# ZhangT-tech/MoCA-Video

Hardware: AMD Instinct MI355X
Metric: denoising UNet-steps/sec @16x320x512 fp16 (higher is better)
Workload: dtype f16

## Files before the change

include/moca_hip.h:

```cpp
#ifndef MOCA_HIP_H
#define MOCA_HIP_H

#include <stdint.h>

#ifdef __cplusplus
extern "C" {
#endif

#define MOCA_OK            0
#define MOCA_E_BADARG     -1
#define MOCA_E_LAUNCH     -2
#define MOCA_E_NODEVICE   -3
#define MOCA_E_GRAPH      -4

#define MOCA_A_LINEAR   0
#define MOCA_A_CONV3X3  1
#define MOCA_A_TCONV3   2

#define MOCA_EP_GEGLU   1
#define MOCA_EP_OUT_F32 2
#define MOCA_FORCE_SMALL_TILE 4
#define MOCA_EP_COLSUM 16
#define MOCA_EP_LN     32
#define MOCA_EP_GELU    8
#define MOCA_EP_ROWSUM 64
#define MOCA_EP_GSTAT  256
#define MOCA_EP_TATTN  512
#define MOCA_EP_LNFOLD 128

#define MOCA_EP_SLABS 1024

typedef struct moca_gemm_params {
    const void* a;
    const void* w;
    void*       out;
    const float* bias;
    const void* rowadd;
    const void* residual;
    float*      splitk_ws;
    int32_t M, N, K;
    int32_t lda, ldw, ldo, ldr, ld_rowadd;
    int32_t rowadd_div;
    int32_t a_mode;
    int32_t C;
    int32_t inH, inW;
    int32_t outH, outW;
    int32_t stride;
    int32_t up;
    int32_t T;
    int32_t HW;
    int32_t flags;
    int32_t splits;
    int32_t nopad_lo;
    int32_t prefetch_kib;
    int32_t tattn_causal;
    float*      colsum;
    const float* ln_gamma;
    const float* ln_beta;
    void*       ln_out;
    int32_t     ld_ln;
    float       ln_eps;
    float*      rowsum;
    const float* lnf_part;
    const float* lnf_wsum;
    int32_t     lnf_nparts;
    int32_t     reserved2_;
    int64_t*    gstat;
    int32_t     gstat_rows;
    float       tattn_scale;
    const void* prefetch;
    int32_t     up_phase;
    int32_t     reserved4_;
    const void* a2;
    int32_t     lda2;
    int32_t     k1;
    int32_t     gstat_cpg;
    int32_t     gstat_coff;
    int32_t     wgroup_rows;
    int32_t     wgroup_stride;
} moca_gemm_params;

int moca_gemm_f16(const moca_gemm_params* p, void* stream);
int moca_gemm_colsum_rows(const moca_gemm_params* p);
int moca_gemm_ln_ok(const moca_gemm_params* p);
int moca_gemm_rowsum_cols(const moca_gemm_params* p);
int moca_gemm_lnfold_ok(const moca_gemm_params* p);
int moca_gemm_tattn_ok(const moca_gemm_params* p);
int moca_gemm_wgroup_ok(const moca_gemm_params* p);
int moca_gemm_cat_ok(const moca_gemm_params* p);
#define MOCA_ROUTE_SMALL64   1
#define MOCA_ROUTE_SMALL128  2
#define MOCA_ROUTE_GLDS128   3
#define MOCA_ROUTE_GLDS160   4
#define MOCA_ROUTE_G4        5
#define MOCA_ROUTE_W80       6
#define MOCA_ROUTE_W80W      7
#define MOCA_ROUTE_SQ256     8
#define MOCA_ROUTE_G4P       9
#define MOCA_ROUTE_SQP       10
#define MOCA_ROUTE_TATTN     11
#define MOCA_ROUTE_WS        12
int moca_gemm_route(const moca_gemm_params* p);
int moca_gemm_splitk_groupnorm_ok(const moca_gemm_params* p, int32_t HW, int32_t frames_per_stat);
int moca_gemm_splitk_groupnorm_f16(const moca_gemm_params* p, void* y, const float* gamma, const float* beta, int32_t HW,
                                   int32_t frames_per_stat, float eps, int32_t silu, int32_t write_x, void* stream);
int64_t moca_gemm_splitk_ws_bytes(int32_t M, int32_t N, int32_t splits);

int moca_groupnorm_nhwc_f16(const void* x, void* y, const float* gamma, const float* beta,
                            int32_t F, int32_t HW, int32_t C, int32_t frames_per_stat,
                            float eps, int32_t silu, float* ws, void* stream);
int64_t moca_groupnorm_ws_bytes(int32_t F, int32_t HW, int32_t C);
int moca_groupnorm_colsum_f16(const void* x, void* y, const float* gamma, const float* beta, const float* colsum,
                              int32_t tile_rows, int32_t F, int32_t HW, int32_t C, int32_t frames_per_stat,
                              float eps, int32_t silu, float* ws, void* stream);

int moca_groupnorm_fold_weights_f16(const void* w, const float* bias, const float* gamma, const float* beta, const int64_t* gstat,
                                    void* wg, float* bg, int32_t n_sg, int32_t N, int32_t K, int32_t ldw, int64_t count, float eps,
                                    void* stream);

int moca_groupnorm_gstat_f16(const void* x, void* y, const float* gamma, const float* beta, const int64_t* gstat,
                             int32_t F, int32_t HW, int32_t C, int32_t frames_per_stat,
                             float eps, int32_t silu, void* stream);
int moca_concat_channels_gstat_f16(const void* a, const void* b, void* out, int32_t F, int32_t HW, int32_t C1, int32_t C2,
                                   int32_t frames_per_stat, int64_t* gstat, void* stream);
int moca_groupnorm_gstat_cat_f16(const void* a, const void* b, void* y, const float* gamma, const float* beta,
                                 const int64_t* gstat_cat, const int64_t* gstat_b, int32_t Fb, int32_t F, int32_t HW, int32_t C1,
                                 int32_t C2, int32_t frames_per_stat, float eps, int32_t silu, void* stream);
int moca_gstat_accum_f16(const void* x, int32_t F, int32_t HW, int32_t C, int32_t frames_per_stat, int32_t cpg, int32_t coff,
                         int64_t* gstat, void* stream);
int moca_memset_zero(void* ptr, int64_t bytes, void* stream);

int moca_layernorm_f16(const void* x, void* y, const float* gamma, const float* beta,
                       int32_t M, int32_t C, float eps, void* stream);

int moca_attention_f16(const void* q, const void* k, const void* v, void* out,
                       int32_t Bq, int32_t heads, int32_t Nq, int32_t Nk,
                       int32_t ldq, int32_t ldk, int32_t ldv, int32_t ldo,
                       int32_t kv_div, float scale, void* stream);

int moca_attention_ip_f16(const void* q, const void* k, const void* v, const void* k_ip, const void* v_ip, void* out,
                          int32_t Bq, int32_t heads, int32_t Nq, int32_t Nt, int32_t Ni,
                          int32_t ldq, int32_t ldk, int32_t ldv, int32_t ldk_ip, int32_t ldv_ip, int32_t ldo,
                          int32_t kv_div, float scale, float ip_scale, void* stream);

int moca_attention_causal_f16(const void* q, const void* k, const void* v, void* out,
                              int32_t B, int32_t heads, int32_t N, int32_t ldq, int32_t ldk, int32_t ldv, int32_t ldo,
                              float scale, void* stream);

int moca_temporal_attention_f16(const void* q, const void* k, const void* v, void* out,
                                int32_t B, int32_t T, int32_t HW, int32_t heads,
                                int32_t ld_qkv, int32_t ldo, float scale, void* stream);
int moca_temporal_attention_causal_f16(const void* q, const void* k, const void* v, void* out,
                                       int32_t B, int32_t T, int32_t HW, int32_t heads,
                                       int32_t ld_qkv, int32_t ldo, float scale, void* stream);
int moca_temporal_attention_long_f16(const void* q, const void* k, const void* v, void* out,
                                     int32_t B, int32_t T, int32_t HW, int32_t heads,
                                     int32_t ld_qkv, int32_t ldo, float scale, int32_t causal, void* stream);

int moca_ncthw_to_nhwc_f16(const void* x, int32_t x_is_f32, void* y, int32_t B, int32_t Cin,
                           int32_t T, int32_t HW, int32_t Cpad, void* stream);
int moca_ncthw_scatter_f16(const void* x, int32_t x_is_f32, void* y, int32_t B, int32_t k, int32_t T,
                           int32_t HW, int32_t Cpad, int32_t c0, void* stream);
int moca_nchw_add_rows_f16(void* rows, const void* src, int32_t src_is_f32, int32_t F, int32_t Fsrc, int32_t C,
                           int32_t HW, int32_t ld, void* stream);
int moca_nhwc_to_ncthw(const void* y, int32_t ld, void* x, int32_t x_is_f32, int32_t B,
                       int32_t Cout, int32_t T, int32_t HW, void* stream);
int moca_concat_channels_f16(const void* a, const void* b, void* out, int64_t rows,
                             int32_t C1, int32_t C2, void* stream);
int moca_repeat_f16(const void* src, void* dst, int64_t bytes, int32_t reps, void* stream);
int moca_timestep_embedding_f16(const int64_t* t, void* out, int32_t n, int32_t dim,
                                float max_period, void* stream);
int moca_silu_add_rows_f16(const void* a, int32_t div_a, const void* b, int32_t div_b, void* out,
                           int32_t rows, int32_t C, int32_t apply_silu, void* stream);

int moca_embed_tokens_f16(const int64_t* tokens, const float* table, const float* pos, void* out,
                          int32_t n_tokens, int32_t L, int32_t C, int32_t vocab, void* stream);

int moca_attention_d80_f16(const void* q, const void* k, const void* v, void* out,
                           int32_t B, int32_t heads, int32_t N, int32_t ldq, int32_t ldk, int32_t ldv, int32_t ldo,
                           float scale, void* stream);
int moca_clip_preprocess_patches_f16(const void* img, int32_t img_is_f32, void* out, int32_t B, int32_t H, int32_t W,
                                     int32_t size, int32_t patch, int32_t ldo, int32_t antialias, void* stream);
int moca_clip_assemble_tokens_f16(const float* patch, int32_t ldp, const float* cls, const float* pos, void* out, int32_t B, int32_t P,
                                  int32_t C, void* stream);

int moca_channel_mix_f16(const void* z, int32_t z_is_f32, const float* w, const float* bias, void* out,
                         int32_t B, int32_t Cin, int32_t T, int32_t HW, int32_t Cout, int32_t Cpad,
                         float inv_scale, void* stream);
int moca_gaussian_sample_f32(const float* moments, const float* noise, float* out, int32_t n, int32_t z, int32_t hw,
                             float scale, void* stream);
int moca_softmax_rows_f16(const float* s, void* p, int64_t R, int32_t N, int64_t lds, int64_t ldp, float scale,
                          void* stream);

int moca_cfg_combine_f32(const float* e_c, const float* e_u, float* out, float scale,
                         int64_t n, void* stream);
int moca_ddim_update_f32(const float* x, const float* e, const float* noise, float* x_prev,
                         float* pred_x0, float a_t, float a_prev, float sigma_t,
                         float sqrt_one_minus_at, int32_t use_scale, float scale_t,
                         float scale_prev, int64_t n, void* stream);
int moca_q_sample_f32(const float* x0, const float* noise, float* out, const float* coef_x, const float* coef_n,
                      const int64_t* t, int32_t B, int32_t n_tab, int64_t per, void* stream);
int moca_fifo_ddim_step_f32(const float* sample, const float* eps, const float* noise,
                            float* momentum, float* x_prev, float* pred_x0,
                            const float* coef, const float* mask, const float* cond,
                            const int32_t* mask_index, const float* enh, float* ws,
                            int32_t B, int32_t C, int32_t F, int32_t Fm, int32_t HW,
                            float beta, float one_minus_beta, float gamma, float one_minus_gamma,
                            void* stream);

typedef struct moca_fifo_state {
    int32_t head;
    int32_t iter;
    uint32_t seed_lo, seed_hi;
    int32_t ext_noise;
    int32_t reserved_[3];
} moca_fifo_state;

int moca_fifo_randn_f32(const moca_fifo_state* state, float* out, int64_t n, void* stream);
int moca_fifo_gather_windows_f32(const moca_fifo_state* state, const float* queue, float* x, float* anchor,
                                 const int32_t* win_start, int32_t nW, int32_t reps, int32_t C, int32_t Q, int32_t f,
                                 int32_t HW, void* stream);
typedef struct moca_fifo_step_params {
    const moca_fifo_state* state;
    const float* x;
    const float* eps_c;
    const float* eps_u;
    const float* noise;
    float* momentum;
    float* queue;
    float* x_prev;
    float* pred_x0;
    const float* coef;
    const int32_t* win_start;
    const float* mask;
    const float* mask_sums;
    const int32_t* mask_frame;
    const float* enh;
    const float* cond;
    const float* sam_eff;
    const int32_t* sam_idx;
    float cfg_scale, beta, one_minus_beta, gamma, one_minus_gamma;
    int32_t nW, C, Q, f, HW, wb_from;
} moca_fifo_step_params;
int moca_fifo_step_windows_f32(const moca_fifo_step_params* p, void* stream);
int moca_sam_select_masks_f32(const float* cand, const int32_t* cand_off, const int32_t* ncand, const int64_t* t_rows, float* eff,
                              int32_t* eff_idx, int32_t nW, int32_t f, int32_t HW, void* stream);
int moca_fifo_advance_f32(moca_fifo_state* state, float* queue, const float* newframe, float* emitted, int32_t n_slots,
                          int32_t emit_frame, float* mask, float* mask_sums, int32_t C, int32_t Q, int32_t HW, void* stream);
int moca_fifo_prepare_queue_f32(const float* z, const float* noise, float* queue, const float* coef_z, const float* coef_noise,
                                const int32_t* frame_idx, int32_t BC, int32_t Tz, int32_t Q, int32_t HW, void* stream);
int moca_base_set_timestep(const moca_fifo_state* state, const int64_t* table, int32_t S, int64_t* rows, int32_t n, void* stream);
int moca_base_ddim_step_f32(moca_fifo_state* state, float* x, const float* eps_c, const float* eps_u, const float* noise,
                            float* pred_x0, const float* coef, int32_t S, float cfg_scale, int32_t use_scale, int64_t n, void* stream);
int moca_mask_frame_sums_f32(const float* mask, float* sums, int32_t frames, int32_t HW, void* stream);

int moca_freq_mix_3d_f32(const float* x, const float* noise, const float* lpf, float* out,
                         int32_t C, int32_t T, int32_t H, int32_t W, float* ws, void* stream);
int64_t moca_freq_mix_ws_bytes(int32_t C, int32_t T, int32_t H, int32_t W);
int moca_freq_filter_f32(float* lpf, int32_t T, int32_t H, int32_t W, int32_t type, int32_t n,
                         double d_s, double d_t, void* stream);

int moca_graph_begin(void* stream);
int moca_graph_end(void* stream, void** graph_exec_out);
int moca_graph_launch(void* graph_exec, void* stream);
int moca_graph_destroy(void* graph_exec);
int moca_stream_create(void** stream_out);
int moca_stream_destroy(void* stream);
int moca_stream_sync(void* stream);
int moca_event_create(void** ev_out);
int moca_event_record(void* ev, void* stream);
int moca_event_elapsed_ms(void* ev_start, void* ev_stop, float* ms_out);
int moca_event_destroy(void* ev);

#define MOCA_TUNE_GEMM_W80   0
#define MOCA_TUNE_GEMM_G4    1
#define MOCA_TUNE_GEMM_SQ256 2
#define MOCA_TUNE_GEMM_WIDE  3
#define MOCA_TUNE_GN_SLAB    4
#define MOCA_TUNE_GEMM_G4P   5
#define MOCA_TUNE_GEMM_MF32  6
#define MOCA_TUNE_GEMM_SQP   7
#define MOCA_TUNE_SQP_WALK   8
#define MOCA_TUNE_SLAB_F16   9
#define MOCA_TUNE_GEMM_WS    10
#define MOCA_TUNE_COUNT      11
int moca_set_tuning(int32_t knob, int32_t value);
int moca_debug_clock_sampler(void* buf, int32_t blocks, int32_t nsamples, const int32_t* stop, void* stream);

int moca_device_info(char* name, int32_t len, int32_t* cu_count);
const char* moca_version(void);

#ifdef __cplusplus
}
#endif
#endif
```

moca_video_amd/csrc/gemm.hip:

```cpp
#include "gemm_launch.h"

namespace {

template <int BN, int AMODE>
__global__ __launch_bounds__(256, 2) void gemm_f16_kernel(const moca_gemm_params p) {
    constexpr int NT = BN / 64;
    constexpr int B_SLOTS = BN / 32;
    constexpr int A_BYTES = BM * ROW_BYTES;
    constexpr int B_BYTES = BN * ROW_BYTES;

    extern __shared__ __attribute__((aligned(16))) char smem[];
    char* sA = smem;
    char* sB = smem + 2 * A_BYTES;

    const int tid = threadIdx.x, lane = tid & 63, wave = tid >> 6;
    const int wave_m = wave >> 1, wave_n = wave & 1;

    const int tiles_m = (p.M + BM - 1) / BM;
    const int tiles_n = p.N / BN;
    const int nblk = tiles_m * tiles_n * p.splits;
    int logical;
    remap_block<BN>(nblk, logical);
    const int split = logical % p.splits;
    const int tile = logical / p.splits;
// ... 148 lines not shown
                    acc[mt][nt] = __builtin_amdgcn_mfma_f32_32x32x16_f16(af[mt], bf[nt], acc[mt][nt], 0, 0, 0);
        }
        if (has_next) store_tile(cur ^ 1);
        __syncthreads();
        cur ^= 1;
    }

    if (p.splits > 1) {
        float* ws = p.splitk_ws + (int64_t)split * p.M * p.N;
#pragma unroll
        for (int mt = 0; mt < 2; ++mt)
#pragma unroll
            for (int nt = 0; nt < NT; ++nt)
#pragma unroll
                for (int r = 0; r < 16; ++r) {
                    const int row = m0 + wave_m * 64 + mt * 32 + (r & 3) + 8 * (r >> 2) + 4 * fh;
                    const int col = n0 + wave_n * (BN / 2) + nt * 32 + frow;
                    if (row < p.M) ws[(int64_t)row * p.N + col] = acc[mt][nt][r];
                }
        return;
    }

    float* sC = reinterpret_cast<float*>(smem);
    const bool geglu = (p.flags & MOCA_EP_GEGLU) != 0;
    const int out_bn = geglu ? BN / 2 : BN;
    if (geglu) {
        if constexpr (NT == 2) {
            const int ncol = n0 + wave_n * 64 + frow;
            const float bv = p.bias ? p.bias[ncol] : 0.f;
            const float bg = p.bias ? p.bias[ncol + 32] : 0.f;
#pragma unroll
            for (int mt = 0; mt < 2; ++mt)
#pragma unroll
                for (int r = 0; r < 16; ++r) {
                    const int row = wave_m * 64 + mt * 32 + (r & 3) + 8 * (r >> 2) + 4 * fh;
                    const float v = acc[mt][0][r] + bv;
                    const float g = acc[mt][1][r] + bg;
                    sC[row * out_bn + wave_n * 32 + frow] = v * moca_gelu(g);
                }
        }
    } else {
#pragma unroll
        for (int nt = 0; nt < NT; ++nt) {
            const int col = wave_n * (BN / 2) + nt * 32 + frow;
            const float bv = p.bias ? p.bias[n0 + col] : 0.f;
#pragma unroll
            for (int mt = 0; mt < 2; ++mt)
#pragma unroll
                for (int r = 0; r < 16; ++r) {
                    const int row = wave_m * 64 + mt * 32 + (r & 3) + 8 * (r >> 2) + 4 * fh;
                    const float v = acc[mt][nt][r] + bv;
                    sC[row * out_bn + col] = (p.flags & MOCA_EP_GELU) ? moca_gelu(v) : v;
                }
        }
    }
    __syncthreads();

    const int chunks_per_row = out_bn / 8;
    const int total_chunks = BM * chunks_per_row;
    const int on0 = geglu ? n0 / 2 : n0;
    const half_t* __restrict__ rowadd = reinterpret_cast<const half_t*>(p.rowadd);
    const half_t* __restrict__ resid = reinterpret_cast<const half_t*>(p.residual);
    for (int idx = tid; idx < total_chunks; idx += 256) {
        const int row = idx / chunks_per_row, ch = idx - row * chunks_per_row;
        const int m = m0 + row;
        if (m >= p.M) continue;
        const int col = on0 + ch * 8;
        float v[8];
        const f32x4 c0 = *reinterpret_cast<const f32x4*>(sC + row * out_bn + ch * 8);
        const f32x4 c1 = *reinterpret_cast<const f32x4*>(sC + row * out_bn + ch * 8 + 4);
        v[0] = c0[0]; v[1] = c0[1]; v[2] = c0[2]; v[3] = c0[3];
        v[4] = c1[0]; v[5] = c1[1]; v[6] = c1[2]; v[7] = c1[3];
        if (rowadd) {
            const half8v e = *reinterpret_cast<const half8v*>(rowadd + (int64_t)(m / p.rowadd_div) * p.ld_rowadd + col);
#pragma unroll
            for (int j = 0; j < 8; ++j) v[j] += (float)e[j];
        }
        if (resid) {
            const half8v e = *reinterpret_cast<const half8v*>(resid + (int64_t)m * p.ldr + col);
#pragma unroll
            for (int j = 0; j < 8; ++j) v[j] += (float)e[j];
        }
        if (p.flags & MOCA_EP_OUT_F32) {
            float* o = reinterpret_cast<float*>(p.out) + (int64_t)m * p.ldo + col;
            *reinterpret_cast<f32x4*>(o) = f32x4{v[0], v[1], v[2], v[3]};
            *reinterpret_cast<f32x4*>(o + 4) = f32x4{v[4], v[5], v[6], v[7]};
        } else {
            half8v h;
#pragma unroll
            for (int j = 0; j < 8; ++j) h[j] = (half_t)v[j];
            *reinterpret_cast<half8v*>(reinterpret_cast<half_t*>(p.out) + (int64_t)m * p.ldo + col) = h;
        }
    }
}

__global__ __launch_bounds__(256) void splitk_reduce_kernel(const moca_gemm_params p) {
    const bool geglu = (p.flags & MOCA_EP_GEGLU) != 0;
    const int out_n = geglu ? p.N / 2 : p.N;
    const int cpr = out_n / 8;
    const int64_t total = (int64_t)p.M * cpr;
    const half_t* __restrict__ rowadd = reinterpret_cast<const half_t*>(p.rowadd);
    const half_t* __restrict__ resid = reinterpret_cast<const half_t*>(p.residual);
    for (int64_t idx = (int64_t)blockIdx.x * 256 + threadIdx.x; idx < total; idx += (int64_t)gridDim.x * 256) {
        const int m = (int)(idx / cpr), ch = (int)(idx - (int64_t)m * cpr);
        const int col = ch * 8;
        float v[8];
        if (geglu) {
            const int vc = (col / 32) * 64 + (col % 32);
            float a[8], g[8];
#pragma unroll
            for (int j = 0; j < 8; ++j) { a[j] = p.bias ? p.bias[vc + j] : 0.f; g[j] = p.bias ? p.bias[vc + 32 + j] : 0.f; }
            for (int s = 0; s < p.splits; ++s) {
                const float* w = p.splitk_ws + ((int64_t)s * p.M + m) * p.N + vc;
                const f32x4 a0 = *reinterpret_cast<const f32x4*>(w), a1 = *reinterpret_cast<const f32x4*>(w + 4);
                const f32x4 g0 = *reinterpret_cast<const f32x4*>(w + 32), g1 = *reinterpret_cast<const f32x4*>(w + 36);
#pragma unroll
                for (int j = 0; j < 4; ++j) { a[j] += a0[j]; a[4 + j] += a1[j]; g[j] += g0[j]; g[4 + j] += g1[j]; }
            }
#pragma unroll
            for (int j = 0; j < 8; ++j) v[j] = a[j] * moca_gelu(g[j]);
        } else {
#pragma unroll
            for (int j = 0; j < 8; ++j) v[j] = p.bias ? p.bias[col + j] : 0.f;
            if (p.reserved4_ & 4) {
                for (int s = 0; s < p.splits; ++s) {
                    const half8v a = *reinterpret_cast<const half8v*>(reinterpret_cast<const half_t*>(p.splitk_ws) + ((int64_t)s * p.M + m) * p.N + col);
#pragma unroll
                    for (int j = 0; j < 8; ++j) v[j] += (float)a[j];
                }
            } else {
                for (int s = 0; s < p.splits; ++s) {
                    const float* w = p.splitk_ws + ((int64_t)s * p.M + m) * p.N + col;
                    const f32x4 a0 = *reinterpret_cast<const f32x4*>(w), a1 = *reinterpret_cast<const f32x4*>(w + 4);
#pragma unroll
                    for (int j = 0; j < 4; ++j) { v[j] += a0[j]; v[4 + j] += a1[j]; }
                }
            }
        }
        if (rowadd) {
            const half8v e = *reinterpret_cast<const half8v*>(rowadd + (int64_t)(m / p.rowadd_div) * p.ld_rowadd + col);
#pragma unroll
            for (int j = 0; j < 8; ++j) v[j] += (float)e[j];
        }
        if (resid) {
            const half8v e = *reinterpret_cast<const half8v*>(resid + (int64_t)m * p.ldr + col);
#pragma unroll
            for (int j = 0; j < 8; ++j) v[j] += (float)e[j];
        }
        if (p.flags & MOCA_EP_OUT_F32) {
            float* o = reinterpret_cast<float*>(p.out) + (int64_t)m * p.ldo + col;
            *reinterpret_cast<f32x4*>(o) = f32x4{v[0], v[1], v[2], v[3]};
            *reinterpret_cast<f32x4*>(o + 4) = f32x4{v[4], v[5], v[6], v[7]};
        } else {
            half8v h;
#pragma unroll
            for (int j = 0; j < 8; ++j) h[j] = (half_t)v[j];
            *reinterpret_cast<half8v*>(reinterpret_cast<half_t*>(p.out) + (int64_t)m * p.ldo + col) = h;
        }
    }
}

template <int CPT>
__global__ __launch_bounds__(1024) void splitk_gn_kernel(const moca_gemm_params p, half_t* __restrict__ y, const float* __restrict__ gamma,
                                                         const float* __restrict__ beta, int R, int cpg, double inv_count, float eps,
                                                         int silu, int write_x) {
    __shared__ float s_red[2][16];
    __shared__ float s_sc[128], s_sh[128];
    const int tid = threadIdx.x, nthr = blockDim.x;
    const int slab = blockIdx.x, sg = slab / 32, g = slab % 32;
    const int vpr = cpg / 8, nchunks = R * vpr;
    const int N = p.N;
    const half_t* __restrict__ rowadd = reinterpret_cast<const half_t*>(p.rowadd);
    const half_t* __restrict__ resid = reinterpret_cast<const half_t*>(p.residual);
    const float gm_t = tid < cpg ? gamma[g * cpg + tid] : 0.f, bt_t = tid < cpg ? beta[g * cpg + tid] : 0.f;
    half8v v[CPT];
    int mrow[CPT], ccol[CPT];
    float s = 0.f, q = 0.f;
#pragma unroll
    for (int i = 0; i < CPT; ++i) {
        const int idx = tid + i * nthr;
        mrow[i] = -1;
        if (idx < nchunks) {
            const int row = idx / vpr, c = idx - row * vpr;
            const int m = sg * R + row, col = g * cpg + c * 8;
            mrow[i] = m; ccol[i] = col;
            float a[8];
#pragma unroll
            for (int j = 0; j < 8; ++j) a[j] = p.bias ? p.bias[col + j] : 0.f;
            if (p.reserved4_ & 4) {
                for (int sp = 0; sp < p.splits; ++sp) {
                    const half8v h = *reinterpret_cast<const half8v*>(reinterpret_cast<const half_t*>(p.splitk_ws) + ((int64_t)sp * p.M + m) * N + col);
#pragma unroll
                    for (int j = 0; j < 8; ++j) a[j] += (float)h[j];
                }
            } else {
                for (int sp = 0; sp < p.splits; ++sp) {
                    const float* w = p.splitk_ws + ((int64_t)sp * p.M + m) * N + col;
                    const f32x4 a0 = *reinterpret_cast<const f32x4*>(w), a1 = *reinterpret_cast<const f32x4*>(w + 4);
#pragma unroll
                    for (int j = 0; j < 4; ++j) { a[j] += a0[j]; a[4 + j] += a1[j]; }
                }
            }
            if (rowadd) {
                const half8v e = *reinterpret_cast<const half8v*>(rowadd + (int64_t)(m / p.rowadd_div) * p.ld_rowadd + col);
#pragma unroll
                for (int j = 0; j < 8; ++j) a[j] += (float)e[j];
            }
            if (resid) {
                const half8v e = *reinterpret_cast<const half8v*>(resid + (int64_t)m * p.ldr + col);
#pragma unroll
                for (int j = 0; j < 8; ++j) a[j] += (float)e[j];
            }
#pragma unroll
            for (int j = 0; j < 8; ++j) v[i][j] = (half_t)a[j];
            if (write_x) *reinterpret_cast<half8v*>(reinterpret_cast<half_t*>(p.out) + (int64_t)m * p.ldo + col) = v[i];
        }
    }
#pragma unroll
    for (int i = 0; i < CPT; ++i)
        if (mrow[i] >= 0) {
#pragma unroll
            for (int j = 0; j < 8; ++j) { const float a = (float)v[i][j]; s += a; q += a * a; }
        }
    s = wave_sum(s); q = wave_sum(q);
    if ((tid & 63) == 0) { s_red[0][tid >> 6] = s; s_red[1][tid >> 6] = q; }
    __syncthreads();
    if (tid < cpg) {
        double a = 0.0, b = 0.0;
        for (int w = 0; w < (nthr >> 6); ++w) { a += (double)s_red[0][w]; b += (double)s_red[1][w]; }
        const double mean = a * inv_count;
        double var = b * inv_count - mean * mean;
        if (var < 0.0) var = 0.0;
        const float rstd = (float)(1.0 / sqrt(var + (double)eps));
        const float sc = rstd * gm_t;
        s_sc[tid] = sc;
        s_sh[tid] = bt_t - (float)mean * sc;
    }
    __syncthreads();
#pragma unroll
    for (int i = 0; i < CPT; ++i)
        if (mrow[i] >= 0) {
            const int c0 = ccol[i] - g * cpg;
            half8v r;
#pragma unroll
            for (int j = 0; j < 8; ++j) {
                float a = (float)v[i][j] * s_sc[c0 + j] + s_sh[c0 + j];
                if (silu) a = moca_silu(a);
                r[j] = (half_t)a;
            }
            *reinterpret_cast<half8v*>(y + (int64_t)mrow[i] * N + ccol[i]) = r;
        }
}

template <int BN, int AMODE>
int launch_gemm(const moca_gemm_params& p, hipStream_t st) {
    const int tiles_m = (p.M + BM - 1) / BM, tiles_n = p.N / BN;
    const int nblk = tiles_m * tiles_n * p.splits;
    constexpr int lds_pipe = 2 * (BM + BN) * ROW_BYTES;
    constexpr int lds_epi = BM * BN * 4;
    constexpr int lds = lds_pipe > lds_epi ? lds_pipe : lds_epi;
    if (!dyn_lds_once<&gemm_f16_kernel<BN, AMODE>>(lds)) return MOCA_E_LAUNCH;
    hipLaunchKernelGGL((gemm_f16_kernel<BN, AMODE>), dim3(nblk), dim3(256), lds, st, p);
    MOCA_CHECK_LAUNCH();
    return MOCA_OK;
}
int launch_gemm_small(int bn, const moca_gemm_params& p, hipStream_t st) {
    if (bn == 128) return with_gather(p, [&](auto am, auto) { return launch_gemm<128, decltype(am)::value>(p, st); });
    return with_gather(p, [&](auto am, auto) { return launch_gemm<64, decltype(am)::value>(p, st); });
}

enum Route : int {
    R_NONE = 0,
    R_SMALL64 = MOCA_ROUTE_SMALL64, R_SMALL128 = MOCA_ROUTE_SMALL128, R_GLDS128 = MOCA_ROUTE_GLDS128, R_GLDS160 = MOCA_ROUTE_GLDS160,
    R_G4 = MOCA_ROUTE_G4, R_W80 = MOCA_ROUTE_W80, R_W80W = MOCA_ROUTE_W80W, R_SQ256 = MOCA_ROUTE_SQ256, R_G4P = MOCA_ROUTE_G4P,
    R_SQP = MOCA_ROUTE_SQP, R_TATTN = MOCA_ROUTE_TATTN, R_WS = MOCA_ROUTE_WS,
};

void normalise_splits(moca_gemm_params& p) {
    if (p.splits < 1) p.splits = 1;
    if (p.splits > (p.K + BK - 1) / BK) p.splits = (p.K + BK - 1) / BK;
    if (p.splits > 1) {
        const int nkt = (p.K + BK - 1) / BK, kts = (nkt + p.splits - 1) / p.splits;
        p.splits = (nkt + kts - 1) / kts;
    }
}

inline int64_t a_span_bytes(const moca_gemm_params& p) {
    if (p.a_mode == MOCA_A_LINEAR) return ((int64_t)p.M * p.lda + 64) * 2;
    if (p.a_mode == MOCA_A_CONV3X3) return ((int64_t)(p.M / (p.outH * p.outW)) * p.inH * p.inW * p.C + 64) * 2;
    return ((int64_t)p.M * p.C + 64) * 2;
}
inline bool buffer_addressable(const moca_gemm_params& p) {
    if (p.a2 && ((int64_t)p.M * p.lda2 + 64) * 2 >= (1ll << 31)) return false;
    return a_span_bytes(p) < (1ll << 31) && (int64_t)p.N * p.ldw * 2 < (1ll << 31);
}

bool persistent_ok(const moca_gemm_params& p, int BN, int blocks) {
    if (p.a_mode != MOCA_A_LINEAR || p.splits != 1 || p.N % BN || p.K % 64 || !buffer_addressable(p)) return false;
    if (p.flags & ~(MOCA_EP_GEGLU | MOCA_EP_LNFOLD)) return false;
    if ((p.flags & MOCA_EP_GEGLU) && (p.residual || p.rowadd)) return false;
    return ((p.M + 255) / 256) * (p.N / BN) >= blocks;
}

Route route_of(const moca_gemm_params& p) {
    if (p.flags & MOCA_EP_TATTN) return R_TATTN;
    const int ws_mode = moca_tuning_get(MOCA_TUNE_GEMM_WS);
    if (ws_mode && moca_gemm_ws_ok(p) && (ws_mode == 2 || p.residual || p.M >= (1 << 17))) return R_WS;
    if (!p.a2 && p.wgroup_rows <= 0) {
        const int sqp_mode = moca_tuning_get(MOCA_TUNE_GEMM_SQP), g4p_mode = moca_tuning_get(MOCA_TUNE_GEMM_G4P);
        if (sqp_mode && persistent_ok(p, 256, SQP_BLOCKS) && (sqp_mode == 2 || (p.flags & MOCA_EP_GEGLU))) return R_SQP;
        if (g4p_mode && persistent_ok(p, 128, G4P_BLOCKS) && (g4p_mode == 2 || (p.flags & MOCA_EP_GEGLU))) return R_G4P;
    }
    const int w80_mode = moca_tuning_get(MOCA_TUNE_GEMM_W80);
    const int tiles320 = ((p.M + 319) / 320) * (p.N / 160);
    if (w80_mode && p.N % 160 == 0 && !(p.flags & (MOCA_EP_GEGLU | MOCA_EP_OUT_F32 | MOCA_FORCE_SMALL_TILE)) && p.M > 160 &&
        (tiles320 * p.splits >= 200 || w80_mode == 2) && fast_gather(p) && buffer_addressable(p)) {
        if (p.flags & MOCA_EP_LN) return R_W80W;
        const int wide_mode = moca_tuning_get(MOCA_TUNE_GEMM_WIDE);
        if (wide_mode == 0 || p.N % 320) return R_W80;
        return (p.a_mode == MOCA_A_LINEAR || wide_mode == 2) ? R_W80W : R_W80;
    }
    const int g4_mode = moca_tuning_get(MOCA_TUNE_GEMM_G4);
    const bool use_g4 = !(p.flags & MOCA_EP_OUT_F32) &&
                        (g4_mode == 2 || (g4_mode == 1 && (p.flags & MOCA_EP_GEGLU) && p.K <= 640 && p.M < (1 << 17)));
    const int sq256_mode = moca_tuning_get(MOCA_TUNE_GEMM_SQ256);
    if (sq256_mode && p.a_mode == MOCA_A_LINEAR && p.N % 256 == 0 && p.N >= 2560 && p.M >= 512 && fast_gather(p) && buffer_addressable(p) &&
        !(p.flags & (MOCA_EP_OUT_F32 | MOCA_FORCE_SMALL_TILE)) && ((p.M + 255) / 256) * (p.N / 256) * p.splits >= 200 &&
        (sq256_mode == 2 || !use_g4)) return R_SQ256;
    const int big_bn = (p.N % 128 == 0) ? 128 : (p.N % 160 == 0 ? 160 : 0);
    if (big_bn != 0 && p.M > 128 && !(p.flags & MOCA_FORCE_SMALL_TILE)) {
        if (big_bn == 128) return use_g4 ? R_G4 : R_GLDS128;
        return R_GLDS160;
    }
    return p.N % 128 == 0 ? R_SMALL128 : R_SMALL64;
}

constexpr int CAN_SPLITK = 1 << 16, CAN_A2 = 1 << 17, CAN_WGROUP = 1 << 18, CAN_UP_PHASE = 1 << 19;
constexpr int EP_STATS = MOCA_EP_COLSUM | MOCA_EP_GSTAT;
struct RouteInfo { int tm, tn, can; };
RouteInfo route_info(Route r) {
    constexpr int GLDS = MOCA_EP_GEGLU | MOCA_EP_OUT_F32 | EP_STATS | MOCA_EP_ROWSUM | MOCA_EP_LNFOLD | CAN_SPLITK | CAN_UP_PHASE;
    constexpr int W80 = EP_STATS | MOCA_EP_ROWSUM | MOCA_EP_LNFOLD | CAN_SPLITK | CAN_UP_PHASE | CAN_A2 | CAN_WGROUP;
    switch (r) {
        case R_SMALL64: return {BM, 64, MOCA_EP_OUT_F32 | MOCA_EP_GELU | CAN_SPLITK};
        case R_SMALL128: return {BM, 128, MOCA_EP_GEGLU | MOCA_EP_OUT_F32 | MOCA_EP_GELU | CAN_SPLITK};
        case R_GLDS128: return {256, 128, GLDS};
        case R_GLDS160: return {256, 160, GLDS};
        case R_G4: return {256, 128, MOCA_EP_GEGLU | MOCA_EP_LNFOLD | CAN_SPLITK | CAN_UP_PHASE};
        case R_W80: return {320, 160, W80};
        case R_W80W: return {160, 320, W80 | MOCA_EP_LN};
        case R_SQ256: return {256, 256, MOCA_EP_GEGLU | MOCA_EP_LNFOLD | CAN_SPLITK};
        case R_G4P: return {256, 128, MOCA_EP_GEGLU | MOCA_EP_LNFOLD};
        case R_SQP: return {256, 256, MOCA_EP_GEGLU | MOCA_EP_LNFOLD};
        case R_TATTN: return {320, 192, MOCA_EP_TATTN | MOCA_EP_LNFOLD};
        case R_WS: return {32, 80, MOCA_EP_ROWSUM | MOCA_EP_GSTAT | CAN_WGROUP};
        case R_NONE: break;
    }
    return {0, 0, 0};
}

bool route_can(Route r, const moca_gemm_params& p) {
    const RouteInfo ri = route_info(r);
    const int f = p.flags & ~(MOCA_FORCE_SMALL_TILE | MOCA_EP_SLABS);
    const int wants = f | (p.splits > 1 ? CAN_SPLITK : 0) | (p.a2 ? CAN_A2 : 0) | (p.wgroup_rows ? CAN_WGROUP : 0) | (p.up_phase ? CAN_UP_PHASE : 0);
    if (r == R_NONE || (wants & ~ri.can) || p.wgroup_rows < 0) return false;
    if (r == R_WS) return true;
    const bool linear1 = p.a_mode == MOCA_A_LINEAR && p.splits == 1;
    if (r == R_TATTN) {
        if (!linear1 || !fast_gather(p) || !buffer_addressable(p) || p.residual || p.rowadd || (p.flags & MOCA_FORCE_SMALL_TILE)) return false;
        if (p.N % 192 || p.T != 16 || p.HW <= 0 || p.HW % 20 || p.M % (16 * p.HW)) return false;
        if (p.ldo % 4 || p.ldo < p.N / 3) return false;
        return p.tattn_causal == 0 || (p.tattn_causal == 1 && p.tattn_scale > 0.f);
    }
    if ((f & EP_STATS) && (p.splits != 1 || (f & (MOCA_EP_GEGLU | MOCA_EP_OUT_F32)))) return false;
    if ((f & MOCA_EP_ROWSUM) && (p.splits != 1 || (f & (MOCA_EP_GEGLU | MOCA_EP_OUT_F32 | EP_STATS | MOCA_EP_LN | MOCA_EP_GELU)))) return false;
    if ((f & MOCA_EP_LN) && !(linear1 && p.N == 320 && !(f & EP_STATS))) return false;
    if ((f & MOCA_EP_LNFOLD) && !(linear1 && !(f & (MOCA_EP_OUT_F32 | EP_STATS | MOCA_EP_LN | MOCA_EP_ROWSUM | MOCA_EP_GELU)) &&
                                  !((r == R_GLDS128 || r == R_GLDS160) && (f & MOCA_EP_GEGLU)))) return false;
    if ((f & MOCA_EP_GELU) && (f & MOCA_EP_GEGLU)) return false;
    if (p.a2) {
        if (!linear1 || (f & ~(EP_STATS | MOCA_EP_ROWSUM))) return false;
        if (p.k1 <= 0 || p.k1 >= p.K || p.k1 % 64 || (p.K - p.k1) % 64 || p.lda % 8 || p.lda2 % 8 || p.lda < p.k1 || p.lda2 < p.K - p.k1) return false;
    }
    if (p.wgroup_rows) {
        if (!linear1 || p.a2 || p.wgroup_stride < p.N * p.ldw || (f & ~(EP_STATS | MOCA_EP_ROWSUM | MOCA_EP_LN))) return false;
        if (p.M % p.wgroup_rows || p.wgroup_rows % ri.tm) return false;
        if ((int64_t)(p.M / p.wgroup_rows) * p.wgroup_stride * 2 >= (1ll << 31)) return false;
    }
    if (p.up_phase && (p.splits != 1 || p.M <= 160 || !fast_gather(p) || p.residual || p.rowadd || (f & ~MOCA_EP_GSTAT) ||
                       (p.N % 128 && p.N % 160))) return false;
    return true;
}

Route checked_route(const moca_gemm_params& p) {
    const Route r = route_of(p);
    return route_can(r, p) ? r : R_NONE;
}

Route query_route(const moca_gemm_params* pp, int flag, moca_gemm_params& p) {
    if (!pp) return R_NONE;
    p = *pp;
    if (p.M <= 0 || p.N <= 0 || p.K <= 0 || p.N % 64 || p.K % 8) return R_NONE;
    normalise_splits(p);
    p.flags |= flag;
    return checked_route(p);
}

bool slab_f16(Route r, const moca_gemm_params& p) {
    return moca_tuning_get(MOCA_TUNE_SLAB_F16) && p.splits > 1 && !(p.flags & (MOCA_EP_GEGLU | MOCA_EP_OUT_F32)) && (r == R_GLDS128 || r == R_GLDS160);
}
bool splitk_gn_ok(const moca_gemm_params& p, int HW, int fps) {
    if (p.splits < 2 || (p.flags & ~MOCA_EP_SLABS) || p.N % 32 || (p.N / 32) % 8 || p.N / 32 > 128 || p.up_phase) return false;
    if (HW <= 0 || fps <= 0 || p.M % (HW * fps)) return false;
    const int64_t nchunks = (int64_t)HW * fps * (p.N / 32 / 8);
    return nchunks >= 64 && nchunks <= 4096;
}

Route prepare(const moca_gemm_params* pp, moca_gemm_params& p) {
    if (!pp) return R_NONE;
    p = *pp;
    if (p.splits < 1) p.splits = 1;
    if (!p.a || !p.w || !p.out) return R_NONE;
    if (p.M <= 0 || p.N <= 0 || p.K <= 0) return R_NONE;
    if (p.N % 64 || p.K % 8 || p.ldw % BK || p.ldw < ((p.K + BK - 1) / BK) * BK) return R_NONE;
    const bool geglu = p.flags & MOCA_EP_GEGLU;
    if (geglu && p.N % 128) return R_NONE;
    if (p.ldo % 8 || (p.residual && p.ldr % 8) || (p.rowadd && (p.ld_rowadd % 8 || p.rowadd_div <= 0))) return R_NONE;
    if (p.splits > 1 && !p.splitk_ws) return R_NONE;
    if (p.prefetch_kib < 0 || (p.prefetch_kib > 0 && (!p.prefetch || (reinterpret_cast<uintptr_t>(p.prefetch) & 15)))) return R_NONE;
    if ((p.flags & MOCA_EP_GELU) && (p.splits != 1 || !((p.flags & MOCA_FORCE_SMALL_TILE) || p.M <= 128))) return R_NONE;
    normalise_splits(p);
    if ((p.flags & MOCA_EP_SLABS) && (p.splits < 2 || (p.flags & ~MOCA_EP_SLABS))) return R_NONE;
    if (p.up_phase && p.a_mode != MOCA_A_CONV3X3) return R_NONE;
    switch (p.a_mode) {
        case MOCA_A_LINEAR:
            if (!p.a2 && (p.lda % 8 || p.lda < p.K)) return R_NONE;
            break;
        case MOCA_A_CONV3X3:
            if (p.up_phase < 0 || p.up_phase > 4) return R_NONE;
            if (p.C % 8 || p.K != (p.up_phase ? 4 : 9) * p.C || p.inH <= 0 || p.inW <= 0 || p.outH <= 0 || p.outW <= 0) return R_NONE;
            if (p.up_phase && (p.stride != 1 || p.up || p.nopad_lo)) return R_NONE;
            if (p.stride != 1 && p.stride != 2) return R_NONE;
            if (p.nopad_lo != 0 && (p.nopad_lo != 1 || p.stride != 2 || p.up || (p.inH | p.inW) & 1)) return R_NONE;
            if (p.up && (p.stride != 1 || p.outH != 2 * p.inH || p.outW != 2 * p.inW)) return R_NONE;
            if (!p.up && p.stride == 1 && (p.outH != p.inH || p.outW != p.inW)) return R_NONE;
            if (p.stride == 2 && (p.outH != (p.inH - 1) / 2 + 1 || p.outW != (p.inW - 1) / 2 + 1)) return R_NONE;
            if (p.M % (p.outH * p.outW)) return R_NONE;
            break;
        case MOCA_A_TCONV3:
            if (p.C % 8 || p.K != 3 * p.C || p.T <= 0 || p.HW <= 0 || p.M % (p.T * p.HW)) return R_NONE;
            break;
        default:
            return R_NONE;
    }
    if (p.a2 && p.a_mode != MOCA_A_LINEAR) return R_NONE;
    if (p.gstat_cpg < 0 || p.gstat_coff < 0 || ((p.gstat_cpg || p.gstat_coff) && !(p.flags & MOCA_EP_GSTAT))) return R_NONE;
    if (p.tattn_causal && !(p.flags & MOCA_EP_TATTN)) return R_NONE;
    const Route r = checked_route(p);
    if (r == R_NONE) return R_NONE;
    if ((p.flags & MOCA_EP_COLSUM) && !p.colsum) return R_NONE;
    if ((p.flags & MOCA_EP_LN) && !(p.ln_gamma && p.ln_beta && p.ln_out && p.ld_ln % 8 == 0)) return R_NONE;
    if ((p.flags & MOCA_EP_ROWSUM) && !p.rowsum) return R_NONE;
    if ((p.flags & MOCA_EP_LNFOLD) && !(p.lnf_part && p.lnf_wsum && p.lnf_nparts >= 1)) return R_NONE;
    if ((p.flags & MOCA_EP_GSTAT) &&
        !(p.gstat && !(p.flags & MOCA_EP_COLSUM) && p.gstat_rows > 0 && p.gstat_rows % route_info(r).tm == 0 && p.M % p.gstat_rows == 0 &&
          (p.gstat_cpg > 0 ? (p.gstat_coff + p.N - 1) / p.gstat_cpg < 32 : (p.N % 32 == 0 && p.gstat_coff == 0)))) return R_NONE;
    p.reserved4_ = 0;
    if ((int64_t)p.M * (geglu ? p.N / 2 : p.N) * 2 >= (128ll << 20)) p.reserved4_ |= 1;
    if (slab_f16(r, p)) p.reserved4_ |= 4;
    return r;
}

int launch_route(Route r, const moca_gemm_params& p, hipStream_t st) {
    switch (r) {
        case R_TATTN: return moca_gemm_w80s_launch(3, p, st);
        case R_WS: return moca_gemm_ws_launch(p, st);
        case R_SQP: return moca_gemm_sqp_launch(p, st);
        case R_G4P: return moca_gemm_g4p_launch(p, st);
        case R_W80: return moca_gemm_w80s_launch(0, p, st);
        case R_W80W: return moca_gemm_w80s_launch(1, p, st);
        case R_SQ256: return moca_gemm_w80s_launch(2, p, st);
        case R_G4: return moca_gemm_g4_launch(p, st);
        case R_GLDS128: return moca_gemm_glds_launch(128, p, st);
        case R_GLDS160: return moca_gemm_glds_launch(160, p, st);
        case R_SMALL128: return launch_gemm_small(128, p, st);
        case R_SMALL64: return launch_gemm_small(64, p, st);
        case R_NONE: break;
    }
    return MOCA_E_BADARG;
}

}

#ifdef MOCA_STAMPS
extern "C" int moca_debug_stamps(unsigned long long* host_out, int n_blocks) {
    if (n_blocks > STAMP_BLOCKS) n_blocks = STAMP_BLOCKS;
    return hipMemcpyFromSymbol(host_out, HIP_SYMBOL(g_stamps), (size_t)n_blocks * STAMP_SLOTS * 8) == hipSuccess ? 0 : -2;
}
#endif

extern "C" int moca_gemm_route(const moca_gemm_params* pp) {
    moca_gemm_params p;
    return prepare(pp, p);
}

extern "C" int moca_gemm_colsum_rows(const moca_gemm_params* pp) {
    moca_gemm_params p;
    return route_info(query_route(pp, (pp && (pp->flags & MOCA_EP_GSTAT)) ? 0 : MOCA_EP_COLSUM, p)).tm;
}
extern "C" int moca_gemm_rowsum_cols(const moca_gemm_params* pp) {
    moca_gemm_params p;
    return route_info(query_route(pp, MOCA_EP_ROWSUM, p)).tn;
}
extern "C" int moca_gemm_ln_ok(const moca_gemm_params* pp) {
    moca_gemm_params p;
    return query_route(pp, MOCA_EP_LN, p) != R_NONE;
}
extern "C" int moca_gemm_lnfold_ok(const moca_gemm_params* pp) {
    moca_gemm_params p;
    return query_route(pp, MOCA_EP_LNFOLD, p) != R_NONE;
}
extern "C" int moca_gemm_tattn_ok(const moca_gemm_params* pp) {
    moca_gemm_params p;
    return query_route(pp, MOCA_EP_TATTN, p) != R_NONE;
}
extern "C" int moca_gemm_cat_ok(const moca_gemm_params* pp) {
    moca_gemm_params p;
    return query_route(pp, 0, p) != R_NONE && p.a2;
}
extern "C" int moca_gemm_wgroup_ok(const moca_gemm_params* pp) {
    moca_gemm_params p;
    return query_route(pp, 0, p) != R_NONE && p.wgroup_rows > 0;
}
extern "C" int moca_gemm_splitk_groupnorm_ok(const moca_gemm_params* pp, int32_t HW, int32_t frames_per_stat) {
    moca_gemm_params p;
    return query_route(pp, 0, p) != R_NONE && splitk_gn_ok(p, HW, frames_per_stat);
}

extern "C" int moca_gemm_splitk_groupnorm_f16(const moca_gemm_params* pp, void* y, const float* gamma, const float* beta, int32_t HW,
                                              int32_t frames_per_stat, float eps, int32_t silu, int32_t write_x, void* stream) {
    if (!pp || !y || !gamma || !beta) return MOCA_E_BADARG;
    moca_gemm_params p = *pp;
    if (p.M <= 0 || p.N <= 0 || p.K <= 0 || p.N % 64 || p.K % 8 || !p.splitk_ws || (write_x && !p.out)) return MOCA_E_BADARG;
    if (p.ldo % 8 || (p.residual && p.ldr % 8) || (p.rowadd && (p.ld_rowadd % 8 || p.rowadd_div <= 0))) return MOCA_E_BADARG;
    normalise_splits(p);
    if (!splitk_gn_ok(p, HW, frames_per_stat)) return MOCA_E_BADARG;
    p.reserved4_ = slab_f16(route_of(p), p) ? 4 : 0;
    const int cpg = p.N / 32, R = HW * frames_per_stat;
    const int nchunks = R * (cpg / 8);
    const int cpt = (nchunks + 1023) / 1024;
    int thr = ((nchunks + cpt - 1) / cpt + 63) / 64 * 64;
    if (thr < (cpg + 63) / 64 * 64) thr = (cpg + 63) / 64 * 64;
    const int n_slabs = (p.M / R) * 32;
    const double inv_count = 1.0 / ((double)R * cpg);
    hipStream_t st = moca_stream(stream);
    half_t* yo = reinterpret_cast<half_t*>(y);
#define MOCA_SKGN(CPT) hipLaunchKernelGGL(splitk_gn_kernel<CPT>, dim3(n_slabs), dim3(thr), 0, st, p, yo, gamma, beta, R, cpg, inv_count, eps, silu, write_x)
    if (cpt == 1) MOCA_SKGN(1); else if (cpt == 2) MOCA_SKGN(2); else if (cpt == 3) MOCA_SKGN(3); else MOCA_SKGN(4);
#undef MOCA_SKGN
    MOCA_CHECK_LAUNCH();
    return MOCA_OK;
}

extern "C" int64_t moca_gemm_splitk_ws_bytes(int32_t M, int32_t N, int32_t splits) {
    return splits > 1 ? (int64_t)splits * M * N * 4 : 0;
}

extern "C" int moca_gemm_f16(const moca_gemm_params* pp, void* stream) {
    moca_gemm_params p;
    const Route r = prepare(pp, p);
    if (r == R_NONE) return MOCA_E_BADARG;
    hipStream_t st = moca_stream(stream);
    const int rc = launch_route(r, p, st);
    if (rc != MOCA_OK) return rc;
    if (p.splits > 1 && !(p.flags & MOCA_EP_SLABS)) {
        const int out_n = (p.flags & MOCA_EP_GEGLU) ? p.N / 2 : p.N;
        const int64_t total = (int64_t)p.M * (out_n / 8);
        int blocks = (int)((total + 255) / 256);
        if (blocks > 2048) blocks = 2048;
        hipLaunchKernelGGL(splitk_reduce_kernel, dim3(blocks), dim3(256), 0, st, p);
        MOCA_CHECK_LAUNCH();
    }
    return MOCA_OK;
}

#ifdef MOCA_DIAG_NAME
extern "C" const char* moca_version(void) { return "moca_hip 0.1 (gfx950) DIAG:" MOCA_DIAG_NAME; }
#else
extern "C" const char* moca_version(void) { return "moca_hip 0.1 (gfx950)"; }
#endif
```

moca_video_amd/csrc/gemm_launch.h:

```cpp
#ifndef MOCA_GEMM_LAUNCH_H
#define MOCA_GEMM_LAUNCH_H
#include "gemm_device.h"

int moca_gemm_glds_launch(int bn, const moca_gemm_params& p, hipStream_t st);
int moca_gemm_g4_launch(const moca_gemm_params& p, hipStream_t st);
int moca_gemm_w80s_launch(int shape, const moca_gemm_params& p, hipStream_t st);
int moca_gemm_g4p_launch(const moca_gemm_params& p, hipStream_t st);
int moca_gemm_sqp_launch(const moca_gemm_params& p, hipStream_t st);

namespace {

constexpr int G4P_BLOCKS = 512;
constexpr int SQP_BLOCKS = 256;

static int choose_xcd_n(const moca_gemm_params& p, int tiles_m, int tiles_n, int BN) {
    if (p.splits != 1 || p.a_mode != MOCA_A_LINEAR) return 1;
    const double Wtot = (double)p.N * p.K * 2, Atot = (double)p.M * p.K * 2;
    auto cost = [&](int xn) {
        const int xm = 8 / xn;
        const double wsub = (double)(tiles_n / xn) * BN * p.K * 2;
        return (wsub <= 3.6e6 ? xm * Wtot : tiles_m * Wtot) + xn * Atot;
    };
    double best = cost(1);
    int best_xn = 1;
    for (int xn = 2; xn <= 8; xn *= 2) {
        if (tiles_m % (8 / xn) || tiles_n % xn) continue;
        const double c = cost(xn);
        if (c < 0.8 * best) { best = c; best_xn = xn; }
    }
    return best_xn;
}

inline bool fast_gather(const moca_gemm_params& p) {
    return (p.a_mode == MOCA_A_LINEAR) ? (p.K % BK == 0 && p.K <= 8192) : (p.C % BK == 0 && p.C <= 8192);
}
template <typename F>
int with_gather(const moca_gemm_params& p, F f) {
    const bool fast = fast_gather(p);
    if (p.a_mode == MOCA_A_LINEAR) return fast ? f(int_c<MOCA_A_LINEAR>{}, yes_t{}) : f(int_c<MOCA_A_LINEAR>{}, no_t{});
    if (p.a_mode == MOCA_A_CONV3X3) return fast ? f(int_c<MOCA_A_CONV3X3>{}, yes_t{}) : f(int_c<MOCA_A_CONV3X3>{}, no_t{});
    return fast ? f(int_c<MOCA_A_TCONV3>{}, yes_t{}) : f(int_c<MOCA_A_TCONV3>{}, no_t{});
}

template <auto KERNEL>
bool dyn_lds_once(int lds) {
    static bool attr_set = false;
    if (!attr_set) {
        if (hipFuncSetAttribute(reinterpret_cast<const void*>(KERNEL), hipFuncAttributeMaxDynamicSharedMemorySize, lds) != hipSuccess) return false;
        attr_set = true;
    }
    return true;
}

}

#endif
```

moca_video_amd/csrc/gemm_persistent.hip:

```cpp
#include "gemm_launch.h"

namespace {

__device__ __forceinline__ int g4p_perm(int rho) {
    const int wn = rho >> 6, nt = (rho >> 4) & 3, j = rho & 15;
    return wn * 64 + (nt >> 1) * 32 + 8 * (j >> 2) + 4 * (nt & 1) + (j & 3);
}
__device__ __forceinline__ void st_out8_nt(half_t* ptr, const half8v v, bool nt) { st_out8(ptr, v, nt); }

template <bool GEGLU>
__global__ __launch_bounds__(256, 2) void gemm_g4p_kernel(const moca_gemm_params p) {
#if defined(__HIP_DEVICE_COMPILE__)
    constexpr int TM = 256, BN = 128, KS = 32, RB = 64, MT = 8, NT = 4;
    constexpr int A_BYTES = TM * RB, STAGE = A_BYTES + BN * RB, RING = 3 * STAGE;
    constexpr int NMMA = MT * NT;
    extern __shared__ __attribute__((aligned(16))) char smem[];
    float* lst = reinterpret_cast<float*>(smem + RING);
    float* lws = lst + 2 * TM;
    float* lbi = lws + BN;

    const int tid = threadIdx.x, lane = tid & 63;
    const int wave = __builtin_amdgcn_readfirstlane(tid >> 6);
    const int wave_m = wave >> 1, wave_n = wave & 1;
    const int nper = p.reserved2_;
// ... 200 lines not shown
#pragma unroll
                    for (int r = 0; r < 4; ++r) { o[r] = v[2 * hh][r]; o[4 + r] = v[2 * hh + 1][r]; }
                    if (m < p.M) {
                        if (rowadd) {
                            const half8v e = *reinterpret_cast<const half8v*>(rowadd + (int64_t)(m / p.rowadd_div) * p.ld_rowadd + col);
#pragma unroll
                            for (int r = 0; r < 8; ++r) o[r] = (float)(half_t)o[r] + (float)e[r];
                        }
                        if (resid) {
                            const half8v e = *reinterpret_cast<const half8v*>(resid + (int64_t)m * p.ldr + col);
#pragma unroll
                            for (int r = 0; r < 8; ++r) o[r] = (rowadd ? o[r] : (float)(half_t)o[r]) + (float)e[r];
                        }
                        half8v h;
#pragma unroll
                        for (int r = 0; r < 8; ++r) h[r] = (half_t)o[r];
                        st_out8(reinterpret_cast<half_t*>(p.out) + (int64_t)m * p.ldo + col, h, nt_out);
                    }
                }
            }
        }
#ifdef MOCA_STAMPS
        if (stamp_it) { MOCA_STAMP(5); MOCA_STAMP_HW(); }
        ++tile_no;
#endif
        if (t_next < 0) break;
        t_cur = t_next;
        asm volatile("s_waitcnt vmcnt(0) lgkmcnt(0)" ::: "memory");
        __builtin_amdgcn_s_barrier();
    }
#endif
}

__device__ __forceinline__ int g4q_perm(int rho) {
    const int wn = rho >> 6, nt = (rho >> 5) & 1, i = rho & 31;
    const int g = i >> 3, h = (i >> 2) & 1, r = i & 3;
    return wn * 64 + nt * 32 + 16 * (g >> 1) + 8 * h + 4 * (g & 1) + r;
}
template <bool GEGLU>
__global__ __launch_bounds__(256, 2) void gemm_g4q_kernel(const moca_gemm_params p) {
#if defined(__HIP_DEVICE_COMPILE__)
    constexpr int TM = 256, BN = 128, KS = 32, RB = 64, MT = 4, NT = 2;
    constexpr int A_BYTES = TM * RB, STAGE = A_BYTES + BN * RB, RING = 3 * STAGE;
        extern __shared__ __attribute__((aligned(16))) char smem[];
    float* lst = reinterpret_cast<float*>(smem + RING);
    float* lws = lst + 2 * TM;
    float* lbi = lws + BN;

    const int tid = threadIdx.x, lane = tid & 63;
    const int wave = __builtin_amdgcn_readfirstlane(tid >> 6);
    const int wave_m = wave >> 1, wave_n = wave & 1;
    const int nper = p.reserved2_;
    if (prefetch_block(p, nper, 256)) return;

    const int tiles_n = p.N / BN;
    const int ntiles = ((p.M + TM - 1) / TM) * tiles_n;
    int t_cur, t_end;
    const int J = nper >> 3;
    {
        const int x = blockIdx.x & 7, j = blockIdx.x >> 3;
        const int q = ntiles >> 3, r = ntiles & 7;
        const int start = x < r ? x * (q + 1) : r * (q + 1) + (x - r) * q;
        t_cur = start + j;
        t_end = start + q + (x < r ? 1 : 0);
    }
    if (t_cur >= t_end) return;
    const int nk = 2 * (p.K / 64);

    const int lrow = lane >> 2, pch = lane & 3;
    const int lch = pch ^ ((0x78 >> (2 * ((lrow >> 2) & 3))) & 3);
    const __amdgpu_buffer_rsrc_t rsrc_a = __builtin_amdgcn_make_buffer_rsrc(const_cast<void*>(p.a), 0, OOB_OFF, 0x00020000);
    const __amdgpu_buffer_rsrc_t rsrc_w = __builtin_amdgcn_make_buffer_rsrc(const_cast<void*>(p.w), 0, OOB_OFF, 0x00020000);
    unsigned a_off[4], w_off[2];
    int w_perm[2];
#pragma unroll
    for (int g = 0; g < 2; ++g) w_perm[g] = g4q_perm((g * 4 + wave) * 16 + lrow);
    auto set_dma_tile = [&](int t) {
        const int tm = t / tiles_n, tn = t - tm * tiles_n;
#pragma unroll
        for (int g = 0; g < 4; ++g) {
            const int row = tm * TM + (g * 4 + wave) * 16 + lrow;
            a_off[g] = (t >= 0 && row < p.M) ? (unsigned)(((int64_t)row * p.lda + lch * 8) * 2) : OOB_OFF;
        }
#pragma unroll
        for (int g = 0; g < 2; ++g)
            w_off[g] = t >= 0 ? (unsigned)(((int64_t)(tn * BN + w_perm[g]) * p.ldw + lch * 8) * 2) : OOB_OFF;
    };
    auto dma_piece = [&](int kt, int slot, int j) {
        const lds_ptr sa = (lds_ptr)smem + slot * STAGE;
        const unsigned soff = (unsigned)(kt * KS * 2);
        if (j < 4) __builtin_amdgcn_raw_ptr_buffer_load_lds(rsrc_a, sa + (j * 4 + wave) * 1024, 16, a_off[j], soff, 0, 0);
        else __builtin_amdgcn_raw_ptr_buffer_load_lds(rsrc_w, sa + A_BYTES + ((j - 4) * 4 + wave) * 1024, 16, w_off[j - 4], soff, 0, 0);
    };

    const int fr = lane & 31, fh = lane >> 5;
    int fa_off[MT][2], fb_off[NT][2];
#pragma unroll
    for (int ks = 0; ks < 2; ++ks) {
#pragma unroll
        for (int mt = 0; mt < MT; ++mt) {
            const int row = wave_m * 128 + mt * 32 + fr;
            fa_off[mt][ks] = row * RB + (((2 * ks + fh) ^ ((0x78 >> (2 * ((row >> 2) & 3))) & 3)) << 4);
        }
#pragma unroll
        for (int nt = 0; nt < NT; ++nt) {
            const int row = wave_n * 64 + nt * 32 + fr;
            fb_off[nt][ks] = A_BYTES + row * RB + (((2 * ks + fh) ^ ((0x78 >> (2 * ((row >> 2) & 3))) & 3)) << 4);
        }
    }

    f32x16 acc[MT][NT];
    half8v af[MT][2], bf[NT][2];
    int s0 = 0, s1 = 1, s2 = 2;
    auto phase = [&](auto even_tag, int kt2) {
        constexpr bool even = decltype(even_tag)::value;
        const char* cur = smem + s0 * STAGE;
#pragma unroll
        for (int ks = 0; ks < 2; ++ks) {
#pragma unroll
            for (int nt = 0; nt < NT; ++nt) bf[nt][ks] = *reinterpret_cast<const half8v*>(cur + fb_off[nt][ks]);
#pragma unroll
            for (int mt = 0; mt < MT; ++mt) af[mt][ks] = *reinterpret_cast<const half8v*>(cur + fa_off[mt][ks]);
        }
        if constexpr (even) {
            asm volatile("s_waitcnt lgkmcnt(0)" ::: "memory");
            __builtin_amdgcn_s_barrier();
        }
        __builtin_amdgcn_s_setprio(1);
#pragma unroll
        for (int j = 0; j < 2 * MT * NT; ++j) {
            const int ks = j / (MT * NT), mt = (j / NT) % MT, nt = j % NT;
            acc[mt][nt] = __builtin_amdgcn_mfma_f32_32x32x16_f16(bf[nt][ks], af[mt][ks], acc[mt][nt], 0, 0, 0);
            if constexpr (even) {
                if ((j & 1) && j / 2 < 6) {
                    dma_piece(kt2, s2, j / 2);
                    dma_piece(kt2 + 1, s0, j / 2);
                    __builtin_amdgcn_sched_barrier(0);
                }
            }
        }
        __builtin_amdgcn_s_setprio(0);
        { const int t = s0; s0 = s1; s1 = s2; s2 = t; }
    };

    const bool fold = (p.flags & MOCA_EP_LNFOLD) != 0;
    float2 rp0, rp1;
    float rws, rbi;
    auto stat_issue = [&](int t) {
        const int tm = t / tiles_n, tn = t - tm * tiles_n;
        rp0 = float2{0.f, 0.f}; rp1 = float2{0.f, 0.f}; rws = 0.f; rbi = 0.f;
        if (tid < BN) {
            const int n = tn * BN + g4q_perm(tid);
            if (fold) rws = p.lnf_wsum[n];
            if (p.bias) rbi = p.bias[n];
        }
        if (fold) {
            const int m = min(tm * TM + tid, p.M - 1);
            rp0 = *reinterpret_cast<const float2*>(p.lnf_part + (int64_t)m * 2);
            if (p.lnf_nparts > 1) rp1 = *reinterpret_cast<const float2*>(p.lnf_part + ((int64_t)p.M + m) * 2);
        }
    };
    auto stat_publish = [&](int t) {
        float rs = 1.f, rb = 0.f;
        if (fold) {
            const int tm = t / tiles_n;
            const int m = min(tm * TM + tid, p.M - 1);
            float s = rp0.x + rp1.x, q = rp0.y + rp1.y;
            for (int i = 2; i < p.lnf_nparts; ++i) {
                const float2 v = *reinterpret_cast<const float2*>(p.lnf_part + ((int64_t)i * p.M + m) * 2);
                s += v.x; q += v.y;
            }
            const float inv_k = 1.0f / (float)p.K;
            const float mean = s * inv_k;
            const float var = fmaxf(q * inv_k - mean * mean, 0.f);
            rs = rsqrtf(var + p.ln_eps);
            rb = -mean * rs;
        }
        *reinterpret_cast<float2*>(lst + 2 * tid) = float2{rs, rb};
        if (tid < BN) { lws[tid] = rws; lbi[tid] = rbi; }
    };

    stat_issue(t_cur);
    set_dma_tile(t_cur);
#pragma unroll
    for (int j = 0; j < 6; ++j) { dma_piece(0, 0, j); dma_piece(1, 1, j); }
    asm volatile("s_waitcnt vmcnt(0)" ::: "memory");
    __builtin_amdgcn_s_barrier();

    const bool nt_out = out_streams(p);
    const half_t* __restrict__ resid = reinterpret_cast<const half_t*>(p.residual);
    const half_t* __restrict__ rowadd = reinterpret_cast<const half_t*>(p.rowadd);
    while (true) {
        const int t_next = t_cur + J < t_end ? t_cur + J : -1;
        const int tm = t_cur / tiles_n, tn = t_cur - tm * tiles_n;
        const int m0 = tm * TM, n0 = tn * BN;
#pragma unroll
        for (int mt = 0; mt < MT; ++mt)
#pragma unroll
            for (int nt = 0; nt < NT; ++nt)
#pragma unroll
                for (int r = 0; r < 16; ++r) acc[mt][nt][r] = 0.f;
        for (int i = 0; i < nk; i += 2) {
            const bool last = i + 2 >= nk;
            if (last) set_dma_tile(t_next);
            phase(yes_t{}, last ? 0 : i + 2);
            asm volatile("s_waitcnt lgkmcnt(0)" ::: "memory");
            __builtin_amdgcn_s_barrier();
            phase(no_t{}, 0);
            if (!last) {
                asm volatile("s_waitcnt vmcnt(0) lgkmcnt(0)" ::: "memory");
                __builtin_amdgcn_s_barrier();
            }
        }
        stat_publish(t_cur);
        if (t_next >= 0) stat_issue(t_next);
        asm volatile("s_waitcnt lgkmcnt(0)" ::: "memory");
        __builtin_amdgcn_s_barrier();

        f32x4 cw[NT][4], cb[NT][4];
        if constexpr (GEGLU) {
#pragma unroll
            for (int nt = 0; nt < NT; ++nt)
#pragma unroll
                for (int g = 0; g < 4; ++g) {
                    cw[nt][g] = *reinterpret_cast<const f32x4*>(lws + wave_n * 64 + nt * 32 + 8 * g + 4 * fh);
                    cb[nt][g] = *reinterpret_cast<const f32x4*>(lbi + wave_n * 64 + nt * 32 + 8 * g + 4 * fh);
                }
        }
#pragma unroll
        for (int mt = 0; mt < MT; ++mt) {
            const int rl = wave_m * 128 + mt * 32 + fr;
            const int m = m0 + rl;
            const float2 st = *reinterpret_cast<const float2*>(lst + 2 * rl);
#pragma unroll
            for (int s = 0; s < 2; ++s) {
                f32x4 v[NT][2];
#pragma unroll
                for (int nt = 0; nt < NT; ++nt)
#pragma unroll
                    for (int gg = 0; gg < 2; ++gg) {
                        const int g = 2 * s + gg;
                        const f32x4 a4 = {acc[mt][nt][4 * g], acc[mt][nt][4 * g + 1], acc[mt][nt][4 * g + 2], acc[mt][nt][4 * g + 3]};
                        if constexpr (!GEGLU) {
                            cw[nt][g] = *reinterpret_cast<const f32x4*>(lws + wave_n * 64 + nt * 32 + 8 * g + 4 * fh);
                            cb[nt][g] = *reinterpret_cast<const f32x4*>(lbi + wave_n * 64 + nt * 32 + 8 * g + 4 * fh);
                        }
                        v[nt][gg] = st.x * a4 + (st.y * cw[nt][g] + cb[nt][g]);
                    }
                if constexpr (GEGLU) {
                    half8v h;
#pragma unroll
                    for (int gg = 0; gg < 2; ++gg) {
                        const f32x2 lo = moca_geglu2(f32x2{v[0][gg][0], v[0][gg][1]}, f32x2{v[1][gg][0], v[1][gg][1]});
                        const f32x2 hi = moca_geglu2(f32x2{v[0][gg][2], v[0][gg][3]}, f32x2{v[1][gg][2], v[1][gg][3]});
                        h[4 * gg + 0] = (half_t)lo[0]; h[4 * gg + 1] = (half_t)lo[1]; h[4 * gg + 2] = (half_t)hi[0]; h[4 * gg + 3] = (half_t)hi[1];
                    }
                    if (m < p.M) st_out8(reinterpret_cast<half_t*>(p.out) + (int64_t)m * p.ldo + (n0 >> 1) + wave_n * 32 + 16 * s + 8 * fh, h, nt_out);
                } else {
#pragma unroll
                    for (int nt = 0; nt < NT; ++nt) {
                        const int col = n0 + wave_n * 64 + nt * 32 + 16 * s + 8 * fh;
                        float o[8];
#pragma unroll
                        for (int r = 0; r < 4; ++r) { o[r] = v[nt][0][r]; o[4 + r] = v[nt][1][r]; }
                        if (m < p.M) {
                            if (rowadd) {
                                const half8v e = *reinterpret_cast<const half8v*>(rowadd + (int64_t)(m / p.rowadd_div) * p.ld_rowadd + col);
#pragma unroll
                                for (int r = 0; r < 8; ++r) o[r] = (float)(half_t)o[r] + (float)e[r];
                            }
                            if (resid) {
                                const half8v e = *reinterpret_cast<const half8v*>(resid + (int64_t)m * p.ldr + col);
#pragma unroll
                                for (int r = 0; r < 8; ++r) o[r] = (rowadd ? o[r] : (float)(half_t)o[r]) + (float)e[r];
                            }
                            half8v h;
#pragma unroll
                            for (int r = 0; r < 8; ++r) h[r] = (half_t)o[r];
                            st_out8(reinterpret_cast<half_t*>(p.out) + (int64_t)m * p.ldo + col, h, nt_out);
                        }
                    }
                }
            }
        }
        if (t_next < 0) break;
        t_cur = t_next;
        asm volatile("s_waitcnt vmcnt(0) lgkmcnt(0)" ::: "memory");
        __builtin_amdgcn_s_barrier();
    }
#endif
}

__device__ __forceinline__ void lds_wr_f2(unsigned a, f32x2 v) { asm volatile("ds_write_b64 %0, %1" ::"v"(a), "v"(v) : "memory"); }
__device__ __forceinline__ void lds_wr_f1(unsigned a, float v) { asm volatile("ds_write_b32 %0, %1" ::"v"(a), "v"(v) : "memory"); }
__device__ __forceinline__ f32x2 lds_rd_f2(unsigned a) { f32x2 v; asm volatile("ds_read_b64 %0, %1" : "=v"(v) : "v"(a) : "memory"); return v; }
__device__ __forceinline__ f32x4 lds_rd_f4(unsigned a) { f32x4 v; asm volatile("ds_read_b128 %0, %1" : "=v"(v) : "v"(a) : "memory"); return v; }
__device__ __forceinline__ float lds_rd_f1(unsigned a) { float v; asm volatile("ds_read_b32 %0, %1" : "=v"(v) : "v"(a) : "memory"); return v; }
__device__ __forceinline__ void lds_wait() { asm volatile("s_waitcnt lgkmcnt(0)" ::: "memory"); __builtin_amdgcn_sched_barrier(0); }

__device__ __forceinline__ int sqp_perm(int rho) {
    return (rho & ~63) + (g4p_perm(rho & 127) & 63);
}

template <bool GEGLU>
__global__ __launch_bounds__(512, 2) void gemm_sqp_kernel(const moca_gemm_params p) {
#if defined(__HIP_DEVICE_COMPILE__)
#ifndef SEG_WAVE
#define SEG_WAVE 0
#endif
    constexpr int MT = 4, NT = 8, KS = 32, RB = 64, WTM = 64, WTN = 128, TM = 256, BN = 256;
    constexpr int A_BYTES = TM * RB, STAGE = A_BYTES + BN * RB, NS = 5, PPW = 4;
    extern __shared__ __attribute__((aligned(16))) char smem[];

    const int tid = threadIdx.x, lane = tid & 63;
    const int wave = __builtin_amdgcn_readfirstlane(tid >> 6);
    const int wave_m = wave >> 1, wave_n = wave & 1;
    const bool late = wave >= 4;
    const int nper = p.reserved2_;
    if (prefetch_block(p, nper, 512)) return;

    const int tiles_n = p.N / BN, tiles_m = (p.M + TM - 1) / TM;
    const int xcd_n = p.reserved4_ >> 8;
    const int J = nper >> 3;
    int q_base, q_cnt, sub_n, tm_base, tn_base;
    {
        const int x = blockIdx.x & 7;
        if (xcd_n > 1) {
            const int xm = 8 / xcd_n, sm = tiles_m / xm;
            sub_n = tiles_n / xcd_n;
            const int xi = x / xcd_n, xj = x - xi * xcd_n;
            tm_base = xi * sm; tn_base = xj * sub_n;
            q_base = 0; q_cnt = sm * sub_n;
        } else {
            const int ntiles = tiles_m * tiles_n, q = ntiles >> 3, r = ntiles & 7;
            q_base = x < r ? x * (q + 1) : r * (q + 1) + (x - r) * q;
            q_cnt = q + (x < r ? 1 : 0);
            sub_n = tiles_n; tm_base = 0; tn_base = 0;
        }
    }
    auto tile_of = [&](int q, int& tm, int& tn) {
        const int l = q_base + q;
        const int a = l / sub_n;
        tm = tm_base + a; tn = tn_base + (l - a * sub_n);
    };
    int q_cur, q_step, q_end;
    {
        const int j = blockIdx.x >> 3;
        if (p.reserved4_ & 2) {
            q_cur = (int)((int64_t)q_cnt * j / J);
            q_end = (int)((int64_t)q_cnt * (j + 1) / J);
            q_step = 1;
        } else {
            q_cur = j; q_end = q_cnt; q_step = J;
        }
    }
    if (q_cur >= q_end) return;
    const int nk = p.K / 32;

    const int lrow = lane >> 2, pch = lane & 3;
    const int lch = pch ^ ((0x78 >> (2 * ((lrow >> 2) & 3))) & 3);
    const __amdgpu_buffer_rsrc_t rsrc_a = __builtin_amdgcn_make_buffer_rsrc(const_cast<void*>(p.a), 0, OOB_OFF, 0x00020000);
    const __amdgpu_buffer_rsrc_t rsrc_w = __builtin_amdgcn_make_buffer_rsrc(const_cast<void*>(p.w), 0, OOB_OFF, 0x00020000);
    unsigned a_off[2], w_off[2];
    int d_q = q_cur, d_k = 0;
    auto set_dma_tile = [&](int q) {
        int tm, tn;
        tile_of(q, tm, tn);
        const bool any = q < q_end;
#pragma unroll
        for (int g = 0; g < 2; ++g) {
            const int row = tm * TM + (g * 8 + wave) * 16 + lrow;
            a_off[g] = (any && row < p.M) ? (unsigned)(((int64_t)row * p.lda + lch * 8) * 2) : OOB_OFF;
            w_off[g] = any ? (unsigned)(((int64_t)(tn * BN + sqp_perm((g * 8 + wave) * 16 + lrow)) * p.ldw + lch * 8) * 2) : OOB_OFF;
        }
    };
    auto issue_pair = [&](int slot_even, int slot_odd) {
        const unsigned soff = (unsigned)(d_k * KS * 2);
        const lds_ptr se = (lds_ptr)smem + slot_even * STAGE, so = (lds_ptr)smem + slot_odd * STAGE;
#pragma unroll
        for (int g = 0; g < 2; ++g) {
            __builtin_amdgcn_raw_ptr_buffer_load_lds(rsrc_a, se + (g * 8 + wave) * 1024, 16, a_off[g], soff, 0, 0);
            __builtin_amdgcn_raw_ptr_buffer_load_lds(rsrc_a, so + (g * 8 + wave) * 1024, 16, a_off[g], soff + KS * 2, 0, 0);
        }
#pragma unroll
        for (int g = 0; g < 2; ++g) {
            __builtin_amdgcn_raw_ptr_buffer_load_lds(rsrc_w, se + A_BYTES + (g * 8 + wave) * 1024, 16, w_off[g], soff, 0, 0);
            __builtin_amdgcn_raw_ptr_buffer_load_lds(rsrc_w, so + A_BYTES + (g * 8 + wave) * 1024, 16, w_off[g], soff + KS * 2, 0, 0);
        }
        d_k += 2;
        if (d_k >= nk) { d_k = 0; d_q += q_step; set_dma_tile(d_q); }
    };

    const int fr = lane & 15, fg = lane >> 4;
    const int swz = (fg ^ ((0x78 >> (2 * ((fr >> 2) & 3))) & 3)) << 4;
    const int a_off0 = (wave_m * WTM + fr) * RB + swz;
    const int b_off0 = A_BYTES + (wave_n * WTN + fr) * RB + swz;
    f32x4 acc[MT][NT];
    half8v af[2][MT], bf[2][NT];
    auto read_tile = [&](auto set_tag, int slot) {
        constexpr int S = decltype(set_tag)::value;
        const char* cur = smem + slot * STAGE;
#pragma unroll
        for (int r = 0; r < NT; ++r) bf[S][r] = *reinterpret_cast<const half8v*>(cur + b_off0 + r * 1024);
#pragma unroll
        for (int r = 0; r < MT; ++r) af[S][r] = *reinterpret_cast<const half8v*>(cur + a_off0 + r * 1024);
    };

    auto tid_now = [&]() -> int {
        int l;
        asm volatile("v_mbcnt_lo_u32_b32 %0, -1, 0\n\tv_mbcnt_hi_u32_b32 %0, -1, %0" : "=v"(l));
        return wave * 64 + l;
    };
    const bool fold = (p.flags & MOCA_EP_LNFOLD) != 0;
    const float* const dummy = reinterpret_cast<const float*>(p.w);
    constexpr unsigned STAT_SCRATCH = 8192;
    const int stat_floats = 2 + 2 * (fold ? p.lnf_nparts : 0);
    auto stat_dma = [&](int q, unsigned slot_off) {
        int tm, tn;
        tile_of(q < q_end ? q : 0, tm, tn);
        const int t = tid_now();
        const int n = tn * BN + sqp_perm(t);
        const int m = min(tm * TM + t, p.M - 1);
        const lds_ptr area = (lds_ptr)smem + slot_off + STAT_SCRATCH + wave * (22 * 256);
        __builtin_amdgcn_global_load_lds((glb_ptr)(fold ? p.lnf_wsum + n : dummy), area, 4, 0, 0);
        __builtin_amdgcn_global_load_lds((glb_ptr)(p.bias ? p.bias + n : dummy), area + 256, 4, 0, 0);
        if (fold) {
            for (int i = 0; i < p.lnf_nparts; ++i) {
                const float* src = p.lnf_part + ((int64_t)i * p.M + m) * 2;
                __builtin_amdgcn_global_load_lds((glb_ptr)src, area + (2 + 2 * i) * 256, 4, 0, 0);
                __builtin_amdgcn_global_load_lds((glb_ptr)(src + 1), area + (3 + 2 * i) * 256, 4, 0, 0);
            }
        }
    };
    auto stat_read = [&](unsigned slot_off, auto after_tag) -> LnFoldRegs {
        constexpr int after = decltype(after_tag)::value;
        asm volatile("s_waitcnt vmcnt(%0)" ::"n"(after) : "memory");
        __builtin_amdgcn_sched_barrier(0);
        int lane_;
        asm volatile("v_mbcnt_lo_u32_b32 %0, -1, 0\n\tv_mbcnt_hi_u32_b32 %0, -1, %0" : "=v"(lane_));
        const unsigned area = (unsigned)(size_t)((lds_ptr)smem + slot_off + STAT_SCRATCH + wave * (22 * 256)) + 4 * lane_;
        const float ws = lds_rd_f1(area), b = lds_rd_f1(area + 256);
        float s = 0.f, qq = 0.f;
        LnFoldRegs f = {1.f, 0.f, 0.f, 0.f};
        if (fold) {
            for (int i = 0; i < p.lnf_nparts; ++i) {
                const float x = lds_rd_f1(area + (2 + 2 * i) * 256), y = lds_rd_f1(area + (3 + 2 * i) * 256);
                lds_wait();
                s += x; qq += y;
            }
        }
        lds_wait();
        f.ws = fold ? ws : 0.f;
        f.b = p.bias ? b : 0.f;
        if (fold) {
            const float inv_k = 1.0f / (float)p.K;
            const float mean = s * inv_k;
            const float var = fmaxf(qq * inv_k - mean * mean, 0.f);
            f.rs = rsqrtf(var + p.ln_eps);
            f.rb = -mean * f.rs;
        }
        return f;
    };
    (void)stat_floats;

    LnFoldRegs lf = {1.f, 0.f, 0.f, 0.f};
    if (!late) {
        stat_dma(q_cur, (NS - 1) * STAGE);
        lf = stat_read((NS - 1) * STAGE, int_c<0>{});
    }
    __builtin_amdgcn_s_barrier();
    set_dma_tile(q_cur);
    issue_pair(0, 1);
    issue_pair(2, 3);
    asm volatile("s_waitcnt vmcnt(%0)" ::"n"(2 * PPW) : "memory");
    __builtin_amdgcn_s_barrier();
    if (late) __builtin_amdgcn_s_barrier();

    const bool nt_out = out_streams(p);
    const half_t* __restrict__ resid = reinterpret_cast<const half_t*>(p.residual);
    const half_t* __restrict__ rowadd = reinterpret_cast<const half_t*>(p.rowadd);
    int s0 = 0;
#ifdef MOCA_STAMPS
    int tile_no = 0;
#endif
    while (true) {
        int tm, tn;
        tile_of(q_cur, tm, tn);
        const int m0 = tm * TM, n0 = tn * BN;
#ifdef MOCA_STAMPS
        const bool stamp_it = tile_no == 3;
        if (stamp_it) { MOCA_STAMP(0); }
#endif
#pragma unroll
        for (int mt = 0; mt < MT; ++mt)
#pragma unroll
            for (int nt = 0; nt < NT; ++nt) acc[mt][nt] = f32x4{0.f, 0.f, 0.f, 0.f};
        for (int i = 0; i < nk; i += 2) {
            const int s1 = s0 + 1 == NS ? 0 : s0 + 1;
            const int sp = s0 == 0 ? NS - 1 : s0 - 1;
#ifdef MOCA_STAMPS
            const bool seg = stamp_it && i == SEG_ITER;
            if (seg) MOCA_STAMP_W(8, SEG_WAVE);
#endif
            read_tile(int_c<0>{}, s0);
            asm volatile("s_waitcnt lgkmcnt(0)" ::: "memory");
            __builtin_amdgcn_sched_barrier(0);
#ifdef MOCA_STAMPS
            if (seg) MOCA_STAMP_W(9, SEG_WAVE);
#endif
            __builtin_amdgcn_s_barrier();
#ifdef MOCA_STAMPS
            if (seg) MOCA_STAMP_W(10, SEG_WAVE);
#endif
            {
                const char* nx = smem + s1 * STAGE;
                __builtin_amdgcn_s_setprio(1);
#pragma unroll
                for (int j = 0; j < MT * NT; ++j) {
                    const int mt = j / NT, nt = j % NT;
                    acc[mt][nt] = __builtin_amdgcn_mfma_f32_16x16x32_f16(bf[0][nt], af[0][mt], acc[mt][nt], 0, 0, 0);
                    if (j % 2 == 0 && j / 2 < MT + NT) {
                        const int r = j / 2;
                        __builtin_amdgcn_sched_barrier(0);
                        if (r < NT) bf[1][r] = *reinterpret_cast<const half8v*>(nx + b_off0 + r * 1024);
                        else af[1][r - NT] = *reinterpret_cast<const half8v*>(nx + a_off0 + (r - NT) * 1024);
                        __builtin_amdgcn_sched_barrier(0);
                    }
                }
                __builtin_amdgcn_s_setprio(0);
            }
            asm volatile("s_waitcnt lgkmcnt(0)" ::: "memory");
            __builtin_amdgcn_sched_barrier(0);
#ifdef MOCA_STAMPS
            if (seg) MOCA_STAMP_W(11, SEG_WAVE);
#endif
            __builtin_amdgcn_s_barrier();
#ifdef MOCA_STAMPS
            if (seg) MOCA_STAMP_W(12, SEG_WAVE);
#endif
            issue_pair(sp, s0);
#ifdef MOCA_STAMPS
            if (seg) MOCA_STAMP_W(13, SEG_WAVE);
#endif
            asm volatile("s_waitcnt vmcnt(%0)" ::"n"(2 * PPW) : "memory");
            __builtin_amdgcn_sched_barrier(0);
#ifdef MOCA_STAMPS
            if (seg) MOCA_STAMP_W(14, SEG_WAVE);
#endif
            __builtin_amdgcn_s_barrier();
#ifdef MOCA_STAMPS
            if (seg) MOCA_STAMP_W(15, SEG_WAVE);
#endif
            __builtin_amdgcn_s_setprio(1);
#pragma unroll
            for (int mt = 0; mt < MT; ++mt)
#pragma unroll
                for (int nt = 0; nt < NT; ++nt)
                    acc[mt][nt] = __builtin_amdgcn_mfma_f32_16x16x32_f16(bf[1][nt], af[1][mt], acc[mt][nt], 0, 0, 0);
            __builtin_amdgcn_s_setprio(0);
            __builtin_amdgcn_sched_barrier(0);
#ifdef MOCA_STAMPS
            if (seg) MOCA_STAMP_W(1, SEG_WAVE);
#endif
            __builtin_amdgcn_s_barrier();
#ifdef MOCA_STAMPS
            if (seg) MOCA_STAMP_W(2, SEG_WAVE);
#endif
            s0 = s1 + 1 == NS ? 0 : s1 + 1;
        }
#ifdef MOCA_STAMPS
        if (stamp_it) MOCA_STAMP(3);
#endif
        if (!late) __builtin_amdgcn_s_barrier();
        const unsigned lst = (unsigned)(size_t)((lds_ptr)smem + (s0 == 0 ? NS - 1 : s0 - 1) * STAGE);
        const unsigned lws = lst + 8 * TM, lbi = lws + 4 * BN;
        if (!late) {
            const int t = tid_now();
            lds_wr_f2(lst + 8 * t, f32x2{lf.rs, lf.rb});
            lds_wr_f1(lws + 4 * t, lf.ws);
            lds_wr_f1(lbi + 4 * t, lf.b);
        }
        lds_wait();
        __builtin_amdgcn_s_barrier();
#ifdef MOCA_STAMPS
        if (stamp_it) MOCA_STAMP(4);
#endif
        f32x2 st[MT];
#pragma unroll
        for (int mt = 0; mt < MT; ++mt) st[mt] = lds_rd_f2(lst + 8 * (wave_m * WTM + mt * 16 + fr));
        const int q_next = q_cur + q_step;
        const unsigned stat_slot = (unsigned)((s0 == 0 ? NS - 1 : s0 - 1) * STAGE);
        if (!late) stat_dma(q_next, stat_slot);
#pragma unroll
        for (int grp = 0; grp < 2; ++grp) {
            f32x4 cw[4], cb[4];
#pragma unroll
            for (int t = 0; t < 4; ++t) {
                cw[t] = lds_rd_f4(lws + 4 * (wave_n * WTN + (grp * 4 + t) * 16 + 4 * fg));
                cb[t] = lds_rd_f4(lbi + 4 * (wave_n * WTN + (grp * 4 + t) * 16 + 4 * fg));
            }
            lds_wait();
#pragma unroll
            for (int mt = 0; mt < MT; ++mt) {
                const int m = m0 + wave_m * WTM + mt * 16 + fr;
                f32x4 v[4];
#pragma unroll
                for (int t = 0; t < 4; ++t) v[t] = st[mt][0] * acc[mt][grp * 4 + t] + (st[mt][1] * cw[t] + cb[t]);
                if constexpr (GEGLU) {
                    half8v h;
#pragma unroll
                    for (int nv = 0; nv < 2; ++nv) {
                        const f32x4 r4 = moca_geglu4(v[nv], v[nv + 2]);
                        h[4 * nv + 0] = (half_t)r4[0]; h[4 * nv + 1] = (half_t)r4[1]; h[4 * nv + 2] = (half_t)r4[2]; h[4 * nv + 3] = (half_t)r4[3];
                    }
                    if (m < p.M) st_out8(reinterpret_cast<half_t*>(p.out) + (int64_t)m * p.ldo + (n0 >> 1) + wave_n * 64 + grp * 32 + 8 * fg, h, nt_out);
                } else {
#pragma unroll
                    for (int hh = 0; hh < 2; ++hh) {
                        const int col = n0 + wave_n * WTN + grp * 64 + hh * 32 + 8 * fg;
                        float o[8];
#pragma unroll
                        for (int r = 0; r < 4; ++r) { o[r] = v[2 * hh][r]; o[4 + r] = v[2 * hh + 1][r]; }
                        if (m < p.M) {
                            if (rowadd) {
                                const half8v e = *reinterpret_cast<const half8v*>(rowadd + (int64_t)(m / p.rowadd_div) * p.ld_rowadd + col);
#pragma unroll
                                for (int r = 0; r < 8; ++r) o[r] = (float)(half_t)o[r] + (float)e[r];
                            }
                            if (resid) {
                                const half8v e = *reinterpret_cast<const half8v*>(resid + (int64_t)m * p.ldr + col);
#pragma unroll
                                for (int r = 0; r < 8; ++r) o[r] = (rowadd ? o[r] : (float)(half_t)o[r]) + (float)e[r];
                            }
                            half8v h;
#pragma unroll
                            for (int r = 0; r < 8; ++r) h[r] = (half_t)o[r];
                            st_out8(reinterpret_cast<half_t*>(p.out) + (int64_t)m * p.ldo + col, h, nt_out);
                        }
                    }
                }
            }
        }
#ifdef MOCA_STAMPS
        if (stamp_it) { MOCA_STAMP(5); MOCA_STAMP_HW(); }
        ++tile_no;
#endif
        if (!late) {
            if (m0 + TM > p.M) lf = stat_read(stat_slot, int_c<0>{});
            else lf = stat_read(stat_slot, int_c<(GEGLU ? 8 : 16)>{});
        }
        if (q_next >= q_end) break;
        q_cur = q_next;
        if (late) __builtin_amdgcn_s_barrier();
    }
    asm volatile("s_waitcnt vmcnt(0) lgkmcnt(0)" ::: "memory");
#endif
}

template <bool GEGLU>
int launch_gemm_g4p(const moca_gemm_params& p, hipStream_t st) {
    constexpr int lds = 3 * (256 + 128) * 64 + (2 * 256 + 2 * 128) * 4;
    if (!dyn_lds_once<&gemm_g4p_kernel<GEGLU>>(lds)) return MOCA_E_LAUNCH;
    moca_gemm_params pl = p;
    pl.reserved2_ = G4P_BLOCKS;
    if (moca_tuning_get(MOCA_TUNE_GEMM_MF32)) {
        if (!dyn_lds_once<&gemm_g4q_kernel<GEGLU>>(lds)) return MOCA_E_LAUNCH;
        hipLaunchKernelGGL((gemm_g4q_kernel<GEGLU>), dim3(G4P_BLOCKS + 2 * prefetch_blocks(pl)), dim3(256), lds, st, pl);
    } else {
        hipLaunchKernelGGL((gemm_g4p_kernel<GEGLU>), dim3(G4P_BLOCKS + 2 * prefetch_blocks(pl)), dim3(256), lds, st, pl);
    }
    MOCA_CHECK_LAUNCH();
    return MOCA_OK;
}

template <bool GEGLU>
int launch_gemm_sqp(const moca_gemm_params& p, hipStream_t st) {
    constexpr int lds = 5 * (256 + 256) * 64;
    if (!dyn_lds_once<&gemm_sqp_kernel<GEGLU>>(lds)) return MOCA_E_LAUNCH;
    moca_gemm_params pl = p;
    pl.reserved2_ = SQP_BLOCKS;
    pl.reserved4_ = (pl.reserved4_ & 0xfd) | (choose_xcd_n(p, (p.M + 255) / 256, p.N / 256, 256) << 8) |
                    (moca_tuning_get(MOCA_TUNE_SQP_WALK) ? 2 : 0);
    hipLaunchKernelGGL((gemm_sqp_kernel<GEGLU>), dim3(SQP_BLOCKS + prefetch_blocks(pl)), dim3(512), lds, st, pl);
    MOCA_CHECK_LAUNCH();
    return MOCA_OK;
}

}

int moca_gemm_g4p_launch(const moca_gemm_params& p, hipStream_t st) {
    return (p.flags & MOCA_EP_GEGLU) ? launch_gemm_g4p<true>(p, st) : launch_gemm_g4p<false>(p, st);
}
int moca_gemm_sqp_launch(const moca_gemm_params& p, hipStream_t st) {
    return (p.flags & MOCA_EP_GEGLU) ? launch_gemm_sqp<true>(p, st) : launch_gemm_sqp<false>(p, st);
}
```

moca_video_amd/csrc/gemm_tiled.hip:

```cpp
#include "gemm_launch.h"

namespace {

constexpr int ZERO_PAGE_HALVES = 8192 + 64;
__device__ __attribute__((aligned(16))) half_t g_zero_page[ZERO_PAGE_HALVES];

template <int AMODE, bool FAST, int NAP, int KS>
struct AGather {
    const moca_gemm_params& p;
    const half_t* Aptr;
    const half_t* zero;
    int lch;
    int64_t row_off[NAP];
    int row_y[NAP], row_x[NAP];
    bool row_ok[NAP];
    const half_t* a_base[NAP];
    int tap_cur = -1, a_koff = 0, tiles_per_tap;

    __device__ __forceinline__ AGather(const moca_gemm_params& p_, int lch_)
        : p(p_), Aptr(reinterpret_cast<const half_t*>(p_.a)), zero(g_zero_page), lch(lch_),
          tiles_per_tap((AMODE == MOCA_A_LINEAR || !FAST) ? (1 << 30) : p_.C / KS) {}

    __device__ __forceinline__ void init_row(int g, int m) {
        row_ok[g] = m < p.M;
// ... 350 lines not shown
        if constexpr (NT == 4) {
#pragma unroll
            for (int nt = 0; nt < 2; ++nt) {
                const int ncol = n0 + wave_n * 64 + nt * 16 + 4 * fg;
                f32x4 bv = {0.f, 0.f, 0.f, 0.f}, bg = {0.f, 0.f, 0.f, 0.f};
                if (p.bias) { bv = *reinterpret_cast<const f32x4*>(p.bias + ncol); bg = *reinterpret_cast<const f32x4*>(p.bias + ncol + 32); }
#pragma unroll
                for (int mt = 0; mt < 4; ++mt) {
                    const int row = wave_m * 64 + mt * 16 + fr;
                    const f32x4 va = acc[mt][nt] + bv, ga = acc[mt][nt + 2] + bg;
                    const f32x2 lo = moca_geglu2(f32x2{va[0], va[1]}, f32x2{ga[0], ga[1]});
                    const f32x2 hi = moca_geglu2(f32x2{va[2], va[3]}, f32x2{ga[2], ga[3]});
                    half4v h;
                    h[0] = (half_t)lo[0]; h[1] = (half_t)lo[1]; h[2] = (half_t)hi[0]; h[3] = (half_t)hi[1];
                    *reinterpret_cast<half4v*>(smem + row * pitch + (wave_n * 32 + nt * 16 + 4 * fg) * 2) = h;
                }
            }
        }
    } else {
        const bool fold = (p.flags & MOCA_EP_LNFOLD) != 0;
        float* rst = reinterpret_cast<float*>(smem + TM * (BN * 2 + 16));
        if (fold) lnfold_publish<TM, BN>(lf, rst, tid);
#pragma unroll
        for (int nt = 0; nt < NT; ++nt) {
            const int col = wave_n * (BN / 2) + nt * 16 + 4 * fg;
            f32x4 bv, ws4 = {0.f, 0.f, 0.f, 0.f};
            if (fold) { ws4 = *reinterpret_cast<const f32x4*>(rst + 2 * TM + col); bv = *reinterpret_cast<const f32x4*>(rst + 2 * TM + BN + col); }
            else bv = ld4_or_zero(p.bias, n0 + col);
#pragma unroll
            for (int mt = 0; mt < 4; ++mt) {
                const int row = wave_m * 64 + mt * 16 + fr;
                f32x4 v;
                if (fold) v = lnfold_apply(acc[mt][nt], *reinterpret_cast<const float2*>(rst + 2 * row), ws4, bv);
                else v = acc[mt][nt] + bv;
                *reinterpret_cast<half4v*>(smem + row * pitch + col * 2) = __builtin_convertvector(v, half4v);
            }
        }
    }
    __syncthreads();
    MOCA_STAMP(4);

    if (p.flags & (MOCA_EP_COLSUM | MOCA_EP_GSTAT)) store_fp16_tile_colsum<TM, BN>(p, smem, reinterpret_cast<float*>(smem + TM * (BN * 2 + 16)), pitch, m0, n0, tile_m, tid);
    else if (p.flags & MOCA_EP_ROWSUM) store_fp16_tile_rowsum<512, BN, 4>(p, smem, pitch, TM, m0, n0, tid);
    else store_fp16_tile<512>(p, smem, pitch, TM, out_bn, m0, on0, tid);
    MOCA_STAMP(5);
    MOCA_STAMP_HW();
}

template <int AMODE, bool FAST>
__global__ __launch_bounds__(256, 2) void gemm_g4_kernel(const moca_gemm_params p) {
    constexpr int TM = 256, BN = 128, KS = 32;
    constexpr int RB = KS * 2;
    constexpr int MT = 8, NT = 4;
    constexpr int A_BYTES = TM * RB;
    constexpr int B_BYTES = BN * RB;
    constexpr int STAGE = A_BYTES + B_BYTES;
    constexpr int NMMA = MT * NT;

    extern __shared__ __attribute__((aligned(16))) char smem[];
    MOCA_STAMP(0);

    const int tid = threadIdx.x, lane = tid & 63;
    const int wave = __builtin_amdgcn_readfirstlane(tid >> 6);
    const int wave_m = wave >> 1, wave_n = wave & 1;

    const int tiles_m = (p.M + TM - 1) / TM;
    const int tiles_n = p.N / BN;
    const int nblk = tiles_m * tiles_n * p.splits;
    if (prefetch_block(p, nblk, 256)) return;
    int split = 0, tile_m, tile_n;
    if ((p.reserved4_ >> 8) > 1) {
        remap_tile_2d(tiles_m, tiles_n, p.reserved4_ >> 8, tile_m, tile_n);
    } else {
        int logical;
        remap_block<BN>(nblk, logical);
        split = logical % p.splits;
        const int tile = logical / p.splits;
        tile_m = tile / tiles_n; tile_n = tile % tiles_n;
    }
    const int m0 = tile_m * TM, n0 = tile_n * BN;

    const int nk_total = 2 * ((p.K + 63) / 64);
    const int kts = 2 * (((p.K + 63) / 64 + p.splits - 1) / p.splits);
    const int kt_begin = split * kts;
    const int nk = min(kt_begin + kts, nk_total) - kt_begin;

    const half_t* __restrict__ Wptr = reinterpret_cast<const half_t*>(p.w);

    const int lrow = lane >> 2, pch = lane & 3;
    const int lch = pch ^ ((0x78 >> (2 * ((lrow >> 2) & 3))) & 3);
    AGather<AMODE, FAST, 4, KS> ga(p, lch);
#pragma unroll
    for (int g = 0; g < 4; ++g) ga.init_row(g, m0 + (g * 4 + wave) * 16 + lrow);
    const half_t* w_row[2];
#pragma unroll
    for (int g = 0; g < 2; ++g) {
        const int n = n0 + (g * 4 + wave) * 16 + lrow;
        w_row[g] = Wptr + (int64_t)n * p.ldw + lch * 8;
    }

    auto dma_piece = [&](int kt, int slot, int j, int odd) {
        const lds_ptr sa = (lds_ptr)smem + slot * STAGE;
        if (j < 4) {
            __builtin_amdgcn_global_load_lds((glb_ptr)ga.src(kt, j, odd), sa + (j * 4 + wave) * 1024, 16, 0, 0);
        } else {
            const int g = j - 4;
            __builtin_amdgcn_global_load_lds((glb_ptr)(w_row[g] + kt * KS), sa + A_BYTES + (g * 4 + wave) * 1024, 16, 0, 0);
        }
    };
    auto issue_pair = [&](int kt_even, int slot_even, int slot_odd) {
        ga.begin_tile(kt_even);
#pragma unroll
        for (int j = 0; j < 6; ++j) {
            dma_piece(kt_even, slot_even, j, 0);
            dma_piece(kt_even + 1, slot_odd, j, 1);
        }
    };

    f32x4 acc[MT][NT];
#pragma unroll
    for (int mt = 0; mt < MT; ++mt)
#pragma unroll
        for (int nt = 0; nt < NT; ++nt) acc[mt][nt] = f32x4{0.f, 0.f, 0.f, 0.f};

    const int fr = lane & 15, fg = lane >> 4;
    int a_off[MT], b_off[NT];
#pragma unroll
    for (int mt = 0; mt < MT; ++mt) {
        const int row = wave_m * 128 + mt * 16 + fr;
        a_off[mt] = row * RB + ((fg ^ ((0x78 >> (2 * ((row >> 2) & 3))) & 3)) << 4);
    }
#pragma unroll
    for (int nt = 0; nt < NT; ++nt) {
        const int row = wave_n * 64 + nt * 16 + fr;
        b_off[nt] = A_BYTES + row * RB + ((fg ^ ((0x78 >> (2 * ((row >> 2) & 3))) & 3)) << 4);
    }

    half8v af[MT], bf[NT];
    int s0 = 0, s1 = 1, s2 = 2;
    const int kt_last_pair = kt_begin + nk - 2;
    auto phase = [&](auto even_tag, int i) {
        constexpr bool even = decltype(even_tag)::value;
        const char* cur = smem + s0 * STAGE;
        const int kt2 = min(kt_begin + i + 2, kt_last_pair);
        if constexpr (even) ga.begin_tile(kt2);
#pragma unroll
        for (int mt = 0; mt < MT; ++mt) af[mt] = *reinterpret_cast<const half8v*>(cur + a_off[mt]);
#pragma unroll
        for (int nt = 0; nt < NT; ++nt) bf[nt] = *reinterpret_cast<const half8v*>(cur + b_off[nt]);
        if constexpr (even) {
            asm volatile("s_waitcnt lgkmcnt(0)" ::: "memory");
            __builtin_amdgcn_s_barrier();
        }
        __builtin_amdgcn_s_setprio(1);
#pragma unroll
        for (int j = 0; j < NMMA; ++j) {
            const int mt = j / NT, nt = j % NT;
            acc[mt][nt] = __builtin_amdgcn_mfma_f32_16x16x32_f16(bf[nt], af[mt], acc[mt][nt], 0, 0, 0);
            if constexpr (even) {
                if (j % 5 == 2 && j / 5 < 6) {
                    dma_piece(kt2, s2, j / 5, 0);
                    dma_piece(kt2 + 1, s0, j / 5, 1);
                    __builtin_amdgcn_sched_barrier(0);
                }
            }
        }
        __builtin_amdgcn_s_setprio(0);
        { const int t = s0; s0 = s1; s1 = s2; s2 = t; }
    };

    LnFoldRaw lraw = {float2{0.f, 0.f}, float2{0.f, 0.f}, 0.f, 0.f};
    if (p.flags & MOCA_EP_LNFOLD) lraw = lnfold_issue<TM, BN>(p, m0 + tid, n0, tid);
    issue_pair(kt_begin, 0, 1);
    LnFoldRegs lf = {0.f, 0.f, 0.f, 0.f};
    if (p.flags & MOCA_EP_LNFOLD) lf = lnfold_finish<TM, BN>(p, lraw, m0 + tid, tid);
    MOCA_STAMP(1);
    asm volatile("s_waitcnt vmcnt(0)" ::: "memory");
    __builtin_amdgcn_s_barrier();
    MOCA_STAMP(2);
    for (int i = 0; i < nk; i += 2) {
        phase(yes_t{}, i);
        asm volatile("s_waitcnt lgkmcnt(0)" ::: "memory");
        __builtin_amdgcn_s_barrier();
        phase(no_t{}, i + 1);
        asm volatile("s_waitcnt vmcnt(0) lgkmcnt(0)" ::: "memory");
        __builtin_amdgcn_s_barrier();
    }
    MOCA_STAMP(3);

    if (p.splits > 1) {
        float* ws = p.splitk_ws + (int64_t)split * p.M * p.N;
#pragma unroll
        for (int mt = 0; mt < MT; ++mt) {
            const int row = m0 + wave_m * 128 + mt * 16 + fr;
            if (row < p.M) {
#pragma unroll
                for (int nt = 0; nt < NT; ++nt) {
                    const int col = n0 + wave_n * 64 + nt * 16 + 4 * fg;
                    *reinterpret_cast<f32x4*>(ws + (int64_t)row * p.N + col) = acc[mt][nt];
                }
            }
        }
        return;
    }
    const bool geglu = (p.flags & MOCA_EP_GEGLU) != 0;
    const int out_bn = geglu ? BN / 2 : BN;
    const int on0 = geglu ? n0 / 2 : n0;
    const int pitch = out_bn * 2 + 16;
    const bool fold = (p.flags & MOCA_EP_LNFOLD) != 0;
    float* rst = reinterpret_cast<float*>(smem + TM * (BN * 2 + 16));
    if (fold) lnfold_publish<TM, BN>(lf, rst, tid);
    if (geglu) {
#pragma unroll
        for (int nt = 0; nt < 2; ++nt) {
            const int lcol = wave_n * 64 + nt * 16 + 4 * fg, ncol = n0 + lcol;
            f32x4 bv, bg, wv = {0.f, 0.f, 0.f, 0.f}, wg = wv;
            if (fold) {
                wv = *reinterpret_cast<const f32x4*>(rst + 2 * TM + lcol); wg = *reinterpret_cast<const f32x4*>(rst + 2 * TM + lcol + 32);
                bv = *reinterpret_cast<const f32x4*>(rst + 2 * TM + BN + lcol); bg = *reinterpret_cast<const f32x4*>(rst + 2 * TM + BN + lcol + 32);
            } else {
                bv = ld4_or_zero(p.bias, ncol); bg = ld4_or_zero(p.bias, ncol + 32);
            }
#pragma unroll
            for (int mt = 0; mt < MT; ++mt) {
                const int row = wave_m * 128 + mt * 16 + fr;
                f32x4 va, ga;
                if (fold) {
                    const float2 st = *reinterpret_cast<const float2*>(rst + 2 * row);
                    va = lnfold_apply(acc[mt][nt], st, wv, bv); ga = lnfold_apply(acc[mt][nt + 2], st, wg, bg);
                } else {
                    va = acc[mt][nt] + bv; ga = acc[mt][nt + 2] + bg;
                }
                const f32x2 lo = moca_geglu2(f32x2{va[0], va[1]}, f32x2{ga[0], ga[1]});
                const f32x2 hi = moca_geglu2(f32x2{va[2], va[3]}, f32x2{ga[2], ga[3]});
                half4v h;
                h[0] = (half_t)lo[0]; h[1] = (half_t)lo[1]; h[2] = (half_t)hi[0]; h[3] = (half_t)hi[1];
                *reinterpret_cast<half4v*>(smem + row * pitch + (wave_n * 32 + nt * 16 + 4 * fg) * 2) = h;
            }
        }
    } else {
#pragma unroll
        for (int nt = 0; nt < NT; ++nt) {
            const int col = wave_n * 64 + nt * 16 + 4 * fg;
            f32x4 bv, ws4 = {0.f, 0.f, 0.f, 0.f};
            if (fold) { ws4 = *reinterpret_cast<const f32x4*>(rst + 2 * TM + col); bv = *reinterpret_cast<const f32x4*>(rst + 2 * TM + BN + col); }
            else bv = ld4_or_zero(p.bias, n0 + col);
#pragma unroll
            for (int mt = 0; mt < MT; ++mt) {
                const int row = wave_m * 128 + mt * 16 + fr;
                f32x4 v;
                if (fold) v = lnfold_apply(acc[mt][nt], *reinterpret_cast<const float2*>(rst + 2 * row), ws4, bv);
                else v = acc[mt][nt] + bv;
                *reinterpret_cast<half4v*>(smem + row * pitch + col * 2) = __builtin_convertvector(v, half4v);
            }
        }
    }
    __syncthreads();
    MOCA_STAMP(4);
    store_fp16_tile<256>(p, smem, pitch, TM, out_bn, m0, on0, tid);
    MOCA_STAMP(5);
    MOCA_STAMP_HW();
}


typedef short tq_short4v __attribute__((ext_vector_type(4)));
typedef __attribute__((address_space(3))) tq_short4v* tq_lds_s4_ptr;
__device__ __forceinline__ half4v tattn_tr_read(const char* addr) {
#if defined(__HIP_DEVICE_COMPILE__)
    const tq_short4v v = __builtin_amdgcn_ds_read_tr16_b64_v4i16((tq_lds_s4_ptr)addr);
    return __builtin_bit_cast(half4v, v);
#else
    return half4v{0, 0, 0, 0};
#endif
}
#if defined(__HIP_DEVICE_COMPILE__)
#define MOCA_XLANE(NAME, SWAP, OP)                                                                         \
    __device__ __forceinline__ float NAME(float x) {                                                       \
        const auto r = SWAP(__float_as_uint(x), __float_as_uint(x), false, false);                         \
        const float a = __uint_as_float(r[0]), b = __uint_as_float(r[1]);                                  \
        return OP;                                                                                         \
    }
MOCA_XLANE(xlane16_max, __builtin_amdgcn_permlane16_swap, fmaxf(a, b))
MOCA_XLANE(xlane32_max, __builtin_amdgcn_permlane32_swap, fmaxf(a, b))
MOCA_XLANE(xlane16_sum, __builtin_amdgcn_permlane16_swap, a + b)
MOCA_XLANE(xlane32_sum, __builtin_amdgcn_permlane32_swap, a + b)
#undef MOCA_XLANE
#else
__device__ __forceinline__ float xlane16_max(float x) { return x; }
__device__ __forceinline__ float xlane32_max(float x) { return x; }
__device__ __forceinline__ float xlane16_sum(float x) { return x; }
__device__ __forceinline__ float xlane32_sum(float x) { return x; }
#endif

#define MOCA_W80S_NAME gemm_w80s_kernel
#define MOCA_W80S_CAUSAL false
#include "gemm_w80s_kernel.inc"
#undef MOCA_W80S_NAME
#undef MOCA_W80S_CAUSAL
#define MOCA_W80S_NAME gemm_w80s_causal_kernel
#define MOCA_W80S_CAUSAL true
#include "gemm_w80s_kernel.inc"
#undef MOCA_W80S_NAME
#undef MOCA_W80S_CAUSAL

template <int AMODE, int SHAPE, bool CAUSAL = false>
int launch_gemm_w80s(const moca_gemm_params& p, hipStream_t st) {
    constexpr auto kernel = [] {
        if constexpr (CAUSAL) return &gemm_w80s_causal_kernel<AMODE, SHAPE>;
        else return &gemm_w80s_kernel<AMODE, SHAPE>;
    }();
    constexpr int TM = SHAPE == 2 ? 256 : (SHAPE == 1 ? 160 : 320), BN = SHAPE == 2 ? 256 : (SHAPE == 1 ? 320 : (SHAPE == 3 ? 192 : 160));
    const int tiles_m = (p.M + TM - 1) / TM, tiles_n = p.N / BN;
    const int nblk = tiles_m * tiles_n * p.splits;
    moca_gemm_params pl = p;
    pl.reserved4_ = (pl.reserved4_ & 0xff) | ((SHAPE == 3 ? 1 : choose_xcd_n(p, tiles_m, tiles_n, BN)) << 8);
    constexpr int lds = 5 * (TM + BN) * 64;
    if (!dyn_lds_once<kernel>(lds)) return MOCA_E_LAUNCH;
    hipLaunchKernelGGL(kernel, dim3(nblk + prefetch_blocks(pl)), dim3(512), lds, st, pl);
    MOCA_CHECK_LAUNCH();
    return MOCA_OK;
}

template <int BN, int AMODE, bool FAST>
int launch_gemm_glds(const moca_gemm_params& p, hipStream_t st) {
    const int tiles_m = (p.M + 255) / 256, tiles_n = p.N / BN;
    const int nblk = tiles_m * tiles_n * p.splits;
    constexpr int lds_pipe = 3 * (256 + BN) * ROW_BYTES;
    constexpr int lds_epi = 256 * BN * 4;
    constexpr int lds = lds_pipe > lds_epi ? lds_pipe : lds_epi;
    if (!dyn_lds_once<&gemm_glds_kernel<BN, AMODE, FAST>>(lds)) return MOCA_E_LAUNCH;
    hipLaunchKernelGGL((gemm_glds_kernel<BN, AMODE, FAST>), dim3(nblk + prefetch_blocks(p)), dim3(512), lds, st, p);
    MOCA_CHECK_LAUNCH();
    return MOCA_OK;
}

template <int AMODE, bool FAST>
int launch_gemm_g4(const moca_gemm_params& p, hipStream_t st) {
    const int tiles_m = (p.M + 255) / 256, tiles_n = p.N / 128;
    const int nblk = tiles_m * tiles_n * p.splits;
    constexpr int lds = 3 * (256 + 128) * 64;
    if (!dyn_lds_once<&gemm_g4_kernel<AMODE, FAST>>(lds)) return MOCA_E_LAUNCH;
    moca_gemm_params pl = p;
    pl.reserved4_ = (pl.reserved4_ & 0xff) | (choose_xcd_n(p, tiles_m, tiles_n, 128) << 8);
    hipLaunchKernelGGL((gemm_g4_kernel<AMODE, FAST>), dim3(nblk + 2 * prefetch_blocks(pl)), dim3(256), lds, st, pl);
    MOCA_CHECK_LAUNCH();
    return MOCA_OK;
}

}

int moca_gemm_glds_launch(int bn, const moca_gemm_params& p, hipStream_t st) {
    if (bn == 128) return with_gather(p, [&](auto am, auto fast) { return launch_gemm_glds<128, decltype(am)::value, decltype(fast)::value>(p, st); });
    return with_gather(p, [&](auto am, auto fast) { return launch_gemm_glds<160, decltype(am)::value, decltype(fast)::value>(p, st); });
}
int moca_gemm_g4_launch(const moca_gemm_params& p, hipStream_t st) {
    return with_gather(p, [&](auto am, auto fast) { return launch_gemm_g4<decltype(am)::value, decltype(fast)::value>(p, st); });
}

int moca_gemm_w80s_launch(int shape, const moca_gemm_params& p, hipStream_t st) {
    switch (shape) {
        case 0:
            if (p.a2) return launch_gemm_w80s<MOCA_A_LINEAR2, 0>(p, st);
            return with_gather(p, [&](auto am, auto) { return launch_gemm_w80s<decltype(am)::value, 0>(p, st); });
        case 1:
            if (p.a2) return launch_gemm_w80s<MOCA_A_LINEAR2, 1>(p, st);
            return with_gather(p, [&](auto am, auto) { return launch_gemm_w80s<decltype(am)::value, 1>(p, st); });
        case 2: return launch_gemm_w80s<MOCA_A_LINEAR, 2>(p, st);
        case 3: return p.tattn_causal ? launch_gemm_w80s<MOCA_A_LINEAR, 3, true>(p, st) : launch_gemm_w80s<MOCA_A_LINEAR, 3>(p, st);
    }
    return MOCA_E_BADARG;
}
```

moca_video_amd/csrc/gemm_w80s_kernel.inc:

```
template <int AMODE, int SHAPE>
__global__ __launch_bounds__(512, 2) void MOCA_W80S_NAME(const moca_gemm_params p) {
#if defined(__HIP_DEVICE_COMPILE__)
    constexpr bool CAUSAL = MOCA_W80S_CAUSAL;
    static_assert(!CAUSAL || SHAPE == 3, "the causal mask belongs to the MOCA_EP_TATTN epilogue");
    constexpr bool WIDE = SHAPE == 1, SQ = SHAPE == 2, TQ = SHAPE == 3;
    constexpr int MT = SQ ? 4 : 5, NT = SQ ? 8 : (TQ ? 6 : 5), KS = 32, RB = 64;
    constexpr int WTM = 16 * MT, WTN = 16 * NT;
    constexpr int TM = SQ ? 256 : (WIDE ? 160 : 320), BN = SQ ? 256 : (WIDE ? 320 : (TQ ? 192 : 160));
    constexpr int A_BYTES = TM * RB, STAGE = A_BYTES + BN * RB;
    constexpr int NS = 5;
    constexpr int PPW = 4;
    constexpr int NAP = SQ ? 2 : (WIDE ? 2 : 3);

    extern __shared__ __attribute__((aligned(16))) char smem[];
    MOCA_STAMP(0);

    const int tid = threadIdx.x, lane = tid & 63;
    const int wave = __builtin_amdgcn_readfirstlane(tid >> 6);
    const int wave_m = WIDE ? wave >> 2 : wave >> 1, wave_n = WIDE ? wave & 3 : wave & 1;
    const bool late = wave >= 4;

    const int tiles_m = (p.M + TM - 1) / TM;
    const int tiles_n = p.N / BN;
    const int nblk = tiles_m * tiles_n * p.splits;
    if (prefetch_block(p, nblk, 512)) return;
    int split = 0, tile_m, tile_n;
    const int xcd_n = p.reserved4_ >> 8;
    if (xcd_n > 1) {
        remap_tile_2d(tiles_m, tiles_n, xcd_n, tile_m, tile_n);
    } else {
        int logical;
        remap_block<BN>(nblk, logical);
        split = logical % p.splits;
        const int tile = logical / p.splits;
        tile_m = tile / tiles_n; tile_n = tile % tiles_n;
    }
    const int m0 = tile_m * TM, n0 = tile_n * BN;

    const int nk_total = 2 * ((p.K + 63) / 64);
    const int kts = 2 * (((p.K + 63) / 64 + p.splits - 1) / p.splits);
    const int kt_begin = split * kts;
    const int nk = min(kt_begin + kts, nk_total) - kt_begin;

    const int lrow = lane >> 2, pch = lane & 3;
    const int lch = pch ^ ((0x78 >> (2 * ((lrow >> 2) & 3))) & 3);
    const bool flex_is_big = wave < 4;
    const int kt_last_pair = kt_begin + nk - 2;
    BGather<AMODE, NAP, KS> ga(p, lch, kt_begin, kt_last_pair);
    const int small1 = TQ ? 4 + wave : (wave < 6 ? 4 + wave : 2 + wave);
    const int tq_tpv = TQ ? p.HW / 20 : 1;
    const int tq_b = tile_m / tq_tpv, tq_pb = tile_m - tq_b * tq_tpv;
    auto grow = [&](int tr) -> int { return TQ ? (tq_b * 16 + (tr & 15)) * p.HW + tq_pb * 20 + (tr >> 4) : m0 + tr; };
    const int wg = (AMODE == MOCA_A_LINEAR && p.wgroup_rows > 0) ? m0 / p.wgroup_rows : 0;
    const unsigned wgo = (unsigned)((int64_t)wg * p.wgroup_stride * 2);
    unsigned w_off[3];
    if constexpr (SQ) {
        ga.init_row(0, m0 + wave * 16 + lrow);
        ga.init_row(1, m0 + (8 + wave) * 16 + lrow);
        w_off[0] = (unsigned)(((int64_t)(n0 + wave * 16 + lrow) * p.ldw + lch * 8) * 2);
        w_off[1] = (unsigned)(((int64_t)(n0 + (8 + wave) * 16 + lrow) * p.ldw + lch * 8) * 2);
        w_off[2] = 0;
    } else if constexpr (!WIDE) {
#pragma unroll
        for (int g = 0; g < NAP; ++g) ga.init_row(g, grow((g < 2 ? g * 8 + wave : 16 + (wave & 3)) * 16 + lrow));
        w_off[0] = (unsigned)(((int64_t)(n0 + (wave & 3) * 16 + lrow) * p.ldw + lch * 8) * 2);
        w_off[1] = (unsigned)(((int64_t)(n0 + small1 * 16 + lrow) * p.ldw + lch * 8) * 2);
        w_off[2] = 0;
    } else {
        ga.init_row(0, m0 + (wave & 3) * 16 + lrow);
        ga.init_row(1, m0 + small1 * 16 + lrow);
        w_off[0] = (unsigned)(((int64_t)(n0 + wave * 16 + lrow) * p.ldw + lch * 8) * 2);
        w_off[1] = (unsigned)(((int64_t)(n0 + (8 + wave) * 16 + lrow) * p.ldw + lch * 8) * 2);
        w_off[2] = (unsigned)(((int64_t)(n0 + (16 + (wave & 3)) * 16 + lrow) * p.ldw + lch * 8) * 2);
    }
    if (wgo) { w_off[0] += wgo; w_off[1] += wgo; w_off[2] += wgo; }
    __amdgpu_buffer_rsrc_t rsrc_a = __builtin_amdgcn_make_buffer_rsrc(const_cast<void*>(p.a), 0, OOB_OFF, 0x00020000);
    const __amdgpu_buffer_rsrc_t rsrc_w = __builtin_amdgcn_make_buffer_rsrc(const_cast<void*>(p.w), 0, OOB_OFF, 0x00020000);
    __amdgpu_buffer_rsrc_t rsrc_f = (flex_is_big != WIDE) ? rsrc_a : rsrc_w;
    auto sync_src = [&]() {
        if constexpr (AMODE == MOCA_A_LINEAR2) {
            if (ga.tap == 1) {
                rsrc_a = __builtin_amdgcn_make_buffer_rsrc(const_cast<void*>(p.a2), 0, OOB_OFF, 0x00020000);
                if (flex_is_big != WIDE) rsrc_f = rsrc_a;
            }
        }
    };

    auto dma_piece = [&](int slot, int j, auto odd_tag) {
        constexpr int odd = decltype(odd_tag)::value;
        const lds_ptr sa = (lds_ptr)smem + slot * STAGE;
        const unsigned a_s = ga.a_soff() + odd * KS * 2, w_s = ga.w_soff() + odd * KS * 2;
        if constexpr (SQ) {
            if (j < 2) __builtin_amdgcn_raw_ptr_buffer_load_lds(rsrc_a, sa + (j * 8 + wave) * 1024, 16, ga.a_off[j], a_s, 0, 0);
            else __builtin_amdgcn_raw_ptr_buffer_load_lds(rsrc_w, sa + A_BYTES + ((j - 2) * 8 + wave) * 1024, 16, w_off[j - 2], w_s, 0, 0);
        } else if constexpr (!WIDE) {
            if (j < 2) {
                __builtin_amdgcn_raw_ptr_buffer_load_lds(rsrc_a, sa + (j * 8 + wave) * 1024, 16, ga.a_off[j], a_s, 0, 0);
            } else if (j == 2) {
                const lds_ptr dst = flex_is_big ? sa + (16 + (wave & 3)) * 1024 : sa + A_BYTES + (wave & 3) * 1024;
                __builtin_amdgcn_raw_ptr_buffer_load_lds(rsrc_f, dst, 16, flex_is_big ? ga.a_off[2] : w_off[0], flex_is_big ? a_s : w_s, 0, 0);
            } else {
                __builtin_amdgcn_raw_ptr_buffer_load_lds(rsrc_w, sa + A_BYTES + small1 * 1024, 16, w_off[1], w_s, 0, 0);
            }
        } else {
            if (j < 2) {
                __builtin_amdgcn_raw_ptr_buffer_load_lds(rsrc_w, sa + A_BYTES + (j * 8 + wave) * 1024, 16, w_off[j], w_s, 0, 0);
            } else if (j == 2) {
                const lds_ptr dst = flex_is_big ? sa + A_BYTES + (16 + (wave & 3)) * 1024 : sa + (wave & 3) * 1024;
                __builtin_amdgcn_raw_ptr_buffer_load_lds(rsrc_f, dst, 16, flex_is_big ? w_off[2] : ga.a_off[0], flex_is_big ? w_s : a_s, 0, 0);
            } else {
                __builtin_amdgcn_raw_ptr_buffer_load_lds(rsrc_a, sa + small1 * 1024, 16, ga.a_off[1], a_s, 0, 0);
            }
        }
    };
    auto issue_pair = [&](int slot_even, int slot_odd) {
#pragma unroll
        for (int j = 0; j < PPW; ++j) {
            dma_piece(slot_even, j, int_c<0>{});
            dma_piece(slot_odd, j, int_c<1>{});
        }
    };

    const int fr = lane & 15, fg = lane >> 4;
    f32x4 acc[MT][NT];
#pragma unroll
    for (int nt = 0; nt < NT; ++nt) {
        f32x4 bv = {0.f, 0.f, 0.f, 0.f};
        if (p.bias && p.splits == 1 && !(p.flags & MOCA_EP_LNFOLD)) bv = *reinterpret_cast<const f32x4*>(p.bias + (int64_t)wg * p.N + n0 + wave_n * WTN + nt * 16 + 4 * fg);
#pragma unroll
        for (int mt = 0; mt < MT; ++mt) acc[mt][nt] = bv;
    }

    const int swz = (fg ^ ((0x78 >> (2 * ((fr >> 2) & 3))) & 3)) << 4;
    const int a_off0 = (wave_m * WTM + fr) * RB + swz;
    const int b_off0 = A_BYTES + (wave_n * WTN + fr) * RB + swz;

    half8v af[2][MT], bf[2][NT];
    auto read_tile = [&](auto set_tag, int slot) {
        constexpr int S = decltype(set_tag)::value;
        const char* cur = smem + slot * STAGE;
#pragma unroll
        for (int r = 0; r < NT; ++r) bf[S][r] = *reinterpret_cast<const half8v*>(cur + b_off0 + r * 1024);
#pragma unroll
        for (int r = 0; r < MT; ++r) af[S][r] = *reinterpret_cast<const half8v*>(cur + a_off0 + r * 1024);
    };
    auto mfma_tile = [&](auto set_tag) {
        constexpr int S = decltype(set_tag)::value;
        __builtin_amdgcn_s_setprio(1);
#pragma unroll
        for (int mt = 0; mt < MT; ++mt)
#pragma unroll
            for (int nt = 0; nt < NT; ++nt)
                acc[mt][nt] = __builtin_amdgcn_mfma_f32_16x16x32_f16(bf[S][nt], af[S][mt], acc[mt][nt], 0, 0, 0);
        __builtin_amdgcn_s_setprio(0);
    };

    LnFoldRaw lraw = {float2{0.f, 0.f}, float2{0.f, 0.f}, 0.f, 0.f};
    if (p.flags & MOCA_EP_LNFOLD) lraw = lnfold_issue<TM, BN>(p, grow(tid), n0, tid);
    ga.seek(kt_begin);
    sync_src();
    issue_pair(0, 1);
    ga.advance();
    sync_src();
    issue_pair(2, 3);
    LnFoldRegs lf = {0.f, 0.f, 0.f, 0.f};
    if (p.flags & MOCA_EP_LNFOLD) lf = lnfold_finish<TM, BN>(p, lraw, grow(tid), tid);
    MOCA_STAMP(1);
    asm volatile("s_waitcnt vmcnt(%0)" ::"n"(2 * PPW) : "memory");
    __builtin_amdgcn_s_barrier();
    MOCA_STAMP(2);
    if (late) __builtin_amdgcn_s_barrier();

    int s0 = 0;
    for (int i = 0; i < nk; i += 2) {
        const int s1 = s0 + 1 == NS ? 0 : s0 + 1;
        const int sp = s0 == 0 ? NS - 1 : s0 - 1;
#if defined(W80S_VARIANT) && W80S_VARIANT == 0
        read_tile(int_c<0>{}, s0);
        read_tile(int_c<1>{}, s1);
        asm volatile("s_waitcnt lgkmcnt(0)" ::: "memory");
        __builtin_amdgcn_sched_barrier(0);
        __builtin_amdgcn_s_barrier();
        mfma_tile(int_c<0>{});
        __builtin_amdgcn_sched_barrier(0);
        __builtin_amdgcn_s_barrier();
#else
#if defined(W80S_GN_DIAG)
        if constexpr (AMODE != MOCA_A_LINEAR && !SQ && !TQ) {
#pragma unroll
            for (int t = 0; t < 2; ++t) {
                char* base = smem + (t == 0 ? s0 : s1) * STAGE;
                for (int c = tid; c < A_BYTES / 16; c += 512) {
                    half8v v = *reinterpret_cast<half8v*>(base + c * 16);
#pragma unroll
                    for (int j = 0; j < 8; ++j) v[j] = (half_t)moca_silu((float)v[j] * 1.0009765625f + 0.0009765625f);
                    *reinterpret_cast<half8v*>(base + c * 16) = v;
                }
            }
            asm volatile("s_waitcnt lgkmcnt(0)" ::: "memory");
            __builtin_amdgcn_s_barrier();
        }
#endif
#ifdef MOCA_STAMPS
#ifndef SEG_WAVE
#define SEG_WAVE 0
#endif
#ifndef SEG_ITER
#define SEG_ITER 2
#endif
        const bool seg = i == SEG_ITER;
        if (seg) MOCA_STAMP_W(8, SEG_WAVE);
#endif
        read_tile(int_c<0>{}, s0);
        asm volatile("s_waitcnt lgkmcnt(0)" ::: "memory");
        __builtin_amdgcn_sched_barrier(0);
#ifdef MOCA_STAMPS
        if (seg) MOCA_STAMP_W(9, SEG_WAVE);
#endif
        __builtin_amdgcn_s_barrier();
#ifdef MOCA_STAMPS
        if (seg) MOCA_STAMP_W(10, SEG_WAVE);
#endif
        {
            const char* nx = smem + s1 * STAGE;
            __builtin_amdgcn_s_setprio(1);
#pragma unroll
            for (int j = 0; j < MT * NT; ++j) {
                const int mt = j / NT, nt = j % NT;
                acc[mt][nt] = __builtin_amdgcn_mfma_f32_16x16x32_f16(bf[0][nt], af[0][mt], acc[mt][nt], 0, 0, 0);
                if (j % 2 == 0 && j / 2 < MT + NT) {
                    const int r = j / 2;
                    __builtin_amdgcn_sched_barrier(0);
                    if (r < NT) bf[1][r] = *reinterpret_cast<const half8v*>(nx + b_off0 + r * 1024);
                    else af[1][r - NT] = *reinterpret_cast<const half8v*>(nx + a_off0 + (r - NT) * 1024);
                    __builtin_amdgcn_sched_barrier(0);
                }
            }
            __builtin_amdgcn_s_setprio(0);
        }
        asm volatile("s_waitcnt lgkmcnt(0)" ::: "memory");
        __builtin_amdgcn_sched_barrier(0);
#ifdef MOCA_STAMPS
        if (seg) MOCA_STAMP_W(11, SEG_WAVE);
#endif
        __builtin_amdgcn_s_barrier();
#ifdef MOCA_STAMPS
        if (seg) MOCA_STAMP_W(12, SEG_WAVE);
#endif
#endif
        ga.advance();
        sync_src();
        issue_pair(sp, s0);
#ifdef MOCA_STAMPS
        if (seg) MOCA_STAMP_W(13, SEG_WAVE);
#endif
        asm volatile("s_waitcnt vmcnt(%0)" ::"n"(2 * PPW) : "memory");
        __builtin_amdgcn_sched_barrier(0);
#ifdef MOCA_STAMPS
        if (seg) MOCA_STAMP_W(14, SEG_WAVE);
#endif
        __builtin_amdgcn_s_barrier();
#ifdef MOCA_STAMPS
        if (seg) MOCA_STAMP_W(15, SEG_WAVE);
#endif
        mfma_tile(int_c<1>{});
        __builtin_amdgcn_sched_barrier(0);
        __builtin_amdgcn_s_barrier();
        s0 = s1 + 1 == NS ? 0 : s1 + 1;
    }
    if (!late) __builtin_amdgcn_s_barrier();
    asm volatile("s_waitcnt vmcnt(0) lgkmcnt(0)" ::: "memory");
    __builtin_amdgcn_s_barrier();
    MOCA_STAMP(3);

    if (p.splits > 1) {
        float* ws = p.splitk_ws + (int64_t)split * p.M * p.N;
#pragma unroll
        for (int mt = 0; mt < MT; ++mt) {
            const int row = m0 + wave_m * WTM + mt * 16 + fr;
            if (row < p.M) {
#pragma unroll
                for (int nt = 0; nt < NT; ++nt) {
                    const int col = n0 + wave_n * WTN + nt * 16 + 4 * fg;
                    *reinterpret_cast<f32x4*>(ws + (int64_t)row * p.N + col) = acc[mt][nt];
                }
            }
        }
        return;
    }
    const bool fold = (p.flags & MOCA_EP_LNFOLD) != 0;
    if constexpr (SQ) {
        if (p.flags & MOCA_EP_GEGLU) {
            constexpr int gpitch = (BN / 2) * 2 + 16;
            float* rst = reinterpret_cast<float*>(smem + TM * gpitch);
            if (fold) lnfold_publish<TM, BN>(lf, rst, tid);
#pragma unroll
            for (int grp = 0; grp < 2; ++grp)
#pragma unroll
                for (int nt = 0; nt < 2; ++nt) {
                    const int lcol = wave_n * WTN + grp * 64 + nt * 16 + 4 * fg;
                    f32x4 wv = {0.f, 0.f, 0.f, 0.f}, wg = wv, bv = wv, bg = wv;
                    if (fold) {
                        wv = *reinterpret_cast<const f32x4*>(rst + 2 * TM + lcol); wg = *reinterpret_cast<const f32x4*>(rst + 2 * TM + lcol + 32);
                        bv = *reinterpret_cast<const f32x4*>(rst + 2 * TM + BN + lcol); bg = *reinterpret_cast<const f32x4*>(rst + 2 * TM + BN + lcol + 32);
                    }
#pragma unroll
                    for (int mt = 0; mt < MT; ++mt) {
                        const int row = wave_m * WTM + mt * 16 + fr;
                        f32x4 va = acc[mt][4 * grp + nt], gt = acc[mt][4 * grp + nt + 2];
                        if (fold) {
                            const float2 st = *reinterpret_cast<const float2*>(rst + 2 * row);
                            va = lnfold_apply(va, st, wv, bv); gt = lnfold_apply(gt, st, wg, bg);
                        }
                        const f32x2 lo = moca_geglu2(f32x2{va[0], va[1]}, f32x2{gt[0], gt[1]});
                        const f32x2 hi = moca_geglu2(f32x2{va[2], va[3]}, f32x2{gt[2], gt[3]});
                        half4v h;
                        h[0] = (half_t)lo[0]; h[1] = (half_t)lo[1]; h[2] = (half_t)hi[0]; h[3] = (half_t)hi[1];
                        *reinterpret_cast<half4v*>(smem + row * gpitch + (wave_n * 64 + grp * 32 + nt * 16 + 4 * fg) * 2) = h;
                    }
                }
            __syncthreads();
            MOCA_STAMP(4);
            store_fp16_tile<512>(p, smem, gpitch, TM, BN / 2, m0, n0 / 2, tid);
            MOCA_STAMP(5);
            MOCA_STAMP_HW();
            return;
        }
    }
    constexpr int pitch = BN * 2 + 16;
    if (fold) {
        float* rst = reinterpret_cast<float*>(smem + TM * pitch);
        lnfold_publish<TM, BN>(lf, rst, tid);
#pragma unroll
        for (int nt = 0; nt < NT; ++nt) {
            const int col = wave_n * WTN + nt * 16 + 4 * fg;
            const f32x4 ws4 = *reinterpret_cast<const f32x4*>(rst + 2 * TM + col);
            const f32x4 b4 = *reinterpret_cast<const f32x4*>(rst + 2 * TM + BN + col);
#pragma unroll
            for (int mt = 0; mt < MT; ++mt) {
                const int row = wave_m * WTM + mt * 16 + fr;
                const float2 st = *reinterpret_cast<const float2*>(rst + 2 * row);
                *reinterpret_cast<half4v*>(smem + row * pitch + col * 2) = __builtin_convertvector(lnfold_apply(acc[mt][nt], st, ws4, b4), half4v);
            }
        }
    } else {
#pragma unroll
        for (int nt = 0; nt < NT; ++nt) {
            const int col = wave_n * WTN + nt * 16 + 4 * fg;
#pragma unroll
            for (int mt = 0; mt < MT; ++mt) {
                const int row = wave_m * WTM + mt * 16 + fr;
                *reinterpret_cast<half4v*>(smem + row * pitch + col * 2) = __builtin_convertvector(acc[mt][nt], half4v);
            }
        }
    }
    __syncthreads();
    MOCA_STAMP(4);
    if constexpr (TQ) {
        const float sl2e = p.tattn_scale * 1.4426950408889634f;
        half_t* outp = reinterpret_cast<half_t*>(p.out);
        constexpr int NPX = 3;
        int pixs[NPX];
        half8v kf[NPX][2], qf[NPX][2];
#pragma unroll
        for (int i = 0; i < NPX; ++i) {
            pixs[i] = min(wave + 8 * i, 19);
            const char* base = smem + (pixs[i] * 16) * pitch;
#pragma unroll
            for (int ks = 0; ks < 2; ++ks) {
                qf[i][ks] = *reinterpret_cast<const half8v*>(base + fr * pitch + (ks * 32 + fg * 8) * 2);
                kf[i][ks] = *reinterpret_cast<const half8v*>(base + fr * pitch + (64 + ks * 32 + fg * 8) * 2);
            }
        }
        half4v vfr[NPX][4];
#pragma unroll
        for (int i = 0; i < NPX; ++i) {
            const char* base = smem + (pixs[i] * 16) * pitch;
#pragma unroll
            for (int dt = 0; dt < 4; ++dt)
                vfr[i][dt] = tattn_tr_read(base + (4 * fg + (fr >> 2)) * pitch + (128 + dt * 16 + 4 * (fr & 3)) * 2);
        }
        f32x4 sc[NPX];
#pragma unroll
        for (int i = 0; i < NPX; ++i) {
            sc[i] = f32x4{0.f, 0.f, 0.f, 0.f};
            sc[i] = __builtin_amdgcn_mfma_f32_16x16x32_f16(kf[i][0], qf[i][0], sc[i], 0, 0, 0);
            sc[i] = __builtin_amdgcn_mfma_f32_16x16x32_f16(kf[i][1], qf[i][1], sc[i], 0, 0, 0);
        }
        if constexpr (CAUSAL) {
#pragma unroll
            for (int i = 0; i < NPX; ++i)
#pragma unroll
                for (int r = 0; r < 4; ++r)
                    if (4 * fg + r > fr) sc[i][r] = -INFINITY;
        }
        half4v pf[NPX];
        float inv[NPX];
#pragma unroll
        for (int i = 0; i < NPX; ++i) {
            float mx = fmaxf(fmaxf(sc[i][0], sc[i][1]), fmaxf(sc[i][2], sc[i][3]));
            mx = xlane16_max(mx);
            mx = xlane32_max(mx);
            float sum = 0.f;
#pragma unroll
            for (int r = 0; r < 4; ++r) {
                const float pv = exp2f((sc[i][r] - mx) * sl2e);
                sum += pv;
                pf[i][r] = (half_t)pv;
            }
            sum = xlane16_sum(sum);
            sum = xlane32_sum(sum);
            inv[i] = 1.0f / sum;
        }
#pragma unroll
        for (int i = 0; i < NPX; ++i) {
            half_t* ob = outp + (int64_t)grow(pixs[i] * 16 + fr) * p.ldo + tile_n * 64;
            const bool live = wave + 8 * i < 20;
#pragma unroll
            for (int dt = 0; dt < 4; ++dt) {
                f32x4 o4 = {0.f, 0.f, 0.f, 0.f};
                o4 = __builtin_amdgcn_mfma_f32_16x16x16f16(vfr[i][dt], pf[i], o4, 0, 0, 0);
                half4v h4;
#pragma unroll
                for (int r = 0; r < 4; ++r) h4[r] = (half_t)(o4[r] * inv[i]);
                if (live) *reinterpret_cast<half4v*>(ob + dt * 16 + 4 * fg) = h4;
            }
        }
    } else if constexpr (SQ) {
        store_fp16_tile<512>(p, smem, pitch, TM, BN, m0, n0, tid);
    } else if constexpr (WIDE) {
        if (p.flags & MOCA_EP_LN) store_fp16_tile_ln(p, smem, reinterpret_cast<float*>(smem + TM * pitch), pitch, m0, tid);
        else if (p.flags & (MOCA_EP_COLSUM | MOCA_EP_GSTAT)) store_fp16_tile_colsum<TM, BN>(p, smem, reinterpret_cast<float*>(smem + TM * pitch), pitch, m0, n0, tile_m, tid);
        else if (p.flags & MOCA_EP_ROWSUM) store_fp16_tile_rowsum<512, BN, 8>(p, smem, pitch, TM, m0, n0, tid);
        else store_fp16_tile<512>(p, smem, pitch, TM, BN, m0, n0, tid);
    } else {
        if (p.flags & (MOCA_EP_COLSUM | MOCA_EP_GSTAT)) store_fp16_tile_colsum<TM, BN>(p, smem, reinterpret_cast<float*>(smem + TM * pitch), pitch, m0, n0, tile_m, tid);
        else if (p.flags & MOCA_EP_ROWSUM) store_fp16_tile_rowsum<512, BN, 4>(p, smem, pitch, TM, m0, n0, tid);
        else store_fp16_tile<512>(p, smem, pitch, TM, BN, m0, n0, tid);
    }
    MOCA_STAMP(5);
    MOCA_STAMP_HW();
#endif
}
```

moca_video_amd/csrc/runtime.hip:

```cpp
#include "common.h"
#include <string.h>
#include <stdio.h>
#include <stdlib.h>

extern "C" int moca_graph_begin(void* stream) {
    if (hipStreamBeginCapture(moca_stream(stream), hipStreamCaptureModeThreadLocal) != hipSuccess) return MOCA_E_GRAPH;
    return MOCA_OK;
}

extern "C" int moca_graph_end(void* stream, void** graph_exec_out) {
    if (!graph_exec_out) return MOCA_E_BADARG;
    hipGraph_t g = nullptr;
    if (hipStreamEndCapture(moca_stream(stream), &g) != hipSuccess || !g) return MOCA_E_GRAPH;
    hipGraphExec_t ge = nullptr;
    hipError_t e = hipGraphInstantiate(&ge, g, nullptr, nullptr, 0);
    (void)hipGraphDestroy(g);
    if (e != hipSuccess || !ge) return MOCA_E_GRAPH;
    *graph_exec_out = reinterpret_cast<void*>(ge);
    return MOCA_OK;
}

extern "C" int moca_graph_launch(void* graph_exec, void* stream) {
    if (!graph_exec) return MOCA_E_BADARG;
    if (hipGraphLaunch(reinterpret_cast<hipGraphExec_t>(graph_exec), moca_stream(stream)) != hipSuccess) return MOCA_E_GRAPH;
    return MOCA_OK;
}

extern "C" int moca_graph_destroy(void* graph_exec) {
    if (!graph_exec) return MOCA_OK;
    return hipGraphExecDestroy(reinterpret_cast<hipGraphExec_t>(graph_exec)) == hipSuccess ? MOCA_OK : MOCA_E_GRAPH;
}

extern "C" int moca_stream_create(void** stream_out) {
    if (!stream_out) return MOCA_E_BADARG;
    hipStream_t s;
    if (hipStreamCreateWithFlags(&s, hipStreamNonBlocking) != hipSuccess) return MOCA_E_LAUNCH;
    *stream_out = reinterpret_cast<void*>(s);
    return MOCA_OK;
}
extern "C" int moca_stream_destroy(void* stream) {
    return hipStreamDestroy(moca_stream(stream)) == hipSuccess ? MOCA_OK : MOCA_E_LAUNCH;
}
extern "C" int moca_stream_sync(void* stream) {
    return hipStreamSynchronize(moca_stream(stream)) == hipSuccess ? MOCA_OK : MOCA_E_LAUNCH;
}

extern "C" int moca_event_create(void** ev_out) {
    if (!ev_out) return MOCA_E_BADARG;
    hipEvent_t e;
    if (hipEventCreate(&e) != hipSuccess) return MOCA_E_LAUNCH;
    *ev_out = reinterpret_cast<void*>(e);
    return MOCA_OK;
}
extern "C" int moca_event_record(void* ev, void* stream) {
    return hipEventRecord(reinterpret_cast<hipEvent_t>(ev), moca_stream(stream)) == hipSuccess ? MOCA_OK : MOCA_E_LAUNCH;
}
extern "C" int moca_event_elapsed_ms(void* ev_start, void* ev_stop, float* ms_out) {
    if (!ms_out) return MOCA_E_BADARG;
    if (hipEventSynchronize(reinterpret_cast<hipEvent_t>(ev_stop)) != hipSuccess) return MOCA_E_LAUNCH;
    return hipEventElapsedTime(ms_out, reinterpret_cast<hipEvent_t>(ev_start), reinterpret_cast<hipEvent_t>(ev_stop)) == hipSuccess
               ? MOCA_OK : MOCA_E_LAUNCH;
}
extern "C" int moca_event_destroy(void* ev) {
    return hipEventDestroy(reinterpret_cast<hipEvent_t>(ev)) == hipSuccess ? MOCA_OK : MOCA_E_LAUNCH;
}

extern "C" int moca_device_info(char* name, int32_t len, int32_t* cu_count) {
    int n = 0;
    if (hipGetDeviceCount(&n) != hipSuccess || n <= 0) return MOCA_E_NODEVICE;
    int dev = 0;
    if (hipGetDevice(&dev) != hipSuccess) return MOCA_E_NODEVICE;
    hipDeviceProp_t prop;
    if (hipGetDeviceProperties(&prop, dev) != hipSuccess) return MOCA_E_NODEVICE;
    if (name && len > 0) {
        strncpy(name, prop.gcnArchName, (size_t)len - 1);
        name[len - 1] = 0;
    }
    if (cu_count) *cu_count = prop.multiProcessorCount;
    return MOCA_OK;
}

__global__ __launch_bounds__(256) void zero_kernel(uint4* __restrict__ p, int64_t n16, unsigned char* __restrict__ tail, int ntail) {
    for (int64_t i = (int64_t)blockIdx.x * 256 + threadIdx.x; i < n16; i += (int64_t)gridDim.x * 256) p[i] = uint4{0u, 0u, 0u, 0u};
    if (blockIdx.x == 0 && (int)threadIdx.x < ntail) tail[threadIdx.x] = 0;
}

extern "C" int moca_memset_zero(void* ptr, int64_t bytes, void* stream) {
    if (!ptr || bytes < 0 || (reinterpret_cast<uintptr_t>(ptr) & 15)) return MOCA_E_BADARG;
    if (bytes == 0) return MOCA_OK;
    const int64_t n16 = bytes / 16;
    int blocks = (int)((n16 + 255) / 256);
    if (blocks < 1) blocks = 1;
    if (blocks > 1024) blocks = 1024;
    hipLaunchKernelGGL(zero_kernel, dim3(blocks), dim3(256), 0, moca_stream(stream), reinterpret_cast<uint4*>(ptr), n16,
                       reinterpret_cast<unsigned char*>(ptr) + n16 * 16, (int)(bytes - n16 * 16));
    MOCA_CHECK_LAUNCH();
    return MOCA_OK;
}

__global__ __launch_bounds__(64) void clock_sampler_kernel(unsigned long long* __restrict__ buf, int nsamples, const volatile int* stop) {
#if defined(__HIP_DEVICE_COMPILE__)
    if (threadIdx.x) return;
    unsigned long long* b = buf + (size_t)blockIdx.x * nsamples * 2;
    for (int i = 0; i < nsamples; ++i) {
        unsigned long long t, r;
        asm volatile("s_memtime %0\n\ts_memrealtime %1\n\ts_waitcnt lgkmcnt(0)" : "=s"(t), "=s"(r)::"memory");
        b[2 * i] = t;
        b[2 * i + 1] = r;
        if (stop && *stop) break;
        __builtin_amdgcn_s_sleep(127);
        __builtin_amdgcn_s_sleep(127);
    }
#endif
}
extern "C" int moca_debug_clock_sampler(void* buf, int32_t blocks, int32_t nsamples, const int32_t* stop, void* stream) {
    if (!buf || blocks < 1 || blocks > 64 || nsamples < 1 || nsamples > (1 << 20)) return MOCA_E_BADARG;
    hipLaunchKernelGGL(clock_sampler_kernel, dim3(blocks), dim3(64), 0, moca_stream(stream), reinterpret_cast<unsigned long long*>(buf), nsamples,
                       reinterpret_cast<const volatile int*>(stop));
    MOCA_CHECK_LAUNCH();
    return MOCA_OK;
}

static int g_tuning[MOCA_TUNE_COUNT] = {1, 1, 1, 1, 1, 1, 0, 1, 0, 0, 1};
int moca_tuning_get(int knob) { return (knob >= 0 && knob < MOCA_TUNE_COUNT) ? g_tuning[knob] : 0; }
extern "C" int moca_set_tuning(int32_t knob, int32_t value) {
    if (knob < 0 || knob >= MOCA_TUNE_COUNT || value < 0 || value > 2) return MOCA_E_BADARG;
    const int old = g_tuning[knob];
    g_tuning[knob] = value;
    return old;
}
```

moca_video_amd/lib.py:

```python
from __future__ import annotations

import ctypes as C
import os

import torch

_HERE = os.path.dirname(os.path.abspath(__file__))
LIB_PATH = os.environ.get("MOCA_HIP_LIB") or os.path.join(_HERE, "libmoca_hip.so")

MOCA_A_LINEAR, MOCA_A_CONV3X3, MOCA_A_TCONV3 = 0, 1, 2
MOCA_EP_GEGLU, MOCA_EP_OUT_F32, MOCA_FORCE_SMALL_TILE, MOCA_EP_GELU, MOCA_EP_COLSUM, MOCA_EP_LN = 1, 2, 4, 8, 16, 32
MOCA_EP_ROWSUM, MOCA_EP_LNFOLD, MOCA_EP_GSTAT, MOCA_EP_TATTN, MOCA_EP_SLABS = 64, 128, 256, 512, 1024
MOCA_TUNE_GEMM_W80, MOCA_TUNE_GEMM_G4, MOCA_TUNE_GEMM_SQ256, MOCA_TUNE_GEMM_WIDE, MOCA_TUNE_GN_SLAB, MOCA_TUNE_GEMM_G4P, MOCA_TUNE_GEMM_MF32, MOCA_TUNE_GEMM_SQP, MOCA_TUNE_SQP_WALK = 0, 1, 2, 3, 4, 5, 6, 7, 8
MOCA_TUNE_SLAB_F16 = 9
MOCA_TUNE_GEMM_WS = 10
(MOCA_ROUTE_SMALL64, MOCA_ROUTE_SMALL128, MOCA_ROUTE_GLDS128, MOCA_ROUTE_GLDS160, MOCA_ROUTE_G4, MOCA_ROUTE_W80, MOCA_ROUTE_W80W,
 MOCA_ROUTE_SQ256, MOCA_ROUTE_G4P, MOCA_ROUTE_SQP, MOCA_ROUTE_TATTN, MOCA_ROUTE_WS) = range(1, 13)

_ERR = {0: "ok", -1: "bad argument (shape/alignment contract)", -2: "HIP launch/runtime error",
        -3: "no gfx950 device", -4: "graph capture/replay failed"}


class MocaHipError(RuntimeError):
    pass


class GemmParams(C.Structure):
    _fields_ = [
        ("a", C.c_void_p), ("w", C.c_void_p), ("out", C.c_void_p), ("bias", C.c_void_p),
        ("rowadd", C.c_void_p), ("residual", C.c_void_p), ("splitk_ws", C.c_void_p),
        ("M", C.c_int32), ("N", C.c_int32), ("K", C.c_int32),
        ("lda", C.c_int32), ("ldw", C.c_int32), ("ldo", C.c_int32), ("ldr", C.c_int32), ("ld_rowadd", C.c_int32),
        ("rowadd_div", C.c_int32), ("a_mode", C.c_int32), ("C", C.c_int32),
        ("inH", C.c_int32), ("inW", C.c_int32), ("outH", C.c_int32), ("outW", C.c_int32),
        ("stride", C.c_int32), ("up", C.c_int32), ("T", C.c_int32), ("HW", C.c_int32),
        ("flags", C.c_int32), ("splits", C.c_int32), ("nopad_lo", C.c_int32), ("prefetch_kib", C.c_int32),
        ("tattn_causal", C.c_int32),
        ("colsum", C.c_void_p), ("ln_gamma", C.c_void_p), ("ln_beta", C.c_void_p), ("ln_out", C.c_void_p),
        ("ld_ln", C.c_int32), ("ln_eps", C.c_float),
        ("rowsum", C.c_void_p), ("lnf_part", C.c_void_p), ("lnf_wsum", C.c_void_p),
        ("lnf_nparts", C.c_int32), ("reserved2_", C.c_int32),
        ("gstat", C.c_void_p), ("gstat_rows", C.c_int32), ("tattn_scale", C.c_float),
        ("prefetch", C.c_void_p), ("up_phase", C.c_int32), ("reserved4_", C.c_int32),
        ("a2", C.c_void_p), ("lda2", C.c_int32), ("k1", C.c_int32), ("gstat_cpg", C.c_int32), ("gstat_coff", C.c_int32),
        ("wgroup_rows", C.c_int32), ("wgroup_stride", C.c_int32),
    ]


class FifoState(C.Structure):
    _fields_ = [("head", C.c_int32), ("iter", C.c_int32), ("seed_lo", C.c_uint32), ("seed_hi", C.c_uint32),
                ("ext_noise", C.c_int32), ("reserved_", C.c_int32 * 3)]


class FifoStepParams(C.Structure):
    _fields_ = [
        ("state", C.c_void_p), ("x", C.c_void_p), ("eps_c", C.c_void_p), ("eps_u", C.c_void_p), ("noise", C.c_void_p),
        ("momentum", C.c_void_p), ("queue", C.c_void_p), ("x_prev", C.c_void_p), ("pred_x0", C.c_void_p), ("coef", C.c_void_p),
        ("win_start", C.c_void_p), ("mask", C.c_void_p), ("mask_sums", C.c_void_p), ("mask_frame", C.c_void_p),
        ("enh", C.c_void_p), ("cond", C.c_void_p), ("sam_eff", C.c_void_p), ("sam_idx", C.c_void_p),
        ("cfg_scale", C.c_float), ("beta", C.c_float), ("one_minus_beta", C.c_float), ("gamma", C.c_float),
        ("one_minus_gamma", C.c_float),
        ("nW", C.c_int32), ("C", C.c_int32), ("Q", C.c_int32), ("f", C.c_int32), ("HW", C.c_int32), ("wb_from", C.c_int32),
    ]


_vp, _i32, _i64, _f32, _f64 = C.c_void_p, C.c_int32, C.c_int64, C.c_float, C.c_double
SIGNATURES = {
    "moca_gemm_f16": (C.c_int, [C.POINTER(GemmParams), _vp]),
    "moca_gemm_splitk_ws_bytes": (_i64, [_i32, _i32, _i32]),
    "moca_gemm_colsum_rows": (C.c_int, [C.POINTER(GemmParams)]),
    "moca_gemm_ln_ok": (C.c_int, [C.POINTER(GemmParams)]),
    "moca_gemm_rowsum_cols": (C.c_int, [C.POINTER(GemmParams)]),
    "moca_gemm_lnfold_ok": (C.c_int, [C.POINTER(GemmParams)]),
    "moca_gemm_tattn_ok": (C.c_int, [C.POINTER(GemmParams)]),
    "moca_gemm_cat_ok": (C.c_int, [C.POINTER(GemmParams)]),
    "moca_gemm_wgroup_ok": (C.c_int, [C.POINTER(GemmParams)]),
    "moca_gemm_route": (C.c_int, [C.POINTER(GemmParams)]),
    "moca_groupnorm_fold_weights_f16": (C.c_int, [_vp, _vp, _vp, _vp, _vp, _vp, _vp, _i32, _i32, _i32, _i32, _i64, _f32, _vp]),
    "moca_gemm_splitk_groupnorm_ok": (C.c_int, [C.POINTER(GemmParams), _i32, _i32]),
    "moca_gemm_splitk_groupnorm_f16": (C.c_int, [C.POINTER(GemmParams), _vp, _vp, _vp, _i32, _i32, _f32, _i32, _i32, _vp]),
    "moca_groupnorm_gstat_cat_f16": (C.c_int, [_vp, _vp, _vp, _vp, _vp, _vp, _vp, _i32, _i32, _i32, _i32, _i32, _i32, _f32, _i32, _vp]),
    "moca_gstat_accum_f16": (C.c_int, [_vp, _i32, _i32, _i32, _i32, _i32, _i32, _vp, _vp]),
    "moca_groupnorm_colsum_f16": (C.c_int, [_vp, _vp, _vp, _vp, _vp, _i32, _i32, _i32, _i32, _i32, _f32, _i32, _vp, _vp]),
    "moca_groupnorm_nhwc_f16": (C.c_int, [_vp, _vp, _vp, _vp, _i32, _i32, _i32, _i32, _f32, _i32, _vp, _vp]),
    "moca_groupnorm_ws_bytes": (_i64, [_i32, _i32, _i32]),
    "moca_groupnorm_gstat_f16": (C.c_int, [_vp, _vp, _vp, _vp, _vp, _i32, _i32, _i32, _i32, _f32, _i32, _vp]),
    "moca_memset_zero": (C.c_int, [_vp, _i64, _vp]),
    "moca_concat_channels_gstat_f16": (C.c_int, [_vp, _vp, _vp, _i32, _i32, _i32, _i32, _i32, _vp, _vp]),
    "moca_layernorm_f16": (C.c_int, [_vp, _vp, _vp, _vp, _i32, _i32, _f32, _vp]),
    "moca_attention_f16": (C.c_int, [_vp, _vp, _vp, _vp, _i32, _i32, _i32, _i32, _i32, _i32, _i32, _i32, _i32, _f32, _vp]),
    "moca_attention_ip_f16": (C.c_int, [_vp, _vp, _vp, _vp, _vp, _vp] + [_i32] * 12 + [_f32, _f32, _vp]),
    "moca_attention_causal_f16": (C.c_int, [_vp, _vp, _vp, _vp, _i32, _i32, _i32, _i32, _i32, _i32, _i32, _f32, _vp]),
    "moca_embed_tokens_f16": (C.c_int, [_vp, _vp, _vp, _vp, _i32, _i32, _i32, _i32, _vp]),
    "moca_attention_d80_f16": (C.c_int, [_vp, _vp, _vp, _vp, _i32, _i32, _i32, _i32, _i32, _i32, _i32, _f32, _vp]),
    "moca_clip_preprocess_patches_f16": (C.c_int, [_vp, _i32, _vp, _i32, _i32, _i32, _i32, _i32, _i32, _i32, _vp]),
    "moca_clip_assemble_tokens_f16": (C.c_int, [_vp, _i32, _vp, _vp, _vp, _i32, _i32, _i32, _vp]),
    "moca_temporal_attention_f16": (C.c_int, [_vp, _vp, _vp, _vp, _i32, _i32, _i32, _i32, _i32, _i32, _f32, _vp]),
    "moca_temporal_attention_causal_f16": (C.c_int, [_vp, _vp, _vp, _vp, _i32, _i32, _i32, _i32, _i32, _i32, _f32, _vp]),
    "moca_temporal_attention_long_f16": (C.c_int, [_vp, _vp, _vp, _vp, _i32, _i32, _i32, _i32, _i32, _i32, _f32, _i32, _vp]),
    "moca_ncthw_to_nhwc_f16": (C.c_int, [_vp, _i32, _vp, _i32, _i32, _i32, _i32, _i32, _vp]),
    "moca_ncthw_scatter_f16": (C.c_int, [_vp, _i32, _vp, _i32, _i32, _i32, _i32, _i32, _i32, _vp]),
    "moca_nchw_add_rows_f16": (C.c_int, [_vp, _vp, _i32, _i32, _i32, _i32, _i32, _i32, _vp]),
    "moca_nhwc_to_ncthw": (C.c_int, [_vp, _i32, _vp, _i32, _i32, _i32, _i32, _i32, _vp]),
    "moca_concat_channels_f16": (C.c_int, [_vp, _vp, _vp, _i64, _i32, _i32, _vp]),
    "moca_repeat_f16": (C.c_int, [_vp, _vp, _i64, _i32, _vp]),
    "moca_timestep_embedding_f16": (C.c_int, [_vp, _vp, _i32, _i32, _f32, _vp]),
    "moca_silu_add_rows_f16": (C.c_int, [_vp, _i32, _vp, _i32, _vp, _i32, _i32, _i32, _vp]),
    "moca_channel_mix_f16": (C.c_int, [_vp, _i32, _vp, _vp, _vp, _i32, _i32, _i32, _i32, _i32, _i32, _f32, _vp]),
    "moca_softmax_rows_f16": (C.c_int, [_vp, _vp, _i64, _i32, _i64, _i64, _f32, _vp]),
    "moca_gaussian_sample_f32": (C.c_int, [_vp, _vp, _vp, _i32, _i32, _i32, _f32, _vp]),
    "moca_cfg_combine_f32": (C.c_int, [_vp, _vp, _vp, _f32, _i64, _vp]),
    "moca_ddim_update_f32": (C.c_int, [_vp, _vp, _vp, _vp, _vp, _f32, _f32, _f32, _f32, _i32, _f32, _f32, _i64, _vp]),
    "moca_q_sample_f32": (C.c_int, [_vp, _vp, _vp, _vp, _vp, _vp, _i32, _i32, _i64, _vp]),
    "moca_fifo_ddim_step_f32": (C.c_int, [_vp, _vp, _vp, _vp, _vp, _vp, _vp, _vp, _vp, _vp, _vp, _vp,
                                          _i32, _i32, _i32, _i32, _i32, _f32, _f32, _f32, _f32, _vp]),
    "moca_fifo_randn_f32": (C.c_int, [_vp, _vp, _i64, _vp]),
    "moca_fifo_gather_windows_f32": (C.c_int, [_vp, _vp, _vp, _vp, _vp, _i32, _i32, _i32, _i32, _i32, _i32, _vp]),
    "moca_fifo_step_windows_f32": (C.c_int, [C.POINTER(FifoStepParams), _vp]),
    "moca_sam_select_masks_f32": (C.c_int, [_vp, _vp, _vp, _vp, _vp, _vp, _i32, _i32, _i32, _vp]),
    "moca_fifo_advance_f32": (C.c_int, [_vp, _vp, _vp, _vp, _i32, _i32, _vp, _vp, _i32, _i32, _i32, _vp]),
    "moca_fifo_prepare_queue_f32": (C.c_int, [_vp, _vp, _vp, _vp, _vp, _vp, _i32, _i32, _i32, _i32, _vp]),
    "moca_base_set_timestep": (C.c_int, [_vp, _vp, _i32, _vp, _i32, _vp]),
    "moca_base_ddim_step_f32": (C.c_int, [_vp, _vp, _vp, _vp, _vp, _vp, _vp, _i32, _f32, _i32, _i64, _vp]),
    "moca_mask_frame_sums_f32": (C.c_int, [_vp, _vp, _i32, _i32, _vp]),
    "moca_freq_mix_3d_f32": (C.c_int, [_vp, _vp, _vp, _vp, _i32, _i32, _i32, _i32, _vp, _vp]),
    "moca_freq_mix_ws_bytes": (_i64, [_i32, _i32, _i32, _i32]),
    "moca_freq_filter_f32": (C.c_int, [_vp, _i32, _i32, _i32, _i32, _i32, _f64, _f64, _vp]),
    "moca_graph_begin": (C.c_int, [_vp]),
    "moca_graph_end": (C.c_int, [_vp, C.POINTER(_vp)]),
    "moca_graph_launch": (C.c_int, [_vp, _vp]),
    "moca_graph_destroy": (C.c_int, [_vp]),
    "moca_stream_create": (C.c_int, [C.POINTER(_vp)]),
    "moca_stream_destroy": (C.c_int, [_vp]),
    "moca_stream_sync": (C.c_int, [_vp]),
    "moca_event_create": (C.c_int, [C.POINTER(_vp)]),
    "moca_event_record": (C.c_int, [_vp, _vp]),
    "moca_event_elapsed_ms": (C.c_int, [_vp, _vp, C.POINTER(_f32)]),
    "moca_event_destroy": (C.c_int, [_vp]),
    "moca_set_tuning": (C.c_int, [_i32, _i32]),
    "moca_debug_clock_sampler": (C.c_int, [_vp, _i32, _i32, _vp, _vp]),
    "moca_device_info": (C.c_int, [C.c_char_p, _i32, C.POINTER(_i32)]),
    "moca_version": (C.c_char_p, []),
}

_lib = None


def load():
    global _lib
    if _lib is not None:
        return _lib
    if not os.path.exists(LIB_PATH):
        raise ImportError(
            f"{LIB_PATH} is missing: the HIP extension has not been built. Run "
            "`python -c 'import __graft_entry__ as g; g.build()'` (or `make -C moca_video_amd/csrc`). "
            "moca_video_amd has no CPU fallback by design.")
    lib = C.CDLL(LIB_PATH)
    for name, (res, args) in SIGNATURES.items():
        fn = getattr(lib, name)
        fn.restype = res
        fn.argtypes = args
    ver = lib.moca_version().decode()
    if "DIAG:" in ver and os.environ.get("MOCA_HIP_DIAG") != "1":
        raise ImportError(f"{LIB_PATH} is a diagnostic build ({ver}); set MOCA_HIP_DIAG=1 to load it on purpose")
    _lib = lib
    for kv in os.environ.get("MOCA_TUNE", "").split(","):
        if kv:
            k, v = kv.split(":")
            if lib.moca_set_tuning(int(k), int(v)) < 0:
                raise MocaHipError(f"MOCA_TUNE: bad knob setting {kv!r}")
    return lib


def check(rc: int, what: str = ""):
    if rc != 0:
        raise MocaHipError(f"{what or 'moca_hip call'} failed: {_ERR.get(rc, rc)} (rc={rc})")


def ptr(t):
    if t is None:
        return None
    return C.c_void_p(t.data_ptr())


def set_tuning(knob: int, value: int) -> int:
    old = load().moca_set_tuning(knob, value)
    if old < 0:
        raise MocaHipError(f"moca_set_tuning({knob}, {value}): bad argument")
    return old


def version() -> str:
    return load().moca_version().decode()


def device_info():
    lib = load()
    name = C.create_string_buffer(64)
    cus = C.c_int32(0)
    check(lib.moca_device_info(name, 64, C.byref(cus)), "moca_device_info")
    return name.value.decode(), cus.value
```

moca_video_amd/ops.py:

```python
from __future__ import annotations

import ctypes as C
import os
import torch

from . import lib as _l

_stream = None


def set_stream(handle):
    global _stream
    _stream = handle


def current_stream():
    if _stream is None:
        return torch.cuda.current_stream().cuda_stream
    return _stream


def _st():
    return C.c_void_p(current_stream())


def _round_up(x, m):
    return (x + m - 1) // m * m


class PackedWeight:
    __slots__ = ("w", "bias", "N", "K", "n_out", "geglu", "wsum", "derived")

    def __init__(self, w, bias, N, K, n_out, geglu=False):
        self.w, self.bias, self.N, self.K, self.n_out, self.geglu = w, bias, N, K, n_out, geglu
        self.wsum = None
        self.derived = False


def _finish(w2d: torch.Tensor, bias, device, n_out=None, geglu=False) -> PackedWeight:
    n, k = w2d.shape
    npad, kpad = _round_up(n, 64), _round_up(k, 64)
    w = torch.zeros(npad, kpad, dtype=torch.float16, device=device)
    w[:n, :k] = w2d.to(device=device, dtype=torch.float16)
    b = None
    if bias is not None:
        b = torch.zeros(npad, dtype=torch.float32, device=device)
        b[:n] = bias.to(device=device, dtype=torch.float32)
    return PackedWeight(w, b, npad, k, n if n_out is None else n_out, geglu)


def pack_linear(weight, bias=None, device="cuda"):
    w = weight.reshape(weight.shape[0], -1)
    return _finish(w, bias, device)


def pack_linear_cat(weights, biases=None, device="cuda"):
    w = torch.cat([x.reshape(x.shape[0], -1) for x in weights], dim=0)
    b = None
    if biases is not None:
        b = torch.cat(list(biases), dim=0)
    return _finish(w, b, device)


def pack_conv3x3(weight, bias=None, cpad=None, device="cuda"):
    n, c = weight.shape[0], weight.shape[1]
    cpad = c if cpad is None else cpad
    w = torch.zeros(n, 3, 3, cpad, dtype=weight.dtype, device=weight.device)
    w[..., :c] = weight.permute(0, 2, 3, 1)
    return _finish(w.reshape(n, 9 * cpad), bias, device)


def pack_upconv_phases(weight, bias=None, device="cuda"):
    n, c = weight.shape[0], weight.shape[1]
    w32 = weight.detach().to(torch.float32)
    rows = (((0,), (1, 2)), ((0, 1), (2,)))
    out = []
    for a in range(2):
        for b in range(2):
            w = torch.zeros(n, 2, 2, c, dtype=torch.float32, device=weight.device)
            for r in range(2):
                for s_ in range(2):
                    for ky in rows[a][r]:
                        for kx in rows[b][s_]:
                            w[:, r, s_, :] += w32[:, :, ky, kx]
            out.append(_finish(w.reshape(n, 4 * c), bias, device))
    return out


def pack_conv1x1(weight, bias=None, device="cuda"):
    return _finish(weight.reshape(weight.shape[0], weight.shape[1]), bias, device)


def pack_tconv3(weight, bias=None, device="cuda"):
    n, c = weight.shape[0], weight.shape[1]
    w = weight.reshape(n, c, 3).permute(0, 2, 1).reshape(n, 3 * c)
    return _finish(w, bias, device)


def pack_geglu(weight, bias, device="cuda"):
    two_inner, k = weight.shape
    inner = two_inner // 2
    assert inner % 32 == 0
    idx = torch.arange(inner, device=weight.device).reshape(inner // 32, 32)
    order = torch.cat([idx, idx + inner], dim=1).reshape(-1)
    p = _finish(weight[order], bias[order] if bias is not None else None, device, n_out=inner, geglu=True)
    return p


def fold_layernorm(weight, bias, gamma, beta):
    w = weight.reshape(weight.shape[0], -1).float()
    g, be = gamma.to(w.device).float(), beta.to(w.device).float()
    b = w @ be
    if bias is not None:
        b = b + bias.to(w.device).float()
    return w * g[None, :], b


def finish_lnfold(pw: PackedWeight) -> PackedWeight:
    pw.wsum = pw.w.float().sum(dim=1).contiguous()
    return pw


def _gemm_params(a, pw: PackedWeight, out, *, M, lda=None, mode=_l.MOCA_A_LINEAR, rowadd=None, rowadd_div=1,
                 residual=None, conv=None, tconv=None, out_f32=False, splits=1, splitk_ws=None, gelu=False, colsum=None, ln=None,
                 force_small=False, rowsum=None, lnfold=None, gstat=None, tattn=None, up_phase=0, prefetch=None, a2=None, slabs=False,
                 wgroup=None):
    p = _l.GemmParams()
    if wgroup is not None:
        p.wgroup_rows, p.wgroup_stride = wgroup
    p.up_phase = up_phase
    if a2 is not None:
        p.a2, p.lda2, p.k1 = a2[0].data_ptr(), a2[0].stride(-2), a2[1]
    if prefetch is not None:
        p.prefetch, p.prefetch_kib = prefetch.data_ptr(), (prefetch.numel() * prefetch.element_size()) >> 10
    p.a, p.w, p.out = a.data_ptr(), pw.w.data_ptr(), (out.data_ptr() if out is not None else None)
    p.bias = pw.bias.data_ptr() if pw.bias is not None else None
    p.rowadd = rowadd.data_ptr() if rowadd is not None else None
    p.residual = residual.data_ptr() if residual is not None else None
    p.splitk_ws = splitk_ws.data_ptr() if splitk_ws is not None else None
    p.M, p.N, p.K = M, pw.N, pw.K
    p.lda = lda if lda is not None else (a.stride(-2) if a.dim() >= 2 else pw.K)
    p.ldw = pw.w.stride(0)
    p.ldo = out.stride(-2) if out is not None else pw.N
    p.ldr = residual.stride(-2) if residual is not None else 0
    p.ld_rowadd = rowadd.stride(-2) if rowadd is not None else 0
    p.rowadd_div = rowadd_div
    p.a_mode = mode
    if conv is not None:
        p.C, p.inH, p.inW, p.outH, p.outW, p.stride, p.up = conv[:7]
        p.nopad_lo = conv[7] if len(conv) > 7 else 0
    if tconv is not None:
        p.C, p.T, p.HW = tconv
    p.flags = (_l.MOCA_EP_GEGLU if pw.geglu else 0) | (_l.MOCA_EP_OUT_F32 if out_f32 else 0) | \
              ((_l.MOCA_EP_GELU | _l.MOCA_FORCE_SMALL_TILE) if gelu else 0) | (_l.MOCA_EP_COLSUM if colsum is not None else 0) | \
              (_l.MOCA_FORCE_SMALL_TILE if force_small else 0)
    p.colsum = colsum.data_ptr() if colsum is not None else None
    if ln is not None:
        p.flags |= _l.MOCA_EP_LN
        p.ln_gamma, p.ln_beta = ln[0].data_ptr(), ln[1].data_ptr()
        p.ln_out = ln[2].data_ptr() if ln[2] is not None else None
        p.ld_ln = ln[2].stride(-2) if ln[2] is not None else pw.N
        p.ln_eps = ln[3]
    if rowsum is not None:
        p.flags |= _l.MOCA_EP_ROWSUM
        p.rowsum = rowsum.data_ptr() if torch.is_tensor(rowsum) else None
    if tattn is not None:
        p.flags |= _l.MOCA_EP_TATTN
        p.T, p.HW, p.tattn_scale = tattn[:3]
        p.tattn_causal = 1 if len(tattn) > 3 and tattn[3] else 0
    if gstat is not None:
        p.flags |= _l.MOCA_EP_GSTAT
        p.gstat = gstat[0].data_ptr()
        p.gstat_rows = gstat[1]
        if len(gstat) > 2:
            p.gstat_cpg, p.gstat_coff = gstat[2], gstat[3]
    if lnfold is not None:
        p.flags |= _l.MOCA_EP_LNFOLD
        p.lnf_part = lnfold[0].data_ptr() if lnfold[0] is not None else None
        p.lnf_nparts = lnfold[1]
        p.ln_eps = lnfold[2]
        p.lnf_wsum = pw.wsum.data_ptr() if pw.wsum is not None else None
    if slabs:
        p.flags |= _l.MOCA_EP_SLABS
    p.splits = splits
    return p


def gemm(a, pw: PackedWeight, out, **kw):
    p = _gemm_params(a, pw, out, **kw)
    _l.check(_l.load().moca_gemm_f16(C.byref(p), _st()), "moca_gemm_f16")
    return out


def gemm_ln_ok(a, pw: PackedWeight, **kw):
    p = _gemm_params(a, pw, None, **kw)
    return bool(_l.load().moca_gemm_ln_ok(C.byref(p)))


def gemm_rowsum_cols(a, pw: PackedWeight, **kw):
    p = _gemm_params(a, pw, None, **kw)
    return int(_l.load().moca_gemm_rowsum_cols(C.byref(p)))


def gemm_lnfold_ok(a, pw: PackedWeight, **kw):
    p = _gemm_params(a, pw, None, **kw)
    return bool(_l.load().moca_gemm_lnfold_ok(C.byref(p)))


def gemm_wgroup_ok(a, pw: PackedWeight, **kw):
    p = _gemm_params(a, pw, None, **kw)
    return bool(_l.load().moca_gemm_wgroup_ok(C.byref(p)))


def gemm_route(a, pw: PackedWeight, out=None, **kw):
    p = _gemm_params(a, pw, out, **kw)
    return int(_l.load().moca_gemm_route(C.byref(p)))


def groupnorm_fold_weights(pw: PackedWeight, gamma, beta, gstat, wg, bg, *, n_sg, count, eps):
    _l.check(_l.load().moca_groupnorm_fold_weights_f16(_l.ptr(pw.w), _l.ptr(pw.bias) if pw.bias is not None else None, _l.ptr(gamma), _l.ptr(beta),
                                                       _l.ptr(gstat), _l.ptr(wg), _l.ptr(bg), n_sg, pw.N, pw.K, pw.w.stride(0), count, eps, _st()),
             "moca_groupnorm_fold_weights_f16")
    out = PackedWeight(wg, bg, pw.N, pw.K, pw.n_out)
    out.derived = True
    return out


def gemm_tattn_ok(a, pw: PackedWeight, **kw):
    p = _gemm_params(a, pw, None, **kw)
    return bool(_l.load().moca_gemm_tattn_ok(C.byref(p)))


def pack_qkv_per_head(wq, wk, wv, heads, bias=None, device="cuda"):
    C_ = wq.shape[0]
    assert C_ == heads * 64 and wk.shape[0] == C_ and wv.shape[0] == C_
    w = torch.stack([wq.reshape(heads, 64, -1), wk.reshape(heads, 64, -1), wv.reshape(heads, 64, -1)], dim=1).reshape(3 * C_, -1)
    b = None
    if bias is not None:
        b = torch.stack([bias[:C_].reshape(heads, 64), bias[C_:2 * C_].reshape(heads, 64), bias[2 * C_:].reshape(heads, 64)], dim=1).reshape(-1)
    return _finish(w, b, device)


def gemm_splitk_groupnorm_ok(a, pw: PackedWeight, *, HW, frames_per_stat, **kw):
    p = _gemm_params(a, pw, None, slabs=True, **kw)
    return bool(_l.load().moca_gemm_splitk_groupnorm_ok(C.byref(p), HW, frames_per_stat))


def gemm_splitk_groupnorm(a, pw: PackedWeight, out, y, gamma, beta, *, HW, frames_per_stat, eps, silu, write_x, **kw):
    kw = {k: v for k, v in kw.items() if k not in ("slabs", "colsum", "prefetch")}
    p = _gemm_params(a, pw, out, slabs=True, **kw)
    _l.check(_l.load().moca_gemm_splitk_groupnorm_f16(C.byref(p), _l.ptr(y), _l.ptr(gamma), _l.ptr(beta), HW, frames_per_stat, eps,
                                                      1 if silu else 0, 1 if write_x else 0, _st()), "moca_gemm_splitk_groupnorm_f16")
    return y


def gemm_cat_ok(a, pw: PackedWeight, **kw):
    p = _gemm_params(a, pw, None, **kw)
    return bool(_l.load().moca_gemm_cat_ok(C.byref(p)))


def gemm_colsum_rows(a, pw: PackedWeight, **kw):
    p = _gemm_params(a, pw, None, **kw)
    return int(_l.load().moca_gemm_colsum_rows(C.byref(p)))


def groupnorm(x, y, gamma, beta, *, F, HW, Cn, frames_per_stat, eps, silu, ws):
    _l.check(_l.load().moca_groupnorm_nhwc_f16(_l.ptr(x), _l.ptr(y), _l.ptr(gamma), _l.ptr(beta), F, HW, Cn,
                                               frames_per_stat, eps, 1 if silu else 0, _l.ptr(ws), _st()),
             "moca_groupnorm_nhwc_f16")
    return y


def groupnorm_colsum(x, y, gamma, beta, colsum, *, tile_rows, F, HW, Cn, frames_per_stat, eps, silu, ws):
    _l.check(_l.load().moca_groupnorm_colsum_f16(_l.ptr(x), _l.ptr(y), _l.ptr(gamma), _l.ptr(beta), _l.ptr(colsum), tile_rows, F, HW, Cn,
                                                 frames_per_stat, eps, 1 if silu else 0, _l.ptr(ws), _st()),
             "moca_groupnorm_colsum_f16")
    return y


def groupnorm_gstat(x, y, gamma, beta, gstat, *, F, HW, Cn, frames_per_stat, eps, silu):
    _l.check(_l.load().moca_groupnorm_gstat_f16(_l.ptr(x), _l.ptr(y), _l.ptr(gamma), _l.ptr(beta), _l.ptr(gstat), F, HW, Cn,
                                                frames_per_stat, eps, 1 if silu else 0, _st()), "moca_groupnorm_gstat_f16")
    return y


def concat_channels_gstat(a, b, out, gstat, *, F, HW, C1, C2, frames_per_stat):
    _l.check(_l.load().moca_concat_channels_gstat_f16(_l.ptr(a), _l.ptr(b), _l.ptr(out), F, HW, C1, C2, frames_per_stat,
                                                      _l.ptr(gstat), _st()), "moca_concat_channels_gstat_f16")
    return out


def groupnorm_gstat_cat(a, b, y, gamma, beta, gstat_cat, gstat_b, *, F, HW, C1, C2, frames_per_stat, eps, silu, Fb=0):
    _l.check(_l.load().moca_groupnorm_gstat_cat_f16(_l.ptr(a), _l.ptr(b), _l.ptr(y), _l.ptr(gamma), _l.ptr(beta), _l.ptr(gstat_cat),
                                                    _l.ptr(gstat_b) if gstat_b is not None else None, Fb, F, HW, C1, C2, frames_per_stat,
                                                    eps, 1 if silu else 0, _st()), "moca_groupnorm_gstat_cat_f16")
    return y


def gstat_accum(x, gstat, *, F, HW, Cn, frames_per_stat, cpg, coff):
    _l.check(_l.load().moca_gstat_accum_f16(_l.ptr(x), F, HW, Cn, frames_per_stat, cpg, coff, _l.ptr(gstat), _st()),
             "moca_gstat_accum_f16")
    return gstat


def memset_zero(t):
    _l.check(_l.load().moca_memset_zero(_l.ptr(t), t.numel() * t.element_size(), _st()), "moca_memset_zero")
    return t


def groupnorm_ws_floats(F, HW, Cn):
    return int(_l.load().moca_groupnorm_ws_bytes(F, HW, Cn)) // 4


def layernorm(x, y, gamma, beta, *, M, Cn, eps=1e-5):
    _l.check(_l.load().moca_layernorm_f16(_l.ptr(x), _l.ptr(y), _l.ptr(gamma), _l.ptr(beta), M, Cn, eps, _st()),
             "moca_layernorm_f16")
    return y


def attention(q, k, v, out, *, Bq, heads, Nq, Nk, ldq, ldk, ldv, ldo, kv_div, scale):
    _l.check(_l.load().moca_attention_f16(_l.ptr(q), _l.ptr(k), _l.ptr(v), _l.ptr(out), Bq, heads, Nq, Nk,
                                          ldq, ldk, ldv, ldo, kv_div, scale, _st()), "moca_attention_f16")
    return out


def attention_ip(q, k, v, k_ip, v_ip, out, *, Bq, heads, Nq, Nt, Ni, ldq, ldk, ldv, ldk_ip, ldv_ip, ldo, kv_div, scale,
                 ip_scale=1.0):
    _l.check(_l.load().moca_attention_ip_f16(_l.ptr(q), _l.ptr(k), _l.ptr(v), _l.ptr(k_ip), _l.ptr(v_ip), _l.ptr(out), Bq, heads, Nq,
                                             Nt, Ni, ldq, ldk, ldv, ldk_ip, ldv_ip, ldo, kv_div, scale, ip_scale, _st()),
             "moca_attention_ip_f16")
    return out


def temporal_attention(q, k, v, out, *, B, T, HW, heads, ld_qkv, ldo, scale):
    _l.check(_l.load().moca_temporal_attention_f16(_l.ptr(q), _l.ptr(k), _l.ptr(v), _l.ptr(out), B, T, HW, heads,
                                                   ld_qkv, ldo, scale, _st()), "moca_temporal_attention_f16")
    return out


def temporal_attention_causal(q, k, v, out, *, B, T, HW, heads, ld_qkv, ldo, scale):
    _l.check(_l.load().moca_temporal_attention_causal_f16(_l.ptr(q), _l.ptr(k), _l.ptr(v), _l.ptr(out), B, T, HW, heads,
                                                          ld_qkv, ldo, scale, _st()), "moca_temporal_attention_causal_f16")
    return out


def temporal_attention_long(q, k, v, out, *, B, T, HW, heads, ld_qkv, ldo, scale, causal=False):
    _l.check(_l.load().moca_temporal_attention_long_f16(_l.ptr(q), _l.ptr(k), _l.ptr(v), _l.ptr(out), B, T, HW, heads,
                                                        ld_qkv, ldo, scale, int(bool(causal)), _st()), "moca_temporal_attention_long_f16")
    return out


def ncthw_to_nhwc(x, y, *, B, Cin, T, HW, Cpad):
    _l.check(_l.load().moca_ncthw_to_nhwc_f16(_l.ptr(x), 1 if x.dtype == torch.float32 else 0, _l.ptr(y), B, Cin, T, HW,
                                              Cpad, _st()), "moca_ncthw_to_nhwc_f16")
    return y


def ncthw_scatter(x, y, *, B, k, T, HW, Cpad, c0):
    if x.dtype not in (torch.float32, torch.float16) or not x.is_contiguous() or x.numel() != B * k * T * HW:
        raise ValueError("ncthw_scatter: x must be a contiguous fp32 / fp16 tensor of B * k * T * HW elements")
    if y.dtype != torch.float16 or not y.is_contiguous() or y.numel() != B * T * HW * Cpad:
        raise ValueError("ncthw_scatter: y must be the contiguous fp16 rows [B * T * HW][Cpad]")
    _l.check(_l.load().moca_ncthw_scatter_f16(_l.ptr(x), 1 if x.dtype == torch.float32 else 0, _l.ptr(y), B, k, T, HW, Cpad, c0,
                                              _st()), "moca_ncthw_scatter_f16")
    return y


def nchw_add_rows(rows, src, *, F, Fsrc, Cn, HW):
    if src.dtype not in (torch.float32, torch.float16) or not src.is_contiguous() or src.numel() != Fsrc * Cn * HW:
        raise ValueError("nchw_add_rows: src must be a contiguous fp32 / fp16 tensor of Fsrc * Cn * HW elements")
    if rows.dtype != torch.float16 or rows.dim() != 2 or rows.shape != (F * HW, Cn) or rows.stride(1) != 1:
        raise ValueError("nchw_add_rows: rows must be fp16 [F * HW][Cn] with unit column stride")
    _l.check(_l.load().moca_nchw_add_rows_f16(_l.ptr(rows), _l.ptr(src), 1 if src.dtype == torch.float32 else 0, F, Fsrc, Cn, HW,
                                              rows.stride(0), _st()), "moca_nchw_add_rows_f16")
    return rows


def nhwc_to_ncthw(y, ld, x, *, B, Cout, T, HW):
    _l.check(_l.load().moca_nhwc_to_ncthw(_l.ptr(y), ld, _l.ptr(x), 1 if x.dtype == torch.float32 else 0, B, Cout, T, HW,
                                          _st()), "moca_nhwc_to_ncthw")
    return x


def concat_channels(a, b, out, *, rows, C1, C2):
    _l.check(_l.load().moca_concat_channels_f16(_l.ptr(a), _l.ptr(b), _l.ptr(out), rows, C1, C2, _st()),
             "moca_concat_channels_f16")
    return out


def repeat(src, dst, *, reps):
    nb = src.numel() * src.element_size()
    assert dst.numel() * dst.element_size() == nb * reps
    _l.check(_l.load().moca_repeat_f16(_l.ptr(src), _l.ptr(dst), nb, reps, _st()), "moca_repeat_f16")
    return dst


def timestep_embedding(t, out, *, n, dim, max_period=10000.0):
    _l.check(_l.load().moca_timestep_embedding_f16(_l.ptr(t), _l.ptr(out), n, dim, max_period, _st()),
             "moca_timestep_embedding_f16")
    return out


def silu_add_rows(a, div_a, b, div_b, out, *, rows, Cn, silu):
    _l.check(_l.load().moca_silu_add_rows_f16(_l.ptr(a), div_a, _l.ptr(b), div_b, _l.ptr(out), rows, Cn,
                                              1 if silu else 0, _st()), "moca_silu_add_rows_f16")
    return out


def channel_mix(z, w, bias, out, *, B, Cin, T, HW, Cout, Cpad, inv_scale):
    _l.check(_l.load().moca_channel_mix_f16(_l.ptr(z), 1 if z.dtype == torch.float32 else 0, _l.ptr(w), _l.ptr(bias), _l.ptr(out),
                                            B, Cin, T, HW, Cout, Cpad, inv_scale, _st()), "moca_channel_mix_f16")
    return out


def softmax_rows(s, p, *, R, N, scale):
    _l.check(_l.load().moca_softmax_rows_f16(_l.ptr(s), _l.ptr(p), R, N, s.stride(-2), p.stride(-2), scale, _st()),
             "moca_softmax_rows_f16")
    return p


def gaussian_sample(moments, noise, out, *, n, z, hw, scale):
    _l.check(_l.load().moca_gaussian_sample_f32(_l.ptr(moments), _l.ptr(noise), _l.ptr(out), n, z, hw, scale, _st()),
             "moca_gaussian_sample_f32")
    return out


def attention_causal(q, k, v, out, *, B, heads, N, ldq, ldk, ldv, ldo, scale):
    _l.check(_l.load().moca_attention_causal_f16(_l.ptr(q), _l.ptr(k), _l.ptr(v), _l.ptr(out), B, heads, N, ldq, ldk, ldv, ldo,
                                                 scale, _st()), "moca_attention_causal_f16")
    return out


def embed_tokens(tokens, table, pos, out, *, n_tokens, L, Cn, vocab):
    _l.check(_l.load().moca_embed_tokens_f16(_l.ptr(tokens), _l.ptr(table), _l.ptr(pos), _l.ptr(out), n_tokens, L, Cn, vocab, _st()),
             "moca_embed_tokens_f16")
    return out


def attention_d80(q, k, v, out, *, B, heads, N, ldq, ldk, ldv, ldo, scale):
    _l.check(_l.load().moca_attention_d80_f16(_l.ptr(q), _l.ptr(k), _l.ptr(v), _l.ptr(out), B, heads, N, ldq, ldk, ldv, ldo, scale,
                                              _st()), "moca_attention_d80_f16")
    return out


def clip_preprocess_patches(img, out, *, size=224, patch=14, antialias=True):
    B, _, H, W = img.shape
    _l.check(_l.load().moca_clip_preprocess_patches_f16(_l.ptr(img), int(img.dtype == torch.float32), _l.ptr(out), B, H, W, size, patch,
                                                        out.stride(0), int(bool(antialias)), _st()), "moca_clip_preprocess_patches_f16")
    return out


def clip_assemble_tokens(patch, cls, pos, out, *, B, P, Cn):
    _l.check(_l.load().moca_clip_assemble_tokens_f16(_l.ptr(patch), patch.stride(0), _l.ptr(cls), _l.ptr(pos), _l.ptr(out), B, P, Cn, _st()),
             "moca_clip_assemble_tokens_f16")
    return out
```

Before: 62.60.

## Add 256-row temporal-attention tile and split SQP tail tiles into halves

Adds a 256-row variant of the fused temporal-attention GEMM kernel (4 M-subtiles, 16 pixels per tile), chosen when it gives fewer waves of tiles across the persistent block count than the 320-row shape. It also adds a persistent SQP GEMM variant that splits leftover tail tiles into two N-halves handled by different blocks, to balance the last wave. Both are on by default through new tuning knobs. The tail-half path makes tile scheduling in the kernel more complex and risks load-balance or correctness problems at the edges.

```diff
diff --git a/include/moca_hip.h b/include/moca_hip.h
--- a/include/moca_hip.h
+++ b/include/moca_hip.h
@@ -86,6 +86,8 @@
 int moca_gemm_rowsum_cols(const moca_gemm_params* p);
 int moca_gemm_lnfold_ok(const moca_gemm_params* p);
 int moca_gemm_tattn_ok(const moca_gemm_params* p);
+int moca_gemm_tattn_rows(const moca_gemm_params* p);
+int moca_gemm_sqp_half_tiles(const moca_gemm_params* p);
 int moca_gemm_wgroup_ok(const moca_gemm_params* p);
 int moca_gemm_cat_ok(const moca_gemm_params* p);
 #define MOCA_ROUTE_SMALL64   1
@@ -283,7 +285,10 @@
 #define MOCA_TUNE_SQP_WALK   8
 #define MOCA_TUNE_SLAB_F16   9
 #define MOCA_TUNE_GEMM_WS    10
-#define MOCA_TUNE_COUNT      11
+#define MOCA_TUNE_TATTN_256  11
+#define MOCA_TUNE_SQP_HALF   12
+#define MOCA_TUNE_SQP_BLOCKS 13
+#define MOCA_TUNE_COUNT      14
 int moca_set_tuning(int32_t knob, int32_t value);
 int moca_debug_clock_sampler(void* buf, int32_t blocks, int32_t nsamples, const int32_t* stop, void* stream);
 
diff --git a/moca_video_amd/csrc/gemm.hip b/moca_video_amd/csrc/gemm.hip
--- a/moca_video_amd/csrc/gemm.hip
+++ b/moca_video_amd/csrc/gemm.hip
@@ -474,13 +474,23 @@
     return ((p.M + 255) / 256) * (p.N / BN) >= blocks;
 }
 
+int tattn_tile_rows(const moca_gemm_params& p) {
+    if (p.HW <= 0 || p.M <= 0 || p.N % 192) return 0;
+    const int mode = moca_tuning_get(MOCA_TUNE_TATTN_256);
+    const bool can320 = p.HW % 20 == 0, can256 = mode && p.HW % 16 == 0;
+    if (!can256 || !can320) return (mode == 2 && can256) ? 256 : (can320 ? 320 : 0);
+    if (mode == 2) return 256;
+    const int64_t heads = p.N / 192, t320 = (p.M / 320) * heads, t256 = (p.M / 256) * heads;
+    return ((t256 + SQP_BLOCKS - 1) / SQP_BLOCKS) * 256 < ((t320 + SQP_BLOCKS - 1) / SQP_BLOCKS) * 320 ? 256 : 320;
+}
+
 Route route_of(const moca_gemm_params& p) {
     if (p.flags & MOCA_EP_TATTN) return R_TATTN;
     const int ws_mode = moca_tuning_get(MOCA_TUNE_GEMM_WS);
     if (ws_mode && moca_gemm_ws_ok(p) && (ws_mode == 2 || p.residual || p.M >= (1 << 17))) return R_WS;
     if (!p.a2 && p.wgroup_rows <= 0) {
         const int sqp_mode = moca_tuning_get(MOCA_TUNE_GEMM_SQP), g4p_mode = moca_tuning_get(MOCA_TUNE_GEMM_G4P);
-        if (sqp_mode && persistent_ok(p, 256, SQP_BLOCKS) && (sqp_mode == 2 || (p.flags & MOCA_EP_GEGLU))) return R_SQP;
+        if (sqp_mode && persistent_ok(p, 256, sqp_blocks()) && (sqp_mode == 2 || (p.flags & MOCA_EP_GEGLU))) return R_SQP;
         if (g4p_mode && persistent_ok(p, 128, G4P_BLOCKS) && (g4p_mode == 2 || (p.flags & MOCA_EP_GEGLU))) return R_G4P;
     }
     const int w80_mode = moca_tuning_get(MOCA_TUNE_GEMM_W80);
@@ -540,7 +550,7 @@
     const bool linear1 = p.a_mode == MOCA_A_LINEAR && p.splits == 1;
     if (r == R_TATTN) {
         if (!linear1 || !fast_gather(p) || !buffer_addressable(p) || p.residual || p.rowadd || (p.flags & MOCA_FORCE_SMALL_TILE)) return false;
-        if (p.N % 192 || p.T != 16 || p.HW <= 0 || p.HW % 20 || p.M % (16 * p.HW)) return false;
+        if (p.N % 192 || p.T != 16 || p.HW <= 0 || !tattn_tile_rows(p) || p.M % (16 * p.HW)) return false;
         if (p.ldo % 4 || p.ldo < p.N / 3) return false;
         return p.tattn_causal == 0 || (p.tattn_causal == 1 && p.tattn_scale > 0.f);
     }
@@ -645,7 +655,7 @@
 
 int launch_route(Route r, const moca_gemm_params& p, hipStream_t st) {
     switch (r) {
-        case R_TATTN: return moca_gemm_w80s_launch(3, p, st);
+        case R_TATTN: return moca_gemm_w80s_launch(tattn_tile_rows(p) == 256 ? 4 : 3, p, st);
         case R_WS: return moca_gemm_ws_launch(p, st);
         case R_SQP: return moca_gemm_sqp_launch(p, st);
         case R_G4P: return moca_gemm_g4p_launch(p, st);
@@ -695,6 +705,14 @@
 extern "C" int moca_gemm_tattn_ok(const moca_gemm_params* pp) {
     moca_gemm_params p;
     return query_route(pp, MOCA_EP_TATTN, p) != R_NONE;
+}
+extern "C" int moca_gemm_tattn_rows(const moca_gemm_params* pp) {
+    moca_gemm_params p;
+    return query_route(pp, MOCA_EP_TATTN, p) != R_NONE ? tattn_tile_rows(p) : 0;
+}
+extern "C" int moca_gemm_sqp_half_tiles(const moca_gemm_params* pp) {
+    moca_gemm_params p;
+    return query_route(pp, 0, p) == R_SQP ? sqp_half_tiles(p) : 0;
 }
 extern "C" int moca_gemm_cat_ok(const moca_gemm_params* pp) {
     moca_gemm_params p;
diff --git a/moca_video_amd/csrc/gemm_launch.h b/moca_video_amd/csrc/gemm_launch.h
--- a/moca_video_amd/csrc/gemm_launch.h
+++ b/moca_video_amd/csrc/gemm_launch.h
@@ -12,6 +12,13 @@
 
 constexpr int G4P_BLOCKS = 512;
 constexpr int SQP_BLOCKS = 256;
+inline int sqp_blocks() { return moca_tuning_get(MOCA_TUNE_SQP_BLOCKS) ? SQP_BLOCKS : 8; }
+inline int sqp_half_tiles(const moca_gemm_params& p) {
+    const int mode = moca_tuning_get(MOCA_TUNE_SQP_HALF);
+    if (!mode || (mode == 1 && p.K < 640) || !(p.flags & MOCA_EP_GEGLU)) return 0;
+    const int nper = sqp_blocks(), rest = (int)((int64_t)((p.M + 255) / 256) * (p.N / 256) % nper);
+    return 2 * rest <= nper ? rest : 0;
+}
 
 static int choose_xcd_n(const moca_gemm_params& p, int tiles_m, int tiles_n, int BN) {
     if (p.splits != 1 || p.a_mode != MOCA_A_LINEAR) return 1;
diff --git a/moca_video_amd/csrc/gemm_persistent.hip b/moca_video_amd/csrc/gemm_persistent.hip
--- a/moca_video_amd/csrc/gemm_persistent.hip
+++ b/moca_video_amd/csrc/gemm_persistent.hip
@@ -526,8 +526,8 @@
     return (rho & ~63) + (g4p_perm(rho & 127) & 63);
 }
 
-template <bool GEGLU>
-__global__ __launch_bounds__(512, 2) void gemm_sqp_kernel(const moca_gemm_params p) {
+template <bool GEGLU, bool HALVES>
+__device__ __forceinline__ void sqp_body(const moca_gemm_params& p) {
 #if defined(__HIP_DEVICE_COMPILE__)
 #ifndef SEG_WAVE
 #define SEG_WAVE 0
@@ -546,26 +546,47 @@
     const int tiles_n = p.N / BN, tiles_m = (p.M + TM - 1) / TM;
     const int xcd_n = p.reserved4_ >> 8;
     const int J = nper >> 3;
+    constexpr int Q_TAIL = 0x40000000, Q_NONE = 0x7fffffff;
     int q_base, q_cnt, sub_n, tm_base, tn_base;
+    int tail_t = 0, tail_h = -1;
     {
-        const int x = blockIdx.x & 7;
+        const int x = blockIdx.x & 7, j = blockIdx.x >> 3;
+        const int ntiles = tiles_m * tiles_n;
+        constexpr bool halves = HALVES;
+        const bool odd = (J & 1) != 0;
+        const int F = (ntiles / nper) * J, R = ntiles - 8 * F;
+        const int ti = (int)blockIdx.x >> 1;
+        const int xo = odd ? ti & 7 : x, k = odd ? ti >> 3 : j >> 1, h = odd ? blockIdx.x & 1 : j & 1;
         if (xcd_n > 1) {
             const int xm = 8 / xcd_n, sm = tiles_m / xm;
             sub_n = tiles_n / xcd_n;
             const int xi = x / xcd_n, xj = x - xi * xcd_n;
             tm_base = xi * sm; tn_base = xj * sub_n;
-            q_base = 0; q_cnt = sm * sub_n;
+            q_base = 0; q_cnt = halves ? F : sm * sub_n;
+            if (halves && k < sm * sub_n - F) {
+                const int l = F + k, a = l / sub_n;
+                tail_t = ((xo / xcd_n) * sm + a) * tiles_n + (xo % xcd_n) * sub_n + (l - a * sub_n);
+                tail_h = h;
+            }
         } else {
-            const int ntiles = tiles_m * tiles_n, q = ntiles >> 3, r = ntiles & 7;
+            const int q = ntiles >> 3, r = ntiles & 7;
             q_base = x < r ? x * (q + 1) : r * (q + 1) + (x - r) * q;
             q_cnt = q + (x < r ? 1 : 0);
             sub_n = tiles_n; tm_base = 0; tn_base = 0;
+            if (halves && odd) {
+                q_base = x * F;
+                if (ti < R) { tail_t = 8 * F + ti; tail_h = h; }
+            } else if (halves) {
+                if (k < q_cnt - F) { tail_t = q_base + F + k; tail_h = h; }
+            }
+            if (halves) q_cnt = F;
         }
     }
     auto tile_of = [&](int q, int& tm, int& tn) {
         const int l = q_base + q;
         const int a = l / sub_n;
         tm = tm_base + a; tn = tn_base + (l - a * sub_n);
+        if (HALVES && q == Q_TAIL) { tm = tail_t / tiles_n; tn = tail_t - tm * tiles_n; }
     };
     int q_cur, q_step, q_end;
     {
@@ -578,7 +599,16 @@
             q_cur = j; q_end = q_cnt; q_step = J;
         }
     }
-    if (q_cur >= q_end) return;
+    if (q_cur >= q_end) {
+        if (!HALVES || tail_h < 0) return;
+        q_cur = Q_TAIL;
+    }
+    auto no_item = [&](int q) -> bool { return HALVES ? q == Q_NONE : q >= q_end; };
+    auto next_item = [&](int q) -> int {
+        if (!HALVES) return q + q_step;
+        if (q < Q_TAIL && q + q_step < q_end) return q + q_step;
+        return (q < Q_TAIL && tail_h >= 0) ? Q_TAIL : Q_NONE;
+    };
     const int nk = p.K / 32;
 
     const int lrow = lane >> 2, pch = lane & 3;
@@ -589,13 +619,14 @@
     int d_q = q_cur, d_k = 0;
     auto set_dma_tile = [&](int q) {
         int tm, tn;
-        tile_of(q, tm, tn);
-        const bool any = q < q_end;
+        const bool any = HALVES ? q != Q_NONE : q < q_end;
+        tile_of((HALVES && !any) ? 0 : q, tm, tn);
+        const bool any_w = any && (!HALVES || q != Q_TAIL || (wave >> 2) == tail_h);
 #pragma unroll
         for (int g = 0; g < 2; ++g) {
             const int row = tm * TM + (g * 8 + wave) * 16 + lrow;
             a_off[g] = (any && row < p.M) ? (unsigned)(((int64_t)row * p.lda + lch * 8) * 2) : OOB_OFF;
-            w_off[g] = any ? (unsigned)(((int64_t)(tn * BN + sqp_perm((g * 8 + wave) * 16 + lrow)) * p.ldw + lch * 8) * 2) : OOB_OFF;
+            w_off[g] = any_w ? (unsigned)(((int64_t)(tn * BN + sqp_perm((g * 8 + wave) * 16 + lrow)) * p.ldw + lch * 8) * 2) : OOB_OFF;
         }
     };
     auto issue_pair = [&](int slot_even, int slot_odd) {
@@ -612,7 +643,7 @@
             __builtin_amdgcn_raw_ptr_buffer_load_lds(rsrc_w, so + A_BYTES + (g * 8 + wave) * 1024, 16, w_off[g], soff + KS * 2, 0, 0);
         }
         d_k += 2;
-        if (d_k >= nk) { d_k = 0; d_q += q_step; set_dma_tile(d_q); }
+        if (d_k >= nk) { d_k = 0; d_q = next_item(d_q); set_dma_tile(d_q); }
     };
 
     const int fr = lane & 15, fg = lane >> 4;
@@ -621,11 +652,11 @@
     const int b_off0 = A_BYTES + (wave_n * WTN + fr) * RB + swz;
     f32x4 acc[MT][NT];
     half8v af[2][MT], bf[2][NT];
-    auto read_tile = [&](auto set_tag, int slot) {
-        constexpr int S = decltype(set_tag)::value;
+    auto read_tile = [&](auto set_tag, auto nt_tag, int slot, int b_off) {
+        constexpr int S = decltype(set_tag)::value, NTH = decltype(nt_tag)::value;
         const char* cur = smem + slot * STAGE;
 #pragma unroll
-        for (int r = 0; r < NT; ++r) bf[S][r] = *reinterpret_cast<const half8v*>(cur + b_off0 + r * 1024);
+        for (int r = 0; r < NTH; ++r) bf[S][r] = *reinterpret_cast<const half8v*>(cur + b_off + r * 1024);
 #pragma unroll
         for (int r = 0; r < MT; ++r) af[S][r] = *reinterpret_cast<const half8v*>(cur + a_off0 + r * 1024);
     };
@@ -641,7 +672,7 @@
     const int stat_floats = 2 + 2 * (fold ? p.lnf_nparts : 0);
     auto stat_dma = [&](int q, unsigned slot_off) {
         int tm, tn;
-        tile_of(q < q_end ? q : 0, tm, tn);
+        tile_of((HALVES ? q != Q_NONE : q < q_end) ? q : 0, tm, tn);
         const int t = tid_now();
         const int n = tn * BN + sqp_perm(t);
         const int m = min(tm * TM + t, p.M - 1);
@@ -707,7 +738,10 @@
 #ifdef MOCA_STAMPS
     int tile_no = 0;
 #endif
-    while (true) {
+    auto do_item = [&](auto half_tag) -> int {
+        constexpr bool HALF = decltype(half_tag)::value;
+        constexpr int NTH = HALF ? NT / 2 : NT;
+        const int b_off = HALF ? b_off0 + tail_h * (WTN / 2) * RB : b_off0;
         int tm, tn;
         tile_of(q_cur, tm, tn);
         const int m0 = tm * TM, n0 = tn * BN;
@@ -718,7 +752,7 @@
 #pragma unroll
         for (int mt = 0; mt < MT; ++mt)
 #pragma unroll
-            for (int nt = 0; nt < NT; ++nt) acc[mt][nt] = f32x4{0.f, 0.f, 0.f, 0.f};
+            for (int nt = 0; nt < NTH; ++nt) acc[mt][nt] = f32x4{0.f, 0.f, 0.f, 0.f};
         for (int i = 0; i < nk; i += 2) {
             const int s1 = s0 + 1 == NS ? 0 : s0 + 1;
             const int sp = s0 == 0 ? NS - 1 : s0 - 1;
@@ -726,7 +760,7 @@
             const bool seg = stamp_it && i == SEG_ITER;
             if (seg) MOCA_STAMP_W(8, SEG_WAVE);
 #endif
-            read_tile(int_c<0>{}, s0);
+            read_tile(int_c<0>{}, int_c<NTH>{}, s0, b_off);
             asm volatile("s_waitcnt lgkmcnt(0)" ::: "memory");
             __builtin_amdgcn_sched_barrier(0);
 #ifdef MOCA_STAMPS
@@ -740,14 +774,14 @@
                 const char* nx = smem + s1 * STAGE;
                 __builtin_amdgcn_s_setprio(1);
 #pragma unroll
-                for (int j = 0; j < MT * NT; ++j) {
-                    const int mt = j / NT, nt = j % NT;
+                for (int j = 0; j < MT * NTH; ++j) {
+                    const int mt = j / NTH, nt = j % NTH;
                     acc[mt][nt] = __builtin_amdgcn_mfma_f32_16x16x32_f16(bf[0][nt], af[0][mt], acc[mt][nt], 0, 0, 0);
-                    if (j % 2 == 0 && j / 2 < MT + NT) {
+                    if (j % 2 == 0 && j / 2 < MT + NTH) {
                         const int r = j / 2;
                         __builtin_amdgcn_sched_barrier(0);
-                        if (r < NT) bf[1][r] = *reinterpret_cast<const half8v*>(nx + b_off0 + r * 1024);
-                        else af[1][r - NT] = *reinterpret_cast<const half8v*>(nx + a_off0 + (r - NT) * 1024);
+                        if (r < NTH) bf[1][r] = *reinterpret_cast<const half8v*>(nx + b_off + r * 1024);
+                        else af[1][r - NTH] = *reinterpret_cast<const half8v*>(nx + a_off0 + (r - NTH) * 1024);
                         __builtin_amdgcn_sched_barrier(0);
                     }
                 }
@@ -779,7 +813,7 @@
 #pragma unroll
             for (int mt = 0; mt < MT; ++mt)
 #pragma unroll
-                for (int nt = 0; nt < NT; ++nt)
+                for (int nt = 0; nt < NTH; ++nt)
                     acc[mt][nt] = __builtin_amdgcn_mfma_f32_16x16x32_f16(bf[1][nt], af[1][mt], acc[mt][nt], 0, 0, 0);
             __builtin_amdgcn_s_setprio(0);
             __builtin_amdgcn_sched_barrier(0);
@@ -812,11 +846,11 @@
         f32x2 st[MT];
 #pragma unroll
         for (int mt = 0; mt < MT; ++mt) st[mt] = lds_rd_f2(lst + 8 * (wave_m * WTM + mt * 16 + fr));
-        const int q_next = q_cur + q_step;
+        const int q_next = HALF ? Q_NONE : next_item(q_cur);
         const unsigned stat_slot = (unsigned)((s0 == 0 ? NS - 1 : s0 - 1) * STAGE);
-        if (!late) stat_dma(q_next, stat_slot);
-#pragma unroll
-        for (int grp = 0; grp < 2; ++grp) {
+        if constexpr (!HALF) { if (!late) stat_dma(q_next, stat_slot); }
+        auto epi_group = [&](auto ag_tag, const int grp) {
+            constexpr int AG = decltype(ag_tag)::value;
             f32x4 cw[4], cb[4];
 #pragma unroll
             for (int t = 0; t < 4; ++t) {
@@ -829,7 +863,7 @@
                 const int m = m0 + wave_m * WTM + mt * 16 + fr;
                 f32x4 v[4];
 #pragma unroll
-                for (int t = 0; t < 4; ++t) v[t] = st[mt][0] * acc[mt][grp * 4 + t] + (st[mt][1] * cw[t] + cb[t]);
+                for (int t = 0; t < 4; ++t) v[t] = st[mt][0] * acc[mt][AG * 4 + t] + (st[mt][1] * cw[t] + cb[t]);
                 if constexpr (GEGLU) {
                     half8v h;
 #pragma unroll
@@ -864,22 +898,41 @@
                     }
                 }
             }
-        }
+        };
+        if constexpr (HALF) epi_group(int_c<0>{}, tail_h);
+        else { epi_group(int_c<0>{}, 0); epi_group(int_c<1>{}, 1); }
 #ifdef MOCA_STAMPS
         if (stamp_it) { MOCA_STAMP(5); MOCA_STAMP_HW(); }
         ++tile_no;
 #endif
-        if (!late) {
-            if (m0 + TM > p.M) lf = stat_read(stat_slot, int_c<0>{});
-            else lf = stat_read(stat_slot, int_c<(GEGLU ? 8 : 16)>{});
-        }
-        if (q_next >= q_end) break;
-        q_cur = q_next;
-        if (late) __builtin_amdgcn_s_barrier();
+        if constexpr (!HALF) {
+            if (!late) {
+                if (m0 + TM > p.M) lf = stat_read(stat_slot, int_c<0>{});
+                else lf = stat_read(stat_slot, int_c<(GEGLU ? 8 : 16)>{});
+            }
+        }
+        return q_next;
+    };
+    if (!HALVES || q_cur != Q_TAIL) {
+        while (true) {
+            const int q_next = do_item(no_t{});
+            if (no_item(q_next)) break;
+            q_cur = q_next;
+            if (late) __builtin_amdgcn_s_barrier();
+            if (HALVES && q_cur == Q_TAIL) break;
+        }
+    }
+    if constexpr (HALVES) {
+        if (q_cur == Q_TAIL) do_item(yes_t{});
     }
     asm volatile("s_waitcnt vmcnt(0) lgkmcnt(0)" ::: "memory");
 #endif
 }
+
+template <bool GEGLU>
+__global__ __launch_bounds__(512, 2) void gemm_sqp_kernel(const moca_gemm_params p) { sqp_body<GEGLU, false>(p); }
+template <bool GEGLU>
+__global__ __launch_bounds__(512, 2) void gemm_sqph_kernel(const moca_gemm_params p) { sqp_body<GEGLU, true>(p); }
 
 template <bool GEGLU>
 int launch_gemm_g4p(const moca_gemm_params& p, hipStream_t st) {
@@ -902,10 +955,19 @@
     constexpr int lds = 5 * (256 + 256) * 64;
     if (!dyn_lds_once<&gemm_sqp_kernel<GEGLU>>(lds)) return MOCA_E_LAUNCH;
     moca_gemm_params pl = p;
-    pl.reserved2_ = SQP_BLOCKS;
-    pl.reserved4_ = (pl.reserved4_ & 0xfd) | (choose_xcd_n(p, (p.M + 255) / 256, p.N / 256, 256) << 8) |
+    const int nper = sqp_blocks(), tiles_m = (p.M + 255) / 256, tiles_n = p.N / 256;
+    pl.reserved2_ = nper;
+    pl.reserved4_ = (pl.reserved4_ & 0xfd) | (choose_xcd_n(p, tiles_m, tiles_n, 256) << 8) |
                     (moca_tuning_get(MOCA_TUNE_SQP_WALK) ? 2 : 0);
-    hipLaunchKernelGGL((gemm_sqp_kernel<GEGLU>), dim3(SQP_BLOCKS + prefetch_blocks(pl)), dim3(512), lds, st, pl);
+    if constexpr (GEGLU) {
+        if (sqp_half_tiles(p) > 0) {
+            if (!dyn_lds_once<&gemm_sqph_kernel<true>>(lds)) return MOCA_E_LAUNCH;
+            hipLaunchKernelGGL((gemm_sqph_kernel<true>), dim3(nper + prefetch_blocks(pl)), dim3(512), lds, st, pl);
+            MOCA_CHECK_LAUNCH();
+            return MOCA_OK;
+        }
+    }
+    hipLaunchKernelGGL((gemm_sqp_kernel<GEGLU>), dim3(nper + prefetch_blocks(pl)), dim3(512), lds, st, pl);
     MOCA_CHECK_LAUNCH();
     return MOCA_OK;
 }
diff --git a/moca_video_amd/csrc/gemm_tiled.hip b/moca_video_amd/csrc/gemm_tiled.hip
--- a/moca_video_amd/csrc/gemm_tiled.hip
+++ b/moca_video_amd/csrc/gemm_tiled.hip
@@ -676,18 +676,30 @@
 #include "gemm_w80s_kernel.inc"
 #undef MOCA_W80S_NAME
 #undef MOCA_W80S_CAUSAL
+#define MOCA_W80S_NAME gemm_w80s_tq16_kernel
+#define MOCA_W80S_CAUSAL false
+#include "gemm_w80s_kernel.inc"
+#undef MOCA_W80S_NAME
+#undef MOCA_W80S_CAUSAL
+#define MOCA_W80S_NAME gemm_w80s_tq16_causal_kernel
+#define MOCA_W80S_CAUSAL true
+#include "gemm_w80s_kernel.inc"
+#undef MOCA_W80S_NAME
+#undef MOCA_W80S_CAUSAL
 
 template <int AMODE, int SHAPE, bool CAUSAL = false>
 int launch_gemm_w80s(const moca_gemm_params& p, hipStream_t st) {
     constexpr auto kernel = [] {
-        if constexpr (CAUSAL) return &gemm_w80s_causal_kernel<AMODE, SHAPE>;
+        if constexpr (SHAPE == 4) return CAUSAL ? &gemm_w80s_tq16_causal_kernel<AMODE, SHAPE> : &gemm_w80s_tq16_kernel<AMODE, SHAPE>;
+        else if constexpr (CAUSAL) return &gemm_w80s_causal_kernel<AMODE, SHAPE>;
         else return &gemm_w80s_kernel<AMODE, SHAPE>;
     }();
-    constexpr int TM = SHAPE == 2 ? 256 : (SHAPE == 1 ? 160 : 320), BN = SHAPE == 2 ? 256 : (SHAPE == 1 ? 320 : (SHAPE == 3 ? 192 : 160));
+    constexpr bool TQ = SHAPE == 3 || SHAPE == 4;
+    constexpr int TM = (SHAPE == 2 || SHAPE == 4) ? 256 : (SHAPE == 1 ? 160 : 320), BN = SHAPE == 2 ? 256 : (SHAPE == 1 ? 320 : (TQ ? 192 : 160));
     const int tiles_m = (p.M + TM - 1) / TM, tiles_n = p.N / BN;
     const int nblk = tiles_m * tiles_n * p.splits;
     moca_gemm_params pl = p;
-    pl.reserved4_ = (pl.reserved4_ & 0xff) | ((SHAPE == 3 ? 1 : choose_xcd_n(p, tiles_m, tiles_n, BN)) << 8);
+    pl.reserved4_ = (pl.reserved4_ & 0xff) | ((TQ ? 1 : choose_xcd_n(p, tiles_m, tiles_n, BN)) << 8);
     constexpr int lds = 5 * (TM + BN) * 64;
     if (!dyn_lds_once<kernel>(lds)) return MOCA_E_LAUNCH;
     hipLaunchKernelGGL(kernel, dim3(nblk + prefetch_blocks(pl)), dim3(512), lds, st, pl);
@@ -741,6 +753,7 @@
             return with_gather(p, [&](auto am, auto) { return launch_gemm_w80s<decltype(am)::value, 1>(p, st); });
         case 2: return launch_gemm_w80s<MOCA_A_LINEAR, 2>(p, st);
         case 3: return p.tattn_causal ? launch_gemm_w80s<MOCA_A_LINEAR, 3, true>(p, st) : launch_gemm_w80s<MOCA_A_LINEAR, 3>(p, st);
+        case 4: return p.tattn_causal ? launch_gemm_w80s<MOCA_A_LINEAR, 4, true>(p, st) : launch_gemm_w80s<MOCA_A_LINEAR, 4>(p, st);
     }
     return MOCA_E_BADARG;
 }
diff --git a/moca_video_amd/csrc/gemm_w80s_kernel.inc b/moca_video_amd/csrc/gemm_w80s_kernel.inc
--- a/moca_video_amd/csrc/gemm_w80s_kernel.inc
+++ b/moca_video_amd/csrc/gemm_w80s_kernel.inc
@@ -2,15 +2,16 @@
 __global__ __launch_bounds__(512, 2) void MOCA_W80S_NAME(const moca_gemm_params p) {
 #if defined(__HIP_DEVICE_COMPILE__)
     constexpr bool CAUSAL = MOCA_W80S_CAUSAL;
-    static_assert(!CAUSAL || SHAPE == 3, "the causal mask belongs to the MOCA_EP_TATTN epilogue");
-    constexpr bool WIDE = SHAPE == 1, SQ = SHAPE == 2, TQ = SHAPE == 3;
-    constexpr int MT = SQ ? 4 : 5, NT = SQ ? 8 : (TQ ? 6 : 5), KS = 32, RB = 64;
+    static_assert(!CAUSAL || SHAPE == 3 || SHAPE == 4, "the causal mask belongs to the MOCA_EP_TATTN epilogue");
+    constexpr bool WIDE = SHAPE == 1, SQ = SHAPE == 2, TQ16 = SHAPE == 4, TQ = SHAPE == 3 || TQ16;
+    constexpr int MT = (SQ || TQ16) ? 4 : 5, NT = SQ ? 8 : (TQ ? 6 : 5), KS = 32, RB = 64;
     constexpr int WTM = 16 * MT, WTN = 16 * NT;
-    constexpr int TM = SQ ? 256 : (WIDE ? 160 : 320), BN = SQ ? 256 : (WIDE ? 320 : (TQ ? 192 : 160));
+    constexpr int TM = (SQ || TQ16) ? 256 : (WIDE ? 160 : 320), BN = SQ ? 256 : (WIDE ? 320 : (TQ ? 192 : 160));
+    constexpr int TQ_PX = TM / 16;
     constexpr int A_BYTES = TM * RB, STAGE = A_BYTES + BN * RB;
     constexpr int NS = 5;
     constexpr int PPW = 4;
-    constexpr int NAP = SQ ? 2 : (WIDE ? 2 : 3);
+    constexpr int NAP = (SQ || TQ16) ? 2 : (WIDE ? 2 : 3);
 
     extern __shared__ __attribute__((aligned(16))) char smem[];
     MOCA_STAMP(0);
@@ -44,13 +45,13 @@
 
     const int lrow = lane >> 2, pch = lane & 3;
     const int lch = pch ^ ((0x78 >> (2 * ((lrow >> 2) & 3))) & 3);
-    const bool flex_is_big = wave < 4;
+    const bool flex_is_big = !TQ16 && wave < 4;
     const int kt_last_pair = kt_begin + nk - 2;
     BGather<AMODE, NAP, KS> ga(p, lch, kt_begin, kt_last_pair);
     const int small1 = TQ ? 4 + wave : (wave < 6 ? 4 + wave : 2 + wave);
-    const int tq_tpv = TQ ? p.HW / 20 : 1;
+    const int tq_tpv = TQ ? p.HW / TQ_PX : 1;
     const int tq_b = tile_m / tq_tpv, tq_pb = tile_m - tq_b * tq_tpv;
-    auto grow = [&](int tr) -> int { return TQ ? (tq_b * 16 + (tr & 15)) * p.HW + tq_pb * 20 + (tr >> 4) : m0 + tr; };
+    auto grow = [&](int tr) -> int { return TQ ? (tq_b * 16 + (tr & 15)) * p.HW + tq_pb * TQ_PX + (tr >> 4) : m0 + tr; };
     const int wg = (AMODE == MOCA_A_LINEAR && p.wgroup_rows > 0) ? m0 / p.wgroup_rows : 0;
     const unsigned wgo = (unsigned)((int64_t)wg * p.wgroup_stride * 2);
     unsigned w_off[3];
@@ -98,7 +99,7 @@
                 __builtin_amdgcn_raw_ptr_buffer_load_lds(rsrc_a, sa + (j * 8 + wave) * 1024, 16, ga.a_off[j], a_s, 0, 0);
             } else if (j == 2) {
                 const lds_ptr dst = flex_is_big ? sa + (16 + (wave & 3)) * 1024 : sa + A_BYTES + (wave & 3) * 1024;
-                __builtin_amdgcn_raw_ptr_buffer_load_lds(rsrc_f, dst, 16, flex_is_big ? ga.a_off[2] : w_off[0], flex_is_big ? a_s : w_s, 0, 0);
+                __builtin_amdgcn_raw_ptr_buffer_load_lds(rsrc_f, dst, 16, flex_is_big ? ga.a_off[NAP - 1] : w_off[0], flex_is_big ? a_s : w_s, 0, 0);
             } else {
                 __builtin_amdgcn_raw_ptr_buffer_load_lds(rsrc_w, sa + A_BYTES + small1 * 1024, 16, w_off[1], w_s, 0, 0);
             }
@@ -359,12 +360,12 @@
     if constexpr (TQ) {
         const float sl2e = p.tattn_scale * 1.4426950408889634f;
         half_t* outp = reinterpret_cast<half_t*>(p.out);
-        constexpr int NPX = 3;
+        constexpr int NPX = (TQ_PX + 7) / 8;
         int pixs[NPX];
         half8v kf[NPX][2], qf[NPX][2];
 #pragma unroll
         for (int i = 0; i < NPX; ++i) {
-            pixs[i] = min(wave + 8 * i, 19);
+            pixs[i] = min(wave + 8 * i, TQ_PX - 1);
             const char* base = smem + (pixs[i] * 16) * pitch;
 #pragma unroll
             for (int ks = 0; ks < 2; ++ks) {
@@ -415,7 +416,7 @@
 #pragma unroll
         for (int i = 0; i < NPX; ++i) {
             half_t* ob = outp + (int64_t)grow(pixs[i] * 16 + fr) * p.ldo + tile_n * 64;
-            const bool live = wave + 8 * i < 20;
+            const bool live = wave + 8 * i < TQ_PX;
 #pragma unroll
             for (int dt = 0; dt < 4; ++dt) {
                 f32x4 o4 = {0.f, 0.f, 0.f, 0.f};
diff --git a/moca_video_amd/csrc/runtime.hip b/moca_video_amd/csrc/runtime.hip
--- a/moca_video_amd/csrc/runtime.hip
+++ b/moca_video_amd/csrc/runtime.hip
@@ -121,7 +121,7 @@
     return MOCA_OK;
 }
 
-static int g_tuning[MOCA_TUNE_COUNT] = {1, 1, 1, 1, 1, 1, 0, 1, 0, 0, 1};
+static int g_tuning[MOCA_TUNE_COUNT] = {1, 1, 1, 1, 1, 1, 0, 1, 0, 0, 1, 1, 1, 1};
 int moca_tuning_get(int knob) { return (knob >= 0 && knob < MOCA_TUNE_COUNT) ? g_tuning[knob] : 0; }
 extern "C" int moca_set_tuning(int32_t knob, int32_t value) {
     if (knob < 0 || knob >= MOCA_TUNE_COUNT || value < 0 || value > 2) return MOCA_E_BADARG;
diff --git a/moca_video_amd/lib.py b/moca_video_amd/lib.py
--- a/moca_video_amd/lib.py
+++ b/moca_video_amd/lib.py
@@ -14,6 +14,7 @@
 MOCA_TUNE_GEMM_W80, MOCA_TUNE_GEMM_G4, MOCA_TUNE_GEMM_SQ256, MOCA_TUNE_GEMM_WIDE, MOCA_TUNE_GN_SLAB, MOCA_TUNE_GEMM_G4P, MOCA_TUNE_GEMM_MF32, MOCA_TUNE_GEMM_SQP, MOCA_TUNE_SQP_WALK = 0, 1, 2, 3, 4, 5, 6, 7, 8
 MOCA_TUNE_SLAB_F16 = 9
 MOCA_TUNE_GEMM_WS = 10
+MOCA_TUNE_TATTN_256, MOCA_TUNE_SQP_HALF, MOCA_TUNE_SQP_BLOCKS = 11, 12, 13
 (MOCA_ROUTE_SMALL64, MOCA_ROUTE_SMALL128, MOCA_ROUTE_GLDS128, MOCA_ROUTE_GLDS160, MOCA_ROUTE_G4, MOCA_ROUTE_W80, MOCA_ROUTE_W80W,
  MOCA_ROUTE_SQ256, MOCA_ROUTE_G4P, MOCA_ROUTE_SQP, MOCA_ROUTE_TATTN, MOCA_ROUTE_WS) = range(1, 13)
 
@@ -73,6 +74,8 @@
     "moca_gemm_rowsum_cols": (C.c_int, [C.POINTER(GemmParams)]),
     "moca_gemm_lnfold_ok": (C.c_int, [C.POINTER(GemmParams)]),
     "moca_gemm_tattn_ok": (C.c_int, [C.POINTER(GemmParams)]),
+    "moca_gemm_tattn_rows": (C.c_int, [C.POINTER(GemmParams)]),
+    "moca_gemm_sqp_half_tiles": (C.c_int, [C.POINTER(GemmParams)]),
     "moca_gemm_cat_ok": (C.c_int, [C.POINTER(GemmParams)]),
     "moca_gemm_wgroup_ok": (C.c_int, [C.POINTER(GemmParams)]),
     "moca_gemm_route": (C.c_int, [C.POINTER(GemmParams)]),
diff --git a/moca_video_amd/ops.py b/moca_video_amd/ops.py
--- a/moca_video_amd/ops.py
+++ b/moca_video_amd/ops.py
@@ -231,6 +231,16 @@
     return bool(_l.load().moca_gemm_tattn_ok(C.byref(p)))
 
 
+def gemm_tattn_rows(a, pw: PackedWeight, **kw):
+    p = _gemm_params(a, pw, None, **kw)
+    return int(_l.load().moca_gemm_tattn_rows(C.byref(p)))
+
+
+def gemm_sqp_half_tiles(a, pw: PackedWeight, **kw):
+    p = _gemm_params(a, pw, None, **kw)
+    return int(_l.load().moca_gemm_sqp_half_tiles(C.byref(p)))
+
+
 def pack_qkv_per_head(wq, wk, wv, heads, bias=None, device="cuda"):
     C_ = wq.shape[0]
     assert C_ == heads * 64 and wk.shape[0] == C_ and wv.shape[0] == C_
```

Result: no change. 62.71, median of 6 (+0.2%).
